# uber/aresdb

Hardware: AMD Instinct MI355X
Metric: rows/sec, 1B-row filter -> group-by-agg (whole job) (higher is better)
Workload: dtype u32 keys / f64 sums; 1 GPU; C3: filter d1<90 -> dims [floor(ts,3600), d1, d2, d3] (4 x uint32) -> SUM(m float32 -> float64) via HashReduce, validity bitmaps with 1% nulls, shard resident in HBM; rows_per_gpu=1000000000, batch_rows=67108864, batches=15, streams_per_query=2, parallelism=1 shard(s), one per GPU

## Files before the change

### aresdb_amd/csrc/algo/hash_reduce_lds.hip

```cpp
#include <hip/hip_runtime.h>

#include <atomic>
#include <functional>
#include <map>
#include <mutex>
#include <string>
#include <unordered_map>

#include <memory>
#include <mutex>
#include <vector>

#include "aggregate.hpp"
#include "common.hpp"
#include "device_model.hpp"
#include "ares_extensions.h"
#include "dim_layout.hpp"
#include "fast_eval.hpp"
#include "hash_reduce_lds.hpp"
#include "hr_kernels.hpp"
#include "hr_rtc.hpp"
#include "sort_reduce_fused.hpp"

namespace ares {

namespace {
using namespace hr;

__global__ __launch_bounds__(kThreads) void hr_partition_kernel(const uint8_t *dimValues, DimLayoutD L, size_t capacity,
                                                                const uint8_t *inputValues, AggSpec a, int length,
                                                                Workspace ws) {
  partition_generic_body(dimValues, L, capacity, inputValues, a, length, ws);
}

template <int ND, int VW>
__global__ __launch_bounds__(kThreads) void hr_partition4_kernel(const uint8_t *dimValues, size_t capacity,
                                                                 const uint8_t *inputValues, uint32_t rowStart, AggSpec a,
                                                                 int length, Workspace ws, int allowDirect) {
  DimVectorSource<ND, VW> src{dimValues, capacity, inputValues, rowStart};
  partition_body(src, a, length, ws, allowDirect);
}

template <int ND>
__global__ __launch_bounds__(kThreads) void hr_fused_scan_kernel(FusedPlanD plan, uint32_t rowBase, AggSpec a, int length,
                                                                 Workspace ws) {
  FusedSource<ND> src(plan, rowBase);
  partition_body(src, a, length, ws, 1);
}

template <int ND4, int RWB>
__global__ __launch_bounds__(kThreads) void hr_merge_kernel(const uint8_t *__restrict__ dimIn,
                                                            const uint8_t *__restrict__ inValues,
                                                            uint8_t *__restrict__ dimOut, DimLayoutD L, size_t capacity,
                                                            uint8_t *__restrict__ outputValues, AggSpec a, Workspace ws,
                                                            uint32_t prevSize) {
  merge_body<ND4, false, RWB>(dimIn, capacity, inValues, dimOut, L, capacity, outputValues, a, ws, nullptr, prevSize);
}

template <int ND, int RWB>
__global__ __launch_bounds__(kThreads) void hr_fused_merge_kernel(FusedPlanD plan, const uint8_t *__restrict__ prevDims,
                                                                  size_t prevCapacity,
                                                                  const uint8_t *__restrict__ prevValues, uint32_t prevSize,
                                                                  uint8_t *__restrict__ dimOut, size_t outCapacity,
                                                                  uint8_t *__restrict__ outputValues, AggSpec a, Workspace ws) {
  DimLayoutD L;
  L.numDims = ND;
  merge_body<ND, true, RWB>(prevDims, prevCapacity, prevValues, dimOut, L, outCapacity, outputValues, a, ws, &plan, prevSize);
}

std::mutex g_rangesMutex;
std::vector<std::pair<int, uint32_t *>> g_freeRanges;

struct SlotWidths {
  int nd = 0, dimBytes = 0;
  uint8_t width[kFusedDims] = {}, off[kFusedDims] = {};
  bool same(const SlotWidths &o) const { return nd == o.nd && memcmp(width, o.width, sizeof(width)) == 0; }
  size_t row_bytes() const { return static_cast<size_t>(dimBytes + nd); }
};
bool slot_widths(const uint8_t numDimsPerDimWidth[NUM_DIM_WIDTH], SlotWidths *out) {
  SlotWidths w;
  if (numDimsPerDimWidth[0] || numDimsPerDimWidth[1]) return false;
  for (int k = 2; k < NUM_DIM_WIDTH; k++)
    for (int j = 0; j < numDimsPerDimWidth[k]; j++) {
      if (w.nd >= kFusedDims) return false;
      w.width[w.nd] = static_cast<uint8_t>(1 << (NUM_DIM_WIDTH - 1 - k));
      w.off[w.nd] = static_cast<uint8_t>(w.dimBytes);
      w.dimBytes += w.width[w.nd];
      w.nd++;
    }
  *out = w;
  return w.nd >= 1;
}

struct GroupedState {
  int device;
  const uint8_t *dims;
  const uint8_t *values;
  size_t capacity;
  SlotWidths slots;
  int valueBytes, size, partBits;
  std::shared_ptr<uint32_t> ranges;
  std::shared_ptr<uint8_t> image;
  uint64_t lineage = 0;
  uint64_t gen = 0, parentGen = 0;
  bool lazyValues = false;
};
std::mutex g_groupedMutex;
std::vector<GroupedState> g_grouped;
constexpr size_t kRangesBytes = sizeof(uint32_t) * kMaxPartitions * kRangeWords;

bool grouped_enabled() {
  static EnvSwitch<bool> on("ARES_GROUPED", [](const char *e) { return !(e && e[0] == '0'); });
  return on.get() && deferral_hooks_active();
}

std::shared_ptr<uint32_t> take_ranges(int device) {
  uint32_t *p = nullptr;
  {
    std::lock_guard<std::mutex> lock(g_rangesMutex);
    for (size_t i = 0; i < g_freeRanges.size(); i++)
      if (g_freeRanges[i].first == device) {
        p = g_freeRanges[i].second;
        g_freeRanges[i] = g_freeRanges.back();
        g_freeRanges.pop_back();
        break;
      }
  }
  if (!p) {
    void *fresh = nullptr;
    hip_check(hipMalloc(&fresh, kRangesBytes), "hipMalloc");
    p = static_cast<uint32_t *>(fresh);
  }
  return std::shared_ptr<uint32_t>(p, [device](uint32_t *q) {
    std::lock_guard<std::mutex> lock(g_rangesMutex);
    g_freeRanges.emplace_back(device, q);
  });
}

constexpr size_t kImagePartBytes = static_cast<size_t>(kSlots) * 16;
constexpr size_t kImageCountsOff = kImagePartBytes * kMaxPartitions;
constexpr size_t kImageBytes = kImageCountsOff + sizeof(uint32_t) * kMaxPartitions;
std::vector<std::pair<int, uint8_t *>> g_freeImages;
std::atomic<uint64_t> g_lineage{0};
std::atomic<uint64_t> g_generation{0};

bool image_enabled() {
  static EnvSwitch<bool> on("ARES_IMAGE", [](const char *e) { return !(e && e[0] == '0'); });
  return on.get() && grouped_enabled();
}

std::shared_ptr<uint8_t> take_image(int device) {
  uint8_t *p = nullptr;
  {
    std::lock_guard<std::mutex> lock(g_rangesMutex);
    for (size_t i = 0; i < g_freeImages.size(); i++)
      if (g_freeImages[i].first == device) {
        p = g_freeImages[i].second;
        g_freeImages[i] = g_freeImages.back();
        g_freeImages.pop_back();
        break;
      }
  }
  if (!p) {
    void *fresh = nullptr;
    if (hipMalloc(&fresh, kImageBytes) != hipSuccess) {
      (void)hipGetLastError();
      grouped_trim(device);
      if (g_memTrimCache) g_memTrimCache(device);
      fresh = nullptr;
      if (hipMalloc(&fresh, kImageBytes) != hipSuccess) {
        (void)hipGetLastError();
        return nullptr;
      }
    }
    p = static_cast<uint8_t *>(fresh);
  }
  return std::shared_ptr<uint8_t>(p, [device](uint8_t *q) {
    std::lock_guard<std::mutex> lock(g_rangesMutex);
    g_freeImages.emplace_back(device, q);
  });
}
uint32_t *image_counts(uint8_t *image) { return reinterpret_cast<uint32_t *>(image + kImageCountsOff); }

template <int VW>
__global__ __launch_bounds__(kThreads) void hr_image_values_kernel(const uint4 *image, uint8_t *values, uint32_t size) {
  const uint4 *img = image + static_cast<size_t>(blockIdx.x) * kSlots;
  const uint32_t *keys = reinterpret_cast<const uint32_t *>(img), *pos = keys + kSlots;
  const uint64_t *vals = reinterpret_cast<const uint64_t *>(img + kSlots / 2);
  for (int s = threadIdx.x; s < kSlots; s += kThreads) {
    if (keys[s] == 0u) continue;
    const uint32_t at = pos[s];
    if (at >= size) continue;
    if (VW == 8) reinterpret_cast<uint64_t *>(values)[at] = vals[s];
    else reinterpret_cast<uint32_t *>(values)[at] = static_cast<uint32_t>(vals[s]);
  }
}

hipStream_t image_stream(int device) {
  static std::mutex mu;
  static std::map<int, hipStream_t> streams;
  std::lock_guard<std::mutex> lock(mu);
  auto it = streams.find(device);
  if (it != streams.end()) return it->second;
  hipStream_t s = nullptr;
  hip_check(hipStreamCreateWithFlags(&s, hipStreamNonBlocking), "hipStreamCreate");
  streams[device] = s;
  return s;
}

void materialize_values(GroupedState &s) {
  if (!s.lazyValues || !s.image) return;
  int current = 0;
  const bool have = hipGetDevice(&current) == hipSuccess;
  if (!have || current != s.device) hip_check(hipSetDevice(s.device), "hipSetDevice");
  hipStream_t stream = image_stream(s.device);
  uint8_t *values = const_cast<uint8_t *>(s.values);
  if (s.valueBytes == 8)
    ARES_LAUNCH("hr_image_values_kernel", hr_image_values_kernel<8>, 1 << s.partBits, kThreads, stream,
                reinterpret_cast<const uint4 *>(s.image.get()), values, static_cast<uint32_t>(s.size));
  else
    ARES_LAUNCH("hr_image_values_kernel", hr_image_values_kernel<4>, 1 << s.partBits, kThreads, stream,
                reinterpret_cast<const uint4 *>(s.image.get()), values, static_cast<uint32_t>(s.size));
  hip_check(hipStreamSynchronize(stream), "hipStreamSynchronize");
  mem_note_write(s.device, values, static_cast<size_t>(s.valueBytes) * s.size);
  s.lazyValues = false;
  if (have && current != s.device) (void)hipSetDevice(current);
}

bool state_overlaps(const GroupedState &s, const uint8_t *lo, const uint8_t *hi) {
  auto hit = [&](const uint8_t *a, size_t bytes) { return a < hi && lo < a + bytes; };
  for (int d = 0; d < s.slots.nd; d++) {
    if (hit(s.dims + s.capacity * s.slots.off[d], static_cast<size_t>(s.slots.width[d]) * s.size)) return true;
    if (hit(s.dims + s.capacity * s.slots.dimBytes + s.capacity * d, static_cast<size_t>(s.size))) return true;
  }
  return hit(s.values, static_cast<size_t>(s.valueBytes) * s.size);
}

bool grouped_lookup(int device, const uint8_t *dims, const uint8_t *values, size_t capacity, const SlotWidths &slots, int valueBytes,
                    GroupedState *out) {
  if (!grouped_enabled()) return false;
  std::lock_guard<std::mutex> lock(g_groupedMutex);
  for (const GroupedState &s : g_grouped)
    if (s.device == device && s.dims == dims && s.values == values && s.capacity == capacity && s.slots.same(slots) &&
        s.valueBytes == valueBytes) {
      *out = s;
      return true;
    }
  return false;
}

void grouped_register(const GroupedState &s) {
  std::lock_guard<std::mutex> lock(g_groupedMutex);
  if (g_grouped.size() >= 64) {
    materialize_values(g_grouped.front());
    g_grouped.erase(g_grouped.begin());
  }
  g_grouped.push_back(s);
}

struct Regions {
  Workspace ws;
  std::unique_ptr<StreamBuffer> buf;
  size_t headBytes;
};

int lean_min_groups() {
  static EnvSwitch<int> v("ARES_LEAN_MIN_GROUPS", [](const char *e) { return e ? atoi(e) : 6000; });
  return v.get();
}

std::mutex g_shapeMutex;
std::unordered_map<size_t, int> g_firstBatchGroups;

int part_bits_for(int64_t length) {
  static EnvSwitch<int> minBits("ARES_MIN_PART_BITS", [](const char *e) { return e ? atoi(e) : 0; });
  int partBits = minBits.get() > 0 ? (minBits.get() < 9 ? minBits.get() : 9) : 0;
  while ((8192ll << partBits) < length && (1 << partBits) < kMaxPartitions) partBits++;
  return partBits;
}

int grid_for(int64_t rows) {
  const int64_t tiles = (rows + kQuadTile - 1) / kQuadTile;
  return static_cast<int>(tiles < kMaxStreams ? (tiles < 1 ? 1 : tiles) : kMaxStreams);
}

bool compact_enabled() {
  static EnvSwitch<bool> on("ARES_COMPACT", [](const char *e) { return !(e && e[0] == '0'); });
  return on.get();
}

void make_regions(Regions &r, int partBits, int64_t rowsA, int64_t rowsB, int streams, int rwB, hipStream_t stream,
                  int lineRecords = 0) {
  const int numParts = 1 << partBits;
  Workspace &ws = r.ws;
  memset(&ws, 0, sizeof(ws));
  ws.partBits = partBits;
  ws.streams = streams;
  ws.capA = ((2ull * (static_cast<uint64_t>(rowsA) / numParts) + 2 * kSlots) | 63ull) + 18;
  ws.capB = 0;
  ws.lineRecords = lineRecords;
  size_t bBytes = 0;
  if (streams > 0) {
    const uint64_t mean = (static_cast<uint64_t>(rowsB) / (static_cast<uint64_t>(numParts) * streams)) << record_stream_slack();
    if (lineRecords == static_cast<int>(kCompactLineRecords)) {
      ws.capB = static_cast<uint32_t>(((2 * mean + 64) / kCompactLineRecords + 2) | 1ull);
      bBytes = 128ull * ws.capB * numParts * streams;
    } else if (lineRecords) {
      ws.capB = static_cast<uint32_t>(((2 * mean + 64 + 7) / 8 * 8) | 8ull);
      bBytes = sizeof(uint32_t) * rwB * static_cast<size_t>(ws.capB) * numParts * streams;
    } else {
      ws.capB = static_cast<uint32_t>(((2 * mean + 64) | 15ull) + 6);
      bBytes = sizeof(uint32_t) * rwB * static_cast<size_t>(ws.capB) * numParts * streams;
    }
  }
  bBytes = (bBytes + 255) / 256 * 256;
  const size_t headBytes = (sizeof(uint32_t) * (numParts + 8) + 255) / 256 * 256;
  const size_t countsBytes = (sizeof(uint32_t) * static_cast<size_t>(numParts) * (streams > 0 ? streams : 1) + 255) / 256 * 256;
  const size_t aBytes = (sizeof(uint4) * ws.capA * numParts + 255) / 256 * 256;
  r.buf.reset(new StreamBuffer(headBytes + countsBytes + aBytes + bBytes + 256, stream));
  uint8_t *base = r.buf->as<uint8_t>();
  ws.cursorsA = reinterpret_cast<uint32_t *>(base);
  ws.outCount = ws.cursorsA + numParts;
  ws.countsB = reinterpret_cast<uint32_t *>(base + headBytes);
  ws.recA = reinterpret_cast<uint4 *>(base + headBytes + countsBytes);
  ws.recB = reinterpret_cast<uint32_t *>(base + headBytes + countsBytes + aBytes);
  r.headBytes = headBytes;
  hip_check(hipMemsetAsync(base, 0, headBytes, stream), "hipMemsetAsync");
}

struct MergeResult {
  uint32_t groups, overflow, stale, needGeneric;
};
MergeResult read_result(const Workspace &ws, hipStream_t stream) {
  uint32_t w[4] = {0, 0, 0, 0};
  read_back_u32(ws.outCount, w, 4, stream);
  return MergeResult{w[0], w[1], w[2], w[3]};
}
uint32_t *result_slot() {
  static EnvSwitch<bool> on("ARES_RESULT_PINNED", [](const char *e) { return e && e[0] == '1'; });
  return on.get() ? reinterpret_cast<uint32_t *>(pinned_words()) : nullptr;
}
MergeResult read_result_pinned(hipStream_t stream) {
  hip_check(hipStreamSynchronize(stream), "hipStreamSynchronize");
  const volatile uint32_t *w = result_slot();
  return MergeResult{w[0], w[1], w[2], w[3]};
}

}

void grouped_note_write(int device, const void *ptr, size_t bytes) {
  sorted_state_note_write(device, ptr, bytes);
  const uint8_t *lo = static_cast<const uint8_t *>(ptr);
  const uint8_t *hi = lo + (bytes ? bytes : 1);
  std::lock_guard<std::mutex> lock(g_groupedMutex);
  for (size_t i = 0; i < g_grouped.size();) {
    GroupedState &st = g_grouped[i];
    if (st.device == device && state_overlaps(st, lo, hi)) {
      const uint8_t *vlo = st.values, *vhi = st.values + static_cast<size_t>(st.valueBytes) * st.size;
      if (st.lazyValues && !(lo <= vlo && vhi <= hi)) materialize_values(st);
      g_grouped.erase(g_grouped.begin() + i);
    } else {
      i++;
    }
  }
}

void grouped_materialize_for_read(int device, const void *ptr, size_t bytes) {
  if (!ptr) return;
  const uint8_t *lo = static_cast<const uint8_t *>(ptr);
  const uint8_t *hi = lo + (bytes ? bytes : 1);
  std::lock_guard<std::mutex> lock(g_groupedMutex);
  for (GroupedState &st : g_grouped) {
    if (st.device != device || !st.lazyValues) continue;
    const uint8_t *vlo = st.values, *vhi = st.values + static_cast<size_t>(st.valueBytes) * st.size;
    if (vlo < hi && lo < vhi) materialize_values(st);
  }
}

void grouped_trim(int device) {
  std::vector<void *> idle;
  {
    std::lock_guard<std::mutex> lock(g_rangesMutex);
    for (size_t i = 0; i < g_freeRanges.size();)
      if (g_freeRanges[i].first == device) {
        idle.push_back(g_freeRanges[i].second);
        g_freeRanges[i] = g_freeRanges.back();
        g_freeRanges.pop_back();
      } else {
        i++;
      }
    for (size_t i = 0; i < g_freeImages.size();)
      if (g_freeImages[i].first == device) {
        idle.push_back(g_freeImages[i].second);
        g_freeImages[i] = g_freeImages.back();
        g_freeImages.pop_back();
      } else {
        i++;
      }
  }
  for (void *p : idle) (void)hipFree(p);
}

void grouped_note_write(int device, const DimensionVector &v) {
  if (v.DimValues && v.VectorCapacity > 0) grouped_note_write(device, v.DimValues, dim_row_bytes(v.NumDimsPerDimWidth) * static_cast<size_t>(v.VectorCapacity));
}

namespace {
std::atomic<int> g_recordStreamSlack{0};
}
int record_stream_slack() { return g_recordStreamSlack.load(std::memory_order_relaxed); }
bool grow_record_stream_slack() {
  int s = g_recordStreamSlack.load(std::memory_order_relaxed);
  while (s < 2)
    if (g_recordStreamSlack.compare_exchange_weak(s, s + 1)) return true;
  return false;
}

bool hash_reduce_lds_supported(const AggSpec &a) {
  if (a.op == OP_AVG) return false;
  if (a.vtype == V_F32 && a.op != OP_SUM) return false;
  return true;
}

int hash_reduce_lds(int device, const DimensionVector &inputKeys, const uint8_t *inputValues,
                    const DimensionVector &outputKeys, uint8_t *outputValues, const AggSpec &a, int length,
                    hipStream_t stream) {
  const DimLayoutD L = make_dim_layout(inputKeys.NumDimsPerDimWidth);
  const size_t capacity = static_cast<size_t>(inputKeys.VectorCapacity);
  bool all4 = L.numDims >= 1 && L.numDims <= 4;
  for (int d = 0; d < L.numDims; d++) all4 = all4 && L.width[d] == 4;
  SlotWidths slots;
  const bool describable = slot_widths(inputKeys.NumDimsPerDimWidth, &slots);
  const int partBits = std::max(part_bits_for(length), (describable && !all4) ? 2 : 0);
  const int numParts = 1 << partBits;
  grouped_note_write(device, outputValues, static_cast<size_t>(a.width) * capacity);
  grouped_note_write(device, outputKeys.DimValues, static_cast<size_t>(L.rowBytes) * capacity);
  GroupedState prev;
  bool grouped = all4 && grouped_lookup(device, inputKeys.DimValues, inputValues, capacity, slots, a.width, &prev) &&
                 prev.ranges && prev.partBits == partBits && prev.size > 0 && prev.size <= length;
  const std::shared_ptr<uint32_t> outRangesRef = (describable && grouped_enabled()) ? take_ranges(device) : nullptr;
  uint32_t *outRanges = outRangesRef.get();
  MergeResult res{0, 0, 0, 0};
  for (;;) {
    const int start = grouped ? prev.size : 0;
    const int rows = length - start;
    RtcKernel lean;
    if (all4 && grouped && rows > 0 && start >= lean_min_groups() && (a.width == 4 || a.width == 8) && rtc_scan_available())
      lean = rtc_lookup(device, rtc_spec_vector_scan(L.numDims, a.width, partBits));
    const int streams = (all4 && rows > 0) ? (lean ? rtc_scan_grid(rows) : grid_for(rows)) : 0;
    const int rwB = (a.width == 8 || lean) ? 4 : 3;
    Regions r;
    make_regions(r, partBits, rows, rows, streams, rwB, stream, lean ? 8 : 0);
    Workspace &ws = r.ws;
    if (lean && a.width == 8) ws.widen.mode = 2;
    ws.prevRanges = grouped ? prev.ranges.get() : nullptr;
    ws.outRanges = outRanges;
    RtcKernel leanMerge = lean ? rtc_lookup(device, rtc_spec_vector_merge(L.numDims, a.width, partBits, a)) : nullptr;
    if (outRanges && !leanMerge) hip_check(hipMemsetAsync(outRanges, 0, kRangesBytes, stream), "hipMemsetAsync");
    if (lean) {
      rtc_vector_scan_launch(lean, RTC_VECTOR_SCAN, inputKeys.DimValues, capacity, inputValues + static_cast<size_t>(a.width) * start,
                             L.numDims, nullptr, static_cast<uint32_t>(start), rows, ws, stream);
    } else if (all4) {
      if (rows > 0) {
#define ARES_HR_CASE(ND)                                                                                             \
  case ND:                                                                                                           \
    if (a.width == 8)                                                                                                \
      ARES_LAUNCH("hr_partition4_kernel", (hr_partition4_kernel<ND, 8>), streams, kThreads, stream, inputKeys.DimValues, \
                  capacity, inputValues, static_cast<uint32_t>(start), a, rows, ws, 1);                             \
    else                                                                                                             \
      ARES_LAUNCH("hr_partition4_kernel", (hr_partition4_kernel<ND, 4>), streams, kThreads, stream, inputKeys.DimValues, \
                  capacity, inputValues, static_cast<uint32_t>(start), a, rows, ws, 1);                             \
    break;
        switch (L.numDims) {
          ARES_HR_CASE(1) ARES_HR_CASE(2) ARES_HR_CASE(3) ARES_HR_CASE(4)
        }
#undef ARES_HR_CASE
      }
    } else {
      const int64_t tiles = (static_cast<int64_t>(length) + kTileRows - 1) / kTileRows;
      const int grid = static_cast<int>(tiles < 256 ? tiles : 256);
      ARES_LAUNCH("hr_partition_kernel", hr_partition_kernel, grid, kThreads, stream, inputKeys.DimValues, L, capacity,
                  inputValues, a, length, ws);
    }
#define ARES_HR_MERGE(ND, RWB)                                                                                       \
  ARES_LAUNCH("hr_merge_kernel", (hr_merge_kernel<ND, RWB>), numParts, kThreads, stream, inputKeys.DimValues, inputValues, \
              outputKeys.DimValues, L, capacity, outputValues, a, ws, static_cast<uint32_t>(start))
#define ARES_HR_MERGE_ND(ND)                       \
  if (rwB == 4) ARES_HR_MERGE(ND, 4);              \
  else ARES_HR_MERGE(ND, 3);
    auto generic_merge = [&] {
      switch (all4 ? L.numDims : 0) {
        case 1: ARES_HR_MERGE_ND(1) break;
        case 2: ARES_HR_MERGE_ND(2) break;
        case 3: ARES_HR_MERGE_ND(3) break;
        case 4: ARES_HR_MERGE_ND(4) break;
        default: ARES_HR_MERGE(0, 3); break;
      }
    };
    if (leanMerge) {
      FusedPlanD none;
      memset(&none, 0, sizeof(none));
      rtc_merge_launch(leanMerge, none, inputKeys.DimValues, capacity, inputValues, static_cast<uint32_t>(start), outputKeys.DimValues,
                       capacity, outputValues, ws, stream, nullptr, result_slot());
    } else {
      generic_merge();
    }
    res = (leanMerge && result_slot()) ? read_result_pinned(stream) : read_result(ws, stream);
    mem_note_dim_rows(device, outputKeys, 0, res.groups);
    mem_note_write(device, outputValues, static_cast<size_t>(a.width) * res.groups);
    if (leanMerge && res.needGeneric && !res.overflow && !(grouped && res.stale)) {
      hip_check(hipMemsetAsync(ws.outCount, 0, 4 * sizeof(uint32_t), stream), "hipMemsetAsync");
      if (outRanges) hip_check(hipMemsetAsync(outRanges, 0, kRangesBytes, stream), "hipMemsetAsync");
      generic_merge();
      res = read_result(ws, stream);
      mem_note_dim_rows(device, outputKeys, 0, res.groups);
      mem_note_write(device, outputValues, static_cast<size_t>(a.width) * res.groups);
    }
#undef ARES_HR_MERGE_ND
#undef ARES_HR_MERGE
    if (hr_trace_enabled())
      fprintf(stderr, "hash_reduce_lds: length %d start %d rows %d streams %d capA %llu capB %u partBits %d -> groups %u overflow %u stale %u\n",
              length, start, rows, streams, static_cast<unsigned long long>(ws.capA), ws.capB, partBits, res.groups, res.overflow, res.stale);
    r.buf->mark_idle();
    if (grouped && res.stale) {
      grouped_note_write(device, inputKeys.DimValues, static_cast<size_t>(L.rowBytes) * capacity);
      grouped = false;
      continue;
    }
    break;
  }
  if (res.overflow) {
    static bool told = false;
    if (!told) {
      told = true;
      fprintf(stderr, "libalgorithm: a hash-partition region overflowed (skewed hashes?): HashReduce falls back to the global table\n");
    }
    return -1;
  }
  if (outRanges) {
    GroupedState s{device, outputKeys.DimValues, outputValues, capacity, slots, a.width, static_cast<int>(res.groups),
                   partBits, outRangesRef};
    if (res.groups > 0) grouped_register(s);
  }
  return static_cast<int>(res.groups);
}

static void fused_note_first_batch(size_t shape, int groups) {
  if (!shape || groups < 0) return;
  std::lock_guard<std::mutex> lock(g_shapeMutex);
  if (g_firstBatchGroups.size() > 4096) g_firstBatchGroups.clear();
  g_firstBatchGroups[shape] = groups;
}

int fused_hash_reduce_run(int device, const FusedPlanD &plan, int batchRows, const DimensionVector &prevKeys,
                          const uint8_t *prevValues, int prevSize, const DimensionVector &outKeys, uint8_t *outValues,
                          const AggSpec &a, hipStream_t stream) {
  SlotWidths slots;
  if (!slot_widths(outKeys.NumDimsPerDimWidth, &slots)) return kFusedUnavailable;
  const int nd = slots.nd;
  const bool narrow = fused_plan_narrow(plan, nd);
  const int mw = plan.measureWidth;
  const int64_t length = static_cast<int64_t>(batchRows) + prevSize;
  if (length == 0) return 0;
  const int partBits = std::max(part_bits_for(length), narrow ? 2 : 0);
  const int numParts = 1 << partBits;
  const size_t prevCapacity = static_cast<size_t>(prevKeys.VectorCapacity);
  const size_t outCapacity = static_cast<size_t>(outKeys.VectorCapacity);
  if (narrow && !(batchRows > 0 && rtc_scan_available())) return kFusedUnavailable;
  GroupedState outOld;
  const bool outFound = image_enabled() && grouped_lookup(device, outKeys.DimValues, outValues, outCapacity, slots, mw, &outOld);
  grouped_note_write(device, outValues, static_cast<size_t>(mw) * outCapacity);
  grouped_note_write(device, outKeys.DimValues, slots.row_bytes() * outCapacity);
  GroupedState prev;
  const bool found = prevSize > 0 && grouped_lookup(device, prevKeys.DimValues, prevValues, prevCapacity, slots, mw, &prev) &&
                     prev.partBits == partBits && prev.size == prevSize;
  bool grouped = found && prev.ranges != nullptr;
  const std::shared_ptr<uint32_t> outRangesRef = grouped_enabled() ? take_ranges(device) : nullptr;
  uint32_t *outRanges = outRangesRef.get();
  MergeResult res{0, 0, 0, 0};
  hr::Widen widen;
  widen.mode = mw == 8 ? 1 : 0;
  widen.rk = plan.measure.f.rk;
  widen.dtype = plan.measureDtype;
  size_t shape = 0;
  int expected = prevSize;
  bool known = prevSize > 0;
  const bool rtc = batchRows > 0 && rtc_scan_available();
  if (rtc && prevSize == 0) {
    const RtcSpec spec = rtc_spec_scan(plan, nd, 0, false);
    shape = std::hash<std::string>()(std::string(reinterpret_cast<const char *>(&spec), sizeof(spec)));
    std::lock_guard<std::mutex> lock(g_shapeMutex);
    auto it = g_firstBatchGroups.find(shape);
    if (it != g_firstBatchGroups.end()) {
      expected = it->second;
      known = true;
    }
  }
  const int chunkTiles = compact_enabled() ? rtc_compact_chunk_tiles(batchRows, partBits) : 0;
  const bool compact = chunkTiles > 0;
  const RtcKind leanKind = compact ? RTC_SCAN_COMPACT : RTC_SCAN_LINES16;
  RtcKernel lean, table, tableMerge, narrowMerge;
  SlowScope slowWhole("fused_hash_reduce_run");
  const bool wantLean = rtc && expected >= lean_min_groups() && (known || lean_min_groups() <= 0);
  const bool wantTable = rtc && !wantLean && (known || narrow);
  if (wantLean) lean = rtc_lookup(device, rtc_spec_scan(plan, nd, partBits, compact));
  else if (wantTable) table = rtc_lookup(device, rtc_spec_table_scan(plan, nd, partBits, a, widen));
  int imageMode = 0;
  RtcKernel imageMerge;
  std::shared_ptr<uint8_t> imageOut;
  uint32_t knownOut = 0;
  if (image_enabled() && wantLean && lean) {
    if (found && prev.image) imageMode = 2;
    else if (prevSize == 0 || grouped) imageMode = 1;
    if (imageMode) imageMerge = rtc_lookup(device, rtc_spec_merge(plan, nd, partBits, a, widen, compact, false, imageMode));
    if (!imageMerge) imageMode = 0;
  }
  if (imageMode == 2) {
    const bool mine = outFound && outOld.lineage == prev.lineage && outOld.image && outOld.image != prev.image &&
                      outOld.partBits == partBits && outOld.size <= prevSize && prev.parentGen != 0 && outOld.gen == prev.parentGen;
    knownOut = mine ? static_cast<uint32_t>(outOld.size) : 0u;
    imageOut = mine ? outOld.image : take_image(device);
    if (imageOut && !mine) hip_check(hipMemsetAsync(image_counts(imageOut.get()), 0xFF, sizeof(uint32_t) * kMaxPartitions, stream), "hipMemsetAsync");
  } else {
    if (imageMode == 1) imageOut = take_image(device);
    if (prevSize > 0) grouped_materialize_for_read(device, prevValues, static_cast<size_t>(mw) * prevSize);
  }
  if (imageMode && !imageOut) {
    imageMode = 0;
    knownOut = 0;
    if (prevSize > 0) grouped_materialize_for_read(device, prevValues, static_cast<size_t>(mw) * prevSize);
  }
  {
    if (hr_trace_enabled())
      fprintf(stderr, "fused_hash_reduce_run: batch %d prev %d partBits %d | found %d (state: size %d partBits %d ranges %d image %d lazy %d) grouped %d "
                      "| lean %d table %d compact %d narrow %d -> image mode %d knownOut %u\n",
              batchRows, prevSize, partBits, found ? 1 : 0, found ? prev.size : -1, found ? prev.partBits : -1, found && prev.ranges ? 1 : 0,
              found && prev.image ? 1 : 0, found && prev.lazyValues ? 1 : 0, grouped ? 1 : 0, lean ? 1 : 0, table ? 1 : 0, compact ? 1 : 0,
              narrow ? 1 : 0, imageMode, knownOut);
  }
  if (narrow && !imageMode) {
    narrowMerge = rtc_lookup(device, rtc_spec_merge(plan, nd, partBits, a, widen, wantLean && compact,
                                                    wantTable || (prevSize > 0 && !grouped)));
    if (!narrowMerge) return kFusedUnavailable;
  }
  if (narrow && !(wantLean ? lean : table)) return kFusedUnavailable;
  bool launched = false;
  for (;;) {
    const bool prevToA = narrow && prevSize > 0 && !grouped && imageMode != 2;
    if (narrow && !imageMode) {
      narrowMerge = rtc_lookup(device, rtc_spec_merge(plan, nd, partBits, a, widen, lean && compact, table || prevToA));
      if (!narrowMerge) return launched ? -1 : kFusedUnavailable;
      if (table) tableMerge = narrowMerge;
    }
    launched = true;
    const int streams = batchRows > 0 ? (lean ? rtc_scan_grid(batchRows) : table ? 0 : grid_for(batchRows)) : 0;
    Regions r;
    {
      SlowScope slow("make_regions");
      const int64_t rowsA = !lean ? length : (prevSize > 0 && !grouped && imageMode != 2) ? prevSize : 0;
      make_regions(r, partBits, rowsA, batchRows, streams, lean ? 4 : 3, stream,
                   !lean ? 0 : compact ? static_cast<int>(kCompactLineRecords) : 8);
    }
    Workspace &ws = r.ws;
    ws.widen = widen;
    ws.chunkRows = static_cast<uint32_t>(chunkTiles) * 4096u;
    ws.rowBase = static_cast<uint32_t>(prevSize);
    ws.prevRanges = (grouped && imageMode != 2) ? prev.ranges.get() : nullptr;
    ws.outRanges = outRanges;
    Workspace wsPrev = ws;
    wsPrev.streams = 0;
    RtcKernel leanMerge = imageMode ? imageMerge
                          : narrow  ? (lean ? narrowMerge : nullptr)
                          : (lean && (prevSize == 0 || grouped)) ? rtc_lookup(device, rtc_spec_merge(plan, nd, partBits, a, widen, compact)) : nullptr;
    RtcImageArgs imageArgs{nullptr, nullptr, nullptr, nullptr, 0u};
    if (imageMode) {
      imageArgs.in = imageMode == 2 ? prev.image.get() : nullptr;
      imageArgs.inCount = imageMode == 2 ? image_counts(prev.image.get()) : nullptr;
      imageArgs.out = imageOut.get();
      imageArgs.outCount = image_counts(imageOut.get());
      imageArgs.knownOut = knownOut;
    }
    const RtcImageArgs *imagePtr = imageMode ? &imageArgs : nullptr;
    if (prevToA) {
      const DimLayoutD prevLayout = make_dim_layout(prevKeys.NumDimsPerDimWidth);
      const int64_t tiles = (static_cast<int64_t>(prevSize) + kTileRows - 1) / kTileRows;
      ARES_LAUNCH("hr_partition_kernel", hr_partition_kernel, static_cast<int>(tiles < 256 ? tiles : 256), kThreads, stream,
                  prevKeys.DimValues, prevLayout, prevCapacity, prevValues, a, prevSize, wsPrev);
    }
    if (outRanges && !leanMerge && !tableMerge) hip_check(hipMemsetAsync(outRanges, 0, kRangesBytes, stream), "hipMemsetAsync");
#define ARES_FUSED_CASE(ND)                                                                                            \
  case ND:                                                                                                             \
    if (prevSize > 0 && !grouped && !narrow && imageMode != 2) {                                                       \
      if (mw == 8)                                                                                                     \
        ARES_LAUNCH("hr_partition4_kernel", (hr_partition4_kernel<ND, 8>), grid_for(prevSize), kThreads, stream,        \
                    prevKeys.DimValues, prevCapacity, prevValues, 0u, a, prevSize, wsPrev, 0);                         \
      else                                                                                                             \
        ARES_LAUNCH("hr_partition4_kernel", (hr_partition4_kernel<ND, 4>), grid_for(prevSize), kThreads, stream,        \
                    prevKeys.DimValues, prevCapacity, prevValues, 0u, a, prevSize, wsPrev, 0);                         \
    }                                                                                                                  \
    if (batchRows > 0 && lean)                                                                                         \
      rtc_scan_launch(lean, leanKind, plan, static_cast<uint32_t>(prevSize), batchRows, ws, stream);                   \
    else if (batchRows > 0 && table)                                                                                   \
      rtc_scan_launch(table, RTC_SCAN_TABLE, plan, static_cast<uint32_t>(prevSize), batchRows, ws, stream);            \
    else if (batchRows > 0)                                                                                            \
      ARES_LAUNCH("hr_fused_scan_kernel", hr_fused_scan_kernel<ND>, streams, kThreads, stream, plan,                   \
                  static_cast<uint32_t>(prevSize), a, batchRows, ws);                                                  \
    if (leanMerge || tableMerge)                                                                                       \
      rtc_merge_launch(leanMerge ? leanMerge : tableMerge, plan, prevKeys.DimValues, prevCapacity, prevValues,         \
                       static_cast<uint32_t>(prevSize), outKeys.DimValues, outCapacity, outValues, ws, stream, imagePtr, \
                       result_slot());                                                                                 \
    else if (lean)                                                                                                     \
      ARES_LAUNCH("hr_fused_merge_kernel", (hr_fused_merge_kernel<ND, 4>), numParts, kThreads, stream, plan,            \
                  prevKeys.DimValues, prevCapacity, prevValues, static_cast<uint32_t>(prevSize), outKeys.DimValues,    \
                  outCapacity, outValues, a, ws);                                                                      \
    else                                                                                                               \
      ARES_LAUNCH("hr_fused_merge_kernel", (hr_fused_merge_kernel<ND, 3>), numParts, kThreads, stream, plan,            \
                  prevKeys.DimValues, prevCapacity, prevValues, static_cast<uint32_t>(prevSize), outKeys.DimValues,    \
                  outCapacity, outValues, a, ws);                                                                      \
    break;
    switch (nd) {
      ARES_FUSED_CASE(1) ARES_FUSED_CASE(2) ARES_FUSED_CASE(3) ARES_FUSED_CASE(4)
      default:
        if (batchRows > 0 && lean) rtc_scan_launch(lean, leanKind, plan, static_cast<uint32_t>(prevSize), batchRows, ws, stream);
        else if (batchRows > 0 && table) rtc_scan_launch(table, RTC_SCAN_TABLE, plan, static_cast<uint32_t>(prevSize), batchRows, ws, stream);
        rtc_merge_launch(leanMerge ? leanMerge : tableMerge, plan, prevKeys.DimValues, prevCapacity, prevValues, static_cast<uint32_t>(prevSize),
                         outKeys.DimValues, outCapacity, outValues, ws, stream, imagePtr, result_slot());
        break;
    }
    {
      SlowScope slow("read_result");
      res = ((leanMerge || tableMerge) && result_slot()) ? read_result_pinned(stream) : read_result(ws, stream);
    }
    if (imageMode == 2) res.groups += static_cast<uint32_t>(prevSize);
    if (imageMode == 2) {
      if (res.groups > knownOut) mem_note_dim_rows(device, outKeys, knownOut, res.groups - knownOut);
    } else {
      mem_note_dim_rows(device, outKeys, 0, res.groups);
      mem_note_write(device, outValues, static_cast<size_t>(mw) * res.groups);
    }
    if ((narrow || imageMode == 2) && res.needGeneric) {
      r.buf->mark_idle();
      return -1;
    }
    if (imageMode == 1 && res.needGeneric) imageMode = 0;
    if (leanMerge && res.needGeneric && !res.overflow && !(grouped && res.stale)) {
      hip_check(hipMemsetAsync(ws.outCount, 0, 4 * sizeof(uint32_t), stream), "hipMemsetAsync");
      if (outRanges) hip_check(hipMemsetAsync(outRanges, 0, kRangesBytes, stream), "hipMemsetAsync");
      switch (nd) {
#define ARES_FUSED_REMERGE(ND)                                                                                         \
  case ND:                                                                                                             \
    ARES_LAUNCH("hr_fused_merge_kernel", (hr_fused_merge_kernel<ND, 4>), numParts, kThreads, stream, plan,              \
                prevKeys.DimValues, prevCapacity, prevValues, static_cast<uint32_t>(prevSize), outKeys.DimValues,      \
                outCapacity, outValues, a, ws);                                                                        \
    break;
        ARES_FUSED_REMERGE(1) ARES_FUSED_REMERGE(2) ARES_FUSED_REMERGE(3) ARES_FUSED_REMERGE(4)
#undef ARES_FUSED_REMERGE
      }
      res = read_result(ws, stream);
      mem_note_dim_rows(device, outKeys, 0, res.groups);
      mem_note_write(device, outValues, static_cast<size_t>(mw) * res.groups);
    }
#undef ARES_FUSED_CASE
    r.buf->mark_idle();
    if (grouped && res.stale) {
      grouped_note_write(device, prevKeys.DimValues, slots.row_bytes() * prevCapacity);
      grouped = false;
      imageMode = 0;
      continue;
    }
    if (res.overflow && lean && grow_record_stream_slack()) continue;
    break;
  }
  if (res.overflow) {
    return -1;
  }
  fused_note_first_batch(shape, static_cast<int>(res.groups));
  if (shape && !lean && !table) {
    if (static_cast<int>(res.groups) >= lean_min_groups()) {
      (void)rtc_lookup(device, rtc_spec_scan(plan, nd, partBits, compact));
      (void)rtc_lookup(device, rtc_spec_merge(plan, nd, partBits, a, widen, compact));
    } else {
      (void)rtc_lookup(device, rtc_spec_table_scan(plan, nd, partBits, a, widen));
    }
  }
  if (outRanges) {
    GroupedState s{device, outKeys.DimValues, outValues, outCapacity, slots, mw, static_cast<int>(res.groups), partBits, outRangesRef};
    if (imageMode == 2) {
      s.ranges = nullptr;
      s.image = imageOut;
      s.lineage = prev.lineage;
      s.gen = ++g_generation;
      s.parentGen = prev.gen;
      s.lazyValues = true;
    } else if (imageMode == 1) {
      s.image = imageOut;
      s.lineage = ++g_lineage;
      s.gen = ++g_generation;
    }
    if (res.groups > 0) grouped_register(s);
  }
  return static_cast<int>(res.groups);
}

namespace {

struct NotFusable : std::runtime_error {
  explicit NotFusable(const std::string &why) : std::runtime_error("not fusable: " + why) {}
};

void fused_expr(const AresFusedExpr &e, bool compareOnly, int batchRows, hipStream_t stream, FusedPlanD &plan, int maxCols,
                FusedExpr &out) {
  if (e.arity != 1 && e.arity != 2) throw NotFusable("arity");
  if (e.lhs.Type != VectorPartyInput || (e.arity == 2 && e.rhs.Type != ConstantInput))
    throw NotFusable("operands must be a main-table column and a constant");
  if (static_cast<int64_t>(e.lhs.Vector.VP.Length) < batchRows) throw NotFusable("column shorter than the batch");
  InputVector ins[2] = {e.lhs, e.arity == 2 ? e.rhs : e.lhs};
  EvalParams p;
  CallTemps temps;
  build_params(ins, e.arity, stream, nullptr, nullptr, 0, e.functor, p, temps);
  FastOperands f;
  if (!fast_operands(p, f, compareOnly)) throw NotFusable("expression shape");
  out.col = fused_column(plan, f, maxCols, compareOnly ? kFusedReuseFirst : kFusedNoReuse);
  if (out.col < 0) throw NotFusable("too many distinct columns");
  out.f = f;
  out.f.vals = nullptr;
  out.f.nulls = nullptr;
  out.outKind = e.outType == Int32 ? K_I32 : e.outType == Uint32 ? K_U32 : K_F32;
}

int fused_filter_hash_reduce(int device, const AresFusedQuery &q, int batchRows, const DimensionVector &prevKeys,
                             uint8_t *prevValues, int prevSize, const DimensionVector &outKeys, uint8_t *outValues,
                             hipStream_t stream) {
  if (q.numDims < 1 || q.numDims > kGenericFusedDims) throw NotFusable("1..4 dimensions");
  if (q.numFilters < 0 || q.numFilters > kExtensionFilters) throw NotFusable("at most 4 filters");
  const int nd = q.numDims;
  for (int k = 0; k < NUM_DIM_WIDTH; k++)
    if (outKeys.NumDimsPerDimWidth[k] != (k == 2 ? nd : 0) || (prevSize > 0 && prevKeys.NumDimsPerDimWidth[k] != (k == 2 ? nd : 0)))
      throw NotFusable("dimension vector layout");
  const int mt = q.measure.outType;
  if (!(mt == Int32 || mt == Uint32 || mt == Float32 || mt == Int64 || mt == Float64)) throw NotFusable("measure type");
  const int mw = (mt == Int64 || mt == Float64) ? 8 : 4;
  const AggSpec a = make_agg_spec(q.aggFunc, mw);
  if (!hash_reduce_lds_supported(a)) throw NotFusable("aggregate");
  if (batchRows < 0 || prevSize < 0 || static_cast<int64_t>(batchRows) + prevSize > INT32_MAX) throw NotFusable("size");
  if (static_cast<int64_t>(outKeys.VectorCapacity) < static_cast<int64_t>(batchRows) + prevSize)
    throw std::invalid_argument("outKeys.VectorCapacity < prevSize + batchRows");

  FusedPlanD plan;
  memset(&plan, 0, sizeof(plan));
  const int maxCols = nd + 2;
  plan.numFilters = q.numFilters;
  for (int d = 0; d < nd; d++) {
    const int t = q.dims[d].outType;
    if (!(t == Int32 || t == Uint32 || t == Float32)) throw NotFusable("dimension type");
    fused_expr(q.dims[d], false, batchRows, stream, plan, maxCols, plan.dims[d]);
  }
  fused_expr(q.measure, false, batchRows, stream, plan, maxCols, plan.measure);
  for (int k = 0; k < q.numFilters; k++) fused_expr(q.filters[k], true, batchRows, stream, plan, maxCols, plan.filters[k]);
  plan.measureDtype = mt;
  plan.measureWidth = mw;
  plan.identity = identity_bits(q.aggFunc, mt);
  if (mw == 8 && plan.identity != 0) throw NotFusable("8-byte aggregate with a non-zero identity");

  const int groups = fused_hash_reduce_run(device, plan, batchRows, prevKeys, prevValues, prevSize, outKeys, outValues, a, stream);
  if (groups == kFusedUnavailable)
    throw NotFusable("the kernels generated for this plan's shape are not loaded yet (compiled in the background), or the shape is outside what they cover; "
                     "run the unfused sequence for this batch");
  if (groups < 0) throw NotFusable("a hash partition overflowed (skewed hashes); run the unfused sequence");
  return groups;
}

}

}

extern "C" CGoCallResHandle AresFusedFilterHashReduce(const AresFusedQuery *query, int batchRows, DimensionVector prevKeys,
                                                      uint8_t *prevValues, int prevSize, DimensionVector outKeys,
                                                      uint8_t *outValues, void *cudaStream, int device) {
  ARES_ABI_BEGIN(device)
  if (!query) throw std::invalid_argument("null query");
  resHandle.res = ares::int_result(ares::fused_filter_hash_reduce(device, *query, batchRows, prevKeys, prevValues, prevSize, outKeys,
                                                                  outValues, reinterpret_cast<hipStream_t>(cudaStream)));
  ARES_ABI_END("AresFusedFilterHashReduce")
}
```

### aresdb_amd/csrc/algo/hr_rtc.hip

```cpp
#include <dlfcn.h>
#include <hip/hip_runtime.h>
#include <sys/stat.h>
#include <cerrno>
#include <unistd.h>

#include <atomic>
#include <chrono>
#include <condition_variable>
#include <fstream>
#include <memory>
#include <mutex>
#include <string>
#include <thread>
#include <unordered_map>
#include <vector>

#include "common.hpp"
#include "hash_reduce_lds.hpp"
#include "hr_kernels.hpp"
#include "hr_rtc.hpp"

namespace ares {

bool phases_enabled() {
  static const bool on = [] { const char *e = getenv("ARES_HR_PHASES"); return e && e[0] == '1'; }();
  return on;
}

namespace {

typedef struct _hiprtcProgram *RtcProgram;
struct RtcApi {
  int (*create)(RtcProgram *, const char *, const char *, int, const char **, const char **) = nullptr;
  int (*compile)(RtcProgram, int, const char **) = nullptr;
  int (*logSize)(RtcProgram, size_t *) = nullptr;
  int (*log)(RtcProgram, char *) = nullptr;
  int (*codeSize)(RtcProgram, size_t *) = nullptr;
  int (*code)(RtcProgram, char *) = nullptr;
  int (*destroy)(RtcProgram *) = nullptr;
  int (*version)(int *, int *) = nullptr;
  bool ok = false;
};
const RtcApi &rtc_api() {
  static const RtcApi api = [] {
    RtcApi a;
    const char *e = getenv("ARES_RTC");
    if (e && e[0] == '0') return a;
    void *h = dlopen("libhiprtc.so", RTLD_NOW | RTLD_LOCAL);
    if (!h) h = dlopen("libhiprtc.so.7", RTLD_NOW | RTLD_LOCAL);
    if (!h) h = dlopen("/opt/rocm/lib/libhiprtc.so", RTLD_NOW | RTLD_LOCAL);
    if (!h) return a;
    a.create = reinterpret_cast<decltype(a.create)>(dlsym(h, "hiprtcCreateProgram"));
    a.compile = reinterpret_cast<decltype(a.compile)>(dlsym(h, "hiprtcCompileProgram"));
    a.logSize = reinterpret_cast<decltype(a.logSize)>(dlsym(h, "hiprtcGetProgramLogSize"));
    a.log = reinterpret_cast<decltype(a.log)>(dlsym(h, "hiprtcGetProgramLog"));
    a.codeSize = reinterpret_cast<decltype(a.codeSize)>(dlsym(h, "hiprtcGetCodeSize"));
    a.code = reinterpret_cast<decltype(a.code)>(dlsym(h, "hiprtcGetCode"));
    a.destroy = reinterpret_cast<decltype(a.destroy)>(dlsym(h, "hiprtcDestroyProgram"));
    a.version = reinterpret_cast<decltype(a.version)>(dlsym(h, "hiprtcVersion"));
    a.ok = a.create && a.compile && a.logSize && a.log && a.codeSize && a.code && a.destroy;
    return a;
  }();
  return api;
}

struct RtcArgs {
  const uint32_t *vals[kFusedCols];
  const uint8_t *nulls[kFusedCols];
  uint32_t *recB;
  uint32_t *countsB;
  uint32_t *overflow;
  uint64_t *phases;
  uint4 *recA;
  uint32_t *cursorsA;
  uint64_t capA;
  uint32_t bitOff[kFusedCols];
  uint32_t rowBase;
  int length;
  uint32_t capB;
  uint32_t chunkTiles;
  uint32_t k[kNumConsts];
  uint32_t pad;
};
static_assert(sizeof(RtcArgs) % 8 == 0, "Args is passed as one buffer");

struct RtcMergeArgs {
  const uint32_t *vals[kFusedCols];
  const uint8_t *nulls[kFusedCols];
  const uint32_t *recB;
  const uint32_t *countsB;
  const uint32_t *prevRanges;
  const uint8_t *prevDims;
  const uint8_t *prevValues;
  uint8_t *dimOut;
  uint8_t *outValues;
  uint32_t *outCount;
  uint32_t *outRanges;
  uint64_t prevCapacity, outCapacity;
  uint32_t bitOff[kFusedCols];
  uint32_t capB, streams, prevSize, chunkRows;
  uint64_t *phases;
  uint32_t k[kNumConsts];
  uint32_t pad;
  const uint4 *recA;
  const uint32_t *cursorsA;
  uint64_t capA;
  const uint4 *imgIn;
  uint4 *imgOut;
  const uint32_t *imgInCount;
  uint32_t *imgOutCount;
  uint32_t *hostOut;
  uint32_t knownOut, pad2;
};
static_assert(sizeof(RtcMergeArgs) % 8 == 0, "MArgs is passed as one buffer");

}

struct RtcEntry {
  int device = 0;
  std::mutex m;
  std::condition_variable cv;
  bool ready = false;
  bool codeReady = false;
  bool fromDisk = false;
  std::vector<char> code;
  std::string diskPath;
  hipModule_t module = nullptr;
  hipFunction_t fn = nullptr;
  std::atomic<uint64_t> lastUse{0};
  ~RtcEntry();
};

namespace {
std::mutex g_graveMutex;
std::vector<std::pair<int, hipModule_t>> g_graveyard;
constexpr size_t kGraveyardLimit = 128;
}

RtcEntry::~RtcEntry() {
  if (!module) return;
  std::vector<std::pair<int, hipModule_t>> unload;
  {
    std::lock_guard<std::mutex> lock(g_graveMutex);
    g_graveyard.emplace_back(device, module);
    if (g_graveyard.size() >= kGraveyardLimit) {
      unload.assign(g_graveyard.begin(), g_graveyard.begin() + kGraveyardLimit / 2);
      g_graveyard.erase(g_graveyard.begin(), g_graveyard.begin() + kGraveyardLimit / 2);
    }
  }
  if (unload.empty()) return;
  int current = 0;
  const bool have = hipGetDevice(&current) == hipSuccess;
  int synced = -1;
  for (auto &dm : unload) {
    if (dm.first != synced) {
      (void)hipSetDevice(dm.first);
      (void)hipDeviceSynchronize();
      synced = dm.first;
    }
    (void)hipModuleUnload(dm.second);
  }
  if (have) (void)hipSetDevice(current);
  (void)hipGetLastError();
}

namespace {

struct RtcCache {
  std::mutex mu;
  std::unordered_map<std::string, std::shared_ptr<RtcEntry>> map;
  std::mutex frontMu;
  std::unordered_map<std::string, RtcKernel> front;
  std::atomic<uint64_t> tick{0};
  std::atomic<int> pending{0};
  std::mutex idleMu;
  std::condition_variable idleCv;
  std::atomic<long> compiles{0}, diskHits{0}, evictions{0};
};
RtcCache &cache() {
  static RtcCache *c = new RtcCache;
  return *c;
}

size_t cache_capacity() {
  static const size_t cap = [] {
    const char *e = getenv("ARES_RTC_CACHE_ENTRIES");
    const long v = e ? atol(e) : 256;
    return static_cast<size_t>(v < 4 ? 4 : v);
  }();
  return cap;
}

bool rtc_async() {
  static const bool on = [] {
    const char *e = getenv("ARES_RTC_ASYNC");
    return !(e && e[0] == '0');
  }();
  return on;
}

std::string disk_dir() {
  static const std::string dir = [] {
    std::string d;
    if (const char *e = getenv("ARES_RTC_CACHE_DIR")) {
      d = e;
      if (d == "0" || d == "off") d.clear();
      if (d.empty()) return d;
    } else if (const char *x = getenv("XDG_CACHE_HOME")) {
      d = std::string(x) + "/aresdb_amd/rtc";
    } else if (const char *h = getenv("HOME")) {
      d = std::string(h) + "/.cache/aresdb_amd/rtc";
    } else {
      return d;
    }
    std::string partial;
    for (size_t i = 0; i <= d.size(); i++)
      if (i == d.size() || (d[i] == '/' && i > 0)) {
        partial = d.substr(0, i);
        if (mkdir(partial.c_str(), 0700) != 0 && errno != EEXIST) return std::string();
      }
    return d;
  }();
  return dir;
}

constexpr uint64_t kDiskMagic = 0x3143545253455241ull;
uint64_t fnv1a(const std::string &s, uint64_t h) {
  for (unsigned char c : s) {
    h ^= c;
    h *= 1099511628211ull;
  }
  return h;
}

constexpr const char *kRtcOptions[] = {"-O3", "-std=c++17", "-munsafe-fp-atomics"};
constexpr int kRtcOptionCount = 3;

std::string disk_name(const std::string &arch, const std::string &source) {
  int major = 0, minor = 0, runtime = 0;
  if (rtc_api().version) (void)rtc_api().version(&major, &minor);
  if (hipRuntimeGetVersion(&runtime) != hipSuccess) {
    (void)hipGetLastError();
    runtime = 0;
  }
  std::string salt = arch + "|hiprtc " + std::to_string(major) + "." + std::to_string(minor) + "|runtime " + std::to_string(runtime) + "|";
  for (int k = 0; k < kRtcOptionCount; k++) salt += std::string(kRtcOptions[k]) + " ";
  salt += "|";
  char b[48];
  snprintf(b, sizeof(b), "%016llx%016llx.co", static_cast<unsigned long long>(fnv1a(source, fnv1a(salt, 14695981039346656037ull))),
           static_cast<unsigned long long>(fnv1a(source, fnv1a(salt, 0x9e3779b97f4a7c15ull))));
  return b;
}

std::string device_arch(int device) {
  hipDeviceProp_t prop;
  if (hipGetDeviceProperties(&prop, device) != hipSuccess) {
    (void)hipGetLastError();
    return "gfx950";
  }
  return prop.gcnArchName[0] ? std::string(prop.gcnArchName) : std::string("gfx950");
}

bool compile_source(const std::string &source, const std::string &arch, const char *entry, std::vector<char> &code) {
  const RtcApi &api = rtc_api();
  RtcProgram prog = nullptr;
  if (!api.ok || !api.create) return false;
  if (api.create(&prog, source.c_str(), "hr_rtc.hip", 0, nullptr, nullptr) != 0) return false;
  const std::string archOpt = "--offload-arch=" + arch;
  const char *opts[1 + kRtcOptionCount] = {archOpt.c_str()};
  for (int k = 0; k < kRtcOptionCount; k++) opts[1 + k] = kRtcOptions[k];
  bool ok = false;
  if (api.compile(prog, 1 + kRtcOptionCount, opts) == 0) {
    size_t size = 0;
    if (api.codeSize(prog, &size) == 0 && size) {
      code.resize(size);
      ok = api.code(prog, code.data()) == 0;
    }
  } else {
    size_t n = 0;
    std::string log;
    if (api.logSize(prog, &n) == 0 && n) {
      log.resize(n);
      api.log(prog, &log[0]);
    }
    fprintf(stderr, "libalgorithm: hiprtc could not compile %s (generic kernel used): %s\n", entry, log.c_str());
  }
  api.destroy(&prog);
  return ok;
}

void rtc_trace(const char *what, const std::string &entry, double ms, size_t bytes) {
  static const char *path = getenv("ARES_RTC_TRACE");
  if (!path || !path[0]) return;
  static std::mutex mu;
  std::lock_guard<std::mutex> lock(mu);
  if (FILE *o = fopen(path, "a")) {
    const double now = std::chrono::duration<double, std::milli>(std::chrono::steady_clock::now().time_since_epoch()).count();
    fprintf(o, "%.3f %s %s %.3f ms %zu bytes\n", now, what, entry.c_str(), ms, bytes);
    fclose(o);
  }
}
struct TraceClock {
  std::chrono::steady_clock::time_point t0 = std::chrono::steady_clock::now();
  double ms() const { return std::chrono::duration<double, std::milli>(std::chrono::steady_clock::now() - t0).count(); }
};

std::string disk_path(int device, const std::string &source) {
  const std::string dir = disk_dir();
  return dir.empty() ? std::string() : dir + "/" + disk_name(device_arch(device), source);
}

bool read_disk(const std::string &path, const std::string &entryName, std::vector<char> &code) {
  code.clear();
  if (path.empty()) return false;
  TraceClock tRead;
  std::ifstream in(path, std::ios::binary | std::ios::ate);
  if (!in) return false;
  const std::streamsize n = in.tellg();
  uint64_t head[3] = {0, 0, 0};
  if (n > static_cast<std::streamsize>(sizeof(head))) {
    in.seekg(0);
    if (in.read(reinterpret_cast<char *>(head), sizeof(head)) && head[0] == kDiskMagic && head[1] == static_cast<uint64_t>(n) - sizeof(head)) {
      code.resize(static_cast<size_t>(head[1]));
      if (!in.read(code.data(), static_cast<std::streamsize>(code.size())) ||
          fnv1a(std::string(code.data(), code.size()), 14695981039346656037ull) != head[2])
        code.clear();
    }
  }
  if (code.empty()) {
    (void)unlink(path.c_str());
    return false;
  }
  rtc_trace("disk_read", entryName, tRead.ms(), code.size());
  return true;
}

void write_disk(const std::string &path, const std::vector<char> &code) {
  if (path.empty() || code.empty()) return;
  const std::string tmp = path + ".tmp" + std::to_string(static_cast<long>(getpid())) + "." + std::to_string(cache().tick.load());
  std::ofstream out(tmp, std::ios::binary);
  const uint64_t head[3] = {kDiskMagic, static_cast<uint64_t>(code.size()), fnv1a(std::string(code.data(), code.size()), 14695981039346656037ull)};
  if (out && out.write(reinterpret_cast<const char *>(head), sizeof(head)) && out.write(code.data(), static_cast<std::streamsize>(code.size())) &&
      (out.close(), true)) {
    if (rename(tmp.c_str(), path.c_str()) != 0) (void)unlink(tmp.c_str());
  } else {
    (void)unlink(tmp.c_str());
  }
}

void load_entry(RtcEntry &e, const std::string &entryName) {
  TraceClock tLoad;
  hipModule_t module = nullptr;
  hipFunction_t fn = nullptr;
  if (!e.code.empty() && hipModuleLoadData(&module, e.code.data()) == hipSuccess) {
    if (hipModuleGetFunction(&fn, module, entryName.c_str()) != hipSuccess) fn = nullptr;
  } else {
    module = nullptr;
  }
  (void)hipGetLastError();
  rtc_trace("module_load", entryName, tLoad.ms(), e.code.size());
  if (fn) {
    int scratch = 0;
    if (hipFuncGetAttribute(&scratch, HIP_FUNC_ATTRIBUTE_LOCAL_SIZE_BYTES, fn) == hipSuccess)
      rtc_trace("scratch_bytes_per_lane", entryName, 0.0, static_cast<size_t>(scratch));
    (void)hipGetLastError();
  }
  if (!fn && e.fromDisk && !e.diskPath.empty()) (void)unlink(e.diskPath.c_str());
  if (fn && !e.fromDisk) write_disk(e.diskPath, e.code);
  e.code.clear();
  e.code.shrink_to_fit();
  e.module = module;
  e.fn = fn;
  e.codeReady = false;
  e.ready = true;
}

void compile_entry(const std::shared_ptr<RtcEntry> &e, const std::string &source, const std::string &entryName) {
  RtcCache &c = cache();
  std::vector<char> code;
  TraceClock tCompile;
  const bool ok = compile_source(source, device_arch(e->device), entryName.c_str(), code);
  c.compiles++;
  rtc_trace("hiprtc_compile", entryName, tCompile.ms(), code.size());
  {
    std::lock_guard<std::mutex> lock(e->m);
    if (ok) {
      e->code.swap(code);
      e->codeReady = true;
    } else {
      e->ready = true;
    }
  }
  e->cv.notify_all();
  if (c.pending.fetch_sub(1) == 1) {
    std::lock_guard<std::mutex> lock(c.idleMu);
    c.idleCv.notify_all();
  }
}

void wait_idle() {
  RtcCache &c = cache();
  std::unique_lock<std::mutex> lock(c.idleMu);
  c.idleCv.wait(lock, [&] { return c.pending.load() == 0; });
}

RtcKernel compiled_kernel(int device, const std::string &source, const char *entry, bool wait) {
  if (source.empty()) return nullptr;
  RtcCache &c = cache();
  const std::string key = std::to_string(device) + "|" + entry + "|" + source;
  std::shared_ptr<RtcEntry> e;
  std::vector<std::shared_ptr<RtcEntry>> evicted;
  bool created = false;
  {
    std::lock_guard<std::mutex> lock(c.mu);
    auto it = c.map.find(key);
    if (it != c.map.end()) {
      e = it->second;
    } else {
      while (c.map.size() >= cache_capacity()) {
        auto victim = c.map.end();
        for (auto jt = c.map.begin(); jt != c.map.end(); ++jt) {
          bool ready;
          {
            std::lock_guard<std::mutex> el(jt->second->m);
            ready = jt->second->ready || jt->second->codeReady;
          }
          if (ready && (victim == c.map.end() || jt->second->lastUse.load() < victim->second->lastUse.load())) victim = jt;
        }
        if (victim == c.map.end()) break;
        evicted.push_back(victim->second);
        c.map.erase(victim);
        c.evictions++;
      }
      e = std::make_shared<RtcEntry>();
      e->device = device;
      c.map.emplace(key, e);
      created = true;
      c.pending++;
      static const int registered = atexit([] { wait_idle(); });
      (void)registered;
    }
    e->lastUse.store(++c.tick);
  }
  evicted.clear();
  if (created) {
    e->diskPath = disk_path(device, source);
    std::vector<char> code;
    if (read_disk(e->diskPath, entry, code)) {
      c.diskHits++;
      {
        std::lock_guard<std::mutex> lock(e->m);
        e->code.swap(code);
        e->fromDisk = true;
        e->codeReady = true;
      }
      e->cv.notify_all();
      if (c.pending.fetch_sub(1) == 1) {
        std::lock_guard<std::mutex> idle(c.idleMu);
        c.idleCv.notify_all();
      }
    } else if (rtc_async() && !wait) {
      std::thread([e, source, name = std::string(entry)] { compile_entry(e, source, name); }).detach();
    } else {
      compile_entry(e, source, entry);
    }
  }
  std::unique_lock<std::mutex> lock(e->m);
  if (!e->ready && !e->codeReady) {
    if (rtc_async() && !wait) return nullptr;
    e->cv.wait(lock, [&] { return e->ready || e->codeReady; });
  }
  if (!e->ready) {
    (void)hipSetDevice(device);
    load_entry(*e, entry);
    e->cv.notify_all();
  }
  return e->fn ? e : nullptr;
}

template <typename Args>
void fill_columns(Args &args, const FusedPlanD &plan) {
  memset(&args, 0, sizeof(args));
  for (int c = 0; c < plan.numCols; c++) {
    args.vals[c] = plan.cols[c].vals;
    args.nulls[c] = plan.cols[c].nulls;
    args.bitOff[c] = plan.cols[c].bitOff;
  }
  for (int d = 0; d < kFusedDims; d++) args.k[const_slot_dim(d)] = plan.dims[d].f.bbits;
}

struct PhaseReport {
  uint64_t *dev = nullptr;
  int launches = 0;
  uint64_t *buffer(size_t workgroups) {
    if (!dev) hip_check(hipMalloc(reinterpret_cast<void **>(&dev), sizeof(uint64_t) * 8 * workgroups), "hipMalloc");
    return dev;
  }
  bool fetch(std::vector<uint64_t> &h, int workgroups, hipStream_t stream) {
    h.resize(static_cast<size_t>(8) * workgroups);
    hip_check(hipMemcpyAsync(h.data(), dev, sizeof(uint64_t) * h.size(), hipMemcpyDeviceToHost, stream), "hipMemcpyAsync");
    hip_check(hipStreamSynchronize(stream), "hipStreamSynchronize");
    return ++launches <= 3 || launches % 64 == 0;
  }
};

void launch(const RtcKernel &kernel, void *args, size_t size, unsigned grid, hipStream_t stream, const char *name) {
  void *config[] = {HIP_LAUNCH_PARAM_BUFFER_POINTER, args, HIP_LAUNCH_PARAM_BUFFER_SIZE, &size, HIP_LAUNCH_PARAM_END};
  KernelTimer timer(name, stream);
  hip_check(hipModuleLaunchKernel(kernel->fn, grid, 1, 1, hr::kThreads, 1, 1, 0, stream, nullptr, config), "hipModuleLaunchKernel");
}

void launch_scan(const RtcKernel &kernel, const FusedPlanD &plan, uint32_t rowBase, int length, const hr::Workspace &ws, int grid,
                 uint32_t chunkTiles, uint32_t pad, hipStream_t stream, const char *name) {
  RtcArgs args;
  fill_columns(args, plan);
  for (int k = 0; k < plan.numFilters && k < kFusedFilters; k++)
    args.k[const_slot_filter(k)] = host_cvt32(plan.filters[k].f.bbits, plan.filters[k].f.bkind, plan.filters[k].f.I);
  args.k[const_slot_measure()] = plan.measure.f.bbits;
  args.recB = ws.recB;
  args.countsB = ws.countsB;
  args.overflow = ws.outCount + 1;
  args.recA = ws.recA;
  args.cursorsA = ws.cursorsA;
  args.capA = ws.capA;
  args.rowBase = rowBase;
  args.length = length;
  args.capB = ws.capB;
  args.chunkTiles = chunkTiles;
  args.pad = pad;
  static PhaseReport report;
  if (phases_enabled()) args.phases = report.buffer(hr::kMaxStreams);
  launch(kernel, &args, sizeof(args), static_cast<unsigned>(grid), stream, name);
  std::vector<uint64_t> h;
  if (phases_enabled() && report.fetch(h, grid, stream)) {
    double sum[7] = {0, 0, 0, 0, 0, 0, 0};
    for (int g = 0; g < grid; g++)
      for (int k = 0; k < 7; k++) sum[k] += static_cast<double>(h[static_cast<size_t>(8) * g + k]);
    const double n = grid * 1e3;
    fprintf(stderr, "%s phases (launch %d, %d workgroups, %d rows): kcycles per workgroup: eval+count %.1f, scan %.1f, scatter %.1f, lines %.1f, leftovers %.1f, drain %.1f, last lines %.1f\n",
            name, report.launches, grid, length, sum[0] / n, sum[1] / n, sum[2] / n, sum[3] / n, sum[4] / n, sum[5] / n, sum[6] / n);
  }
}

}

bool rtc_scan_available() { return rtc_api().ok; }

int rtc_scan_grid(int64_t rows) {
  const int64_t tiles = (rows + 4095) / 4096;
  return static_cast<int>(tiles < hr::kMaxStreams ? (tiles < 1 ? 1 : tiles) : hr::kMaxStreams);
}

int rtc_compact_chunk_tiles(int64_t rows, int partBits) {
  if (partBits < 3 || rows <= 0) return 0;
  const int64_t tiles = (rows + 4095) / 4096;
  const int64_t grid = rtc_scan_grid(rows);
  const int64_t chunk = (tiles + grid - 1) / grid;
  return chunk <= (1ll << (partBits - 3)) ? static_cast<int>(chunk) : 0;
}

RtcKernel rtc_lookup(int device, const RtcSpec &spec, bool wait) {
  if (!rtc_api().ok) return nullptr;
  std::string key(reinterpret_cast<const char *>(&spec), sizeof(spec));
  key.append(reinterpret_cast<const char *>(&device), sizeof(device));
  RtcCache &c = cache();
  {
    std::lock_guard<std::mutex> lock(c.frontMu);
    auto it = c.front.find(key);
    if (it != c.front.end()) return it->second;
  }
  RtcKernel k = compiled_kernel(device, rtc_source(spec), rtc_entry_name(spec.kind), wait);
  if (k) {
    std::lock_guard<std::mutex> lock(c.frontMu);
    if (c.front.size() >= 64) c.front.clear();
    c.front.emplace(key, k);
  }
  return k;
}

void rtc_scan_launch(const RtcKernel &kernel, RtcKind kind, const FusedPlanD &plan, uint32_t rowBase, int length, const hr::Workspace &ws,
                     hipStream_t stream) {
  const int grid = kind == RTC_SCAN_TABLE ? rtc_scan_grid(length) : ws.streams;
  const uint32_t chunkTiles = kind == RTC_SCAN_COMPACT ? ws.chunkRows / 4096u : 0u;
  launch_scan(kernel, plan, rowBase, length, ws, grid, chunkTiles, 0u, stream,
              kind == RTC_SCAN_TABLE ? "hr_table_scan_rtc" : rtc_entry_name(kind));
}

void rtc_vector_scan_launch(const RtcKernel &kernel, RtcKind kind, const uint8_t *dimValues, size_t capacity, const void *measures, int nd,
                            const int *widths, uint32_t rowBase, int length, const hr::Workspace &ws, hipStream_t stream, int totalPartBits,
                            bool spread) {
  FusedPlanD plan;
  memset(&plan, 0, sizeof(plan));
  fused_plan_vector_columns(plan, dimValues, capacity, nd, widths, rowBase);
  plan.cols[nd].vals = static_cast<const uint32_t *>(measures);
  launch_scan(kernel, plan, rowBase, length, ws, ws.streams, totalPartBits > 0 ? static_cast<uint32_t>(32 - totalPartBits) : 0u,
              spread ? 1u : 0u, stream, kind == RTC_SORT_VECTOR_SCAN ? "sr_vector_scan_rtc" : rtc_entry_name(kind));
}

void rtc_merge_launch(const RtcKernel &kernel, const FusedPlanD &plan, const uint8_t *prevDims, size_t prevCapacity, const uint8_t *prevValues,
                      uint32_t prevSize, uint8_t *dimOut, size_t outCapacity, uint8_t *outValues, const hr::Workspace &ws,
                      hipStream_t stream, const RtcImageArgs *image, uint32_t *hostOut) {
  RtcMergeArgs args;
  fill_columns(args, plan);
  args.recB = ws.recB;
  args.countsB = ws.countsB;
  args.prevRanges = ws.prevRanges;
  args.prevDims = prevDims;
  args.prevValues = prevValues;
  args.dimOut = dimOut;
  args.outValues = outValues;
  args.outCount = ws.outCount;
  args.outRanges = ws.outRanges;
  args.prevCapacity = prevCapacity;
  args.outCapacity = outCapacity;
  args.capB = ws.capB;
  args.recA = ws.recA;
  args.cursorsA = ws.cursorsA;
  args.capA = ws.capA;
  args.streams = static_cast<uint32_t>(ws.streams);
  args.prevSize = prevSize;
  args.chunkRows = ws.chunkRows;
  if (image) {
    args.imgIn = reinterpret_cast<const uint4 *>(image->in);
    args.imgOut = reinterpret_cast<uint4 *>(image->out);
    args.imgInCount = image->inCount;
    args.imgOutCount = image->outCount;
    args.knownOut = image->knownOut;
  }
  args.hostOut = hostOut;
  static PhaseReport report;
  if (phases_enabled()) {
    args.phases = report.buffer(hr::kMaxPartitions);
    hip_check(hipMemsetAsync(args.phases, 0, sizeof(uint64_t) * 8 * hr::kMaxPartitions, stream), "hipMemsetAsync");
  }
  launch(kernel, &args, sizeof(args), 1u << ws.partBits, stream, "hr_merge_rtc");
  const int np = 1 << ws.partBits;
  std::vector<uint64_t> h;
  if (phases_enabled() && report.fetch(h, np, stream)) {
    uint64_t first = ~0ull, last = 0;
    double sum[5] = {0, 0, 0, 0, 0}, whole = 0;
    for (int p = 0; p < np; p++) {
      const uint64_t *t = &h[static_cast<size_t>(8) * p];
      if (t[0] < first) first = t[0];
      if (t[5] > last) last = t[5];
      for (int k = 0; k < 5; k++) sum[k] += static_cast<double>(t[k + 1] - t[k]) * 0.01;
      whole += static_cast<double>(t[5] - t[0]) * 0.01;
    }
    fprintf(stderr, "hr_merge_rtc phases (launch %d, %d partitions, prev %u): span %.1f us; per partition avg %.1f us = init %.1f + prev %.1f + records %.1f + count %.1f + emit %.1f\n",
            report.launches, np, prevSize, static_cast<double>(last - first) * 0.01, whole / np, sum[0] / np, sum[1] / np, sum[2] / np, sum[3] / np, sum[4] / np);
  }
}

}

extern "C" size_t AresRtcWait(long *counters) {
  ares::wait_idle();
  ares::RtcCache &c = ares::cache();
  if (counters) {
    counters[0] = c.compiles.load();
    counters[1] = c.diskHits.load();
    counters[2] = c.evictions.load();
  }
  std::lock_guard<std::mutex> lock(c.mu);
  return c.map.size();
}
```

### aresdb_amd/csrc/algo/hr_rtc.hpp

```cpp
#pragma once

#include <hip/hip_runtime.h>

#include <memory>

#include "hr_rtc_gen.hpp"

namespace ares {
namespace hr { struct Workspace; }

struct RtcEntry;
using RtcKernel = std::shared_ptr<RtcEntry>;

bool rtc_scan_available();
int rtc_scan_grid(int64_t rows);
int rtc_compact_chunk_tiles(int64_t rows, int partBits);

RtcKernel rtc_lookup(int device, const RtcSpec &spec, bool wait = false);

void rtc_scan_launch(const RtcKernel &kernel, RtcKind kind, const FusedPlanD &plan, uint32_t rowBase, int length, const hr::Workspace &ws,
                     hipStream_t stream);
void rtc_vector_scan_launch(const RtcKernel &kernel, RtcKind kind, const uint8_t *dimValues, size_t capacity, const void *measures, int nd,
                            const int *widths, uint32_t rowBase, int length, const hr::Workspace &ws, hipStream_t stream,
                            int totalPartBits = 0, bool spread = false);
struct RtcImageArgs {
  const void *in;
  void *out;
  const uint32_t *inCount;
  uint32_t *outCount;
  uint32_t knownOut;
};
void rtc_merge_launch(const RtcKernel &kernel, const FusedPlanD &plan, const uint8_t *prevDims, size_t prevCapacity,
                      const uint8_t *prevValues, uint32_t prevSize, uint8_t *dimOut, size_t outCapacity, uint8_t *outValues,
                      const hr::Workspace &ws, hipStream_t stream, const RtcImageArgs *image = nullptr, uint32_t *hostOut = nullptr);

}
```

### aresdb_amd/csrc/algo/hr_rtc_gen.hip

```cpp
#include <cstdio>
#include <functional>
#include <sstream>
#include <string>
#include <vector>

#include "hr_kernels.hpp"
#include "hr_rtc_gen.hpp"

namespace ares {

namespace {

bool int_kind(int k) { return k == K_I32 || k == K_U32; }
bool col_kind(int k) { return k == K_I32 || k == K_U32 || k == K_F32; }

std::string hex(uint32_t v) {
  char b[16];
  snprintf(b, sizeof(b), "0x%08xu", v);
  return b;
}

std::string const_name(int slot) { return "a.k[" + std::to_string(slot) + "]"; }

bool gen_value(const RtcExpr &f, std::ostringstream &o, const char *v, const char *okb, const char *r, const std::string &kc,
// ... 93 lines not shown
bool gen_widen(std::ostringstream &o, const RtcSpec &s) {
  o << "__device__ __forceinline__ u64 widen(u32 raw) {\n";
  if (s.widenMode == 0) o << "  return raw;\n";
  else if (s.widenDtype == Float64)
    o << (s.widenRk == K_F32 ? "  return (u64)__double_as_longlong((double)__uint_as_float(raw));\n"
          : s.widenRk == K_I32 ? "  return (u64)__double_as_longlong((double)(i32)raw);\n"
                          : "  return (u64)__double_as_longlong((double)raw);\n");
  else
    o << (s.widenRk == K_F32 ? "  return (u64)(i64)__uint_as_float(raw);\n" : s.widenRk == K_I32 ? "  return (u64)(i64)(i32)raw;\n" : "  return (u64)(i64)raw;\n");
  o << "}\n";
  return true;
}

bool gen_agg(std::ostringstream &o, const RtcSpec &s) {
  o << "__device__ __forceinline__ void agg(u64 *slot, u64 bits) {\n";
  switch (s.aggVtype) {
    case V_F64: o << "  __hip_atomic_fetch_add(reinterpret_cast<double *>(slot), __longlong_as_double((long long)bits), __ATOMIC_RELAXED, __HIP_MEMORY_SCOPE_WORKGROUP);\n"; break;
    case V_U64: case V_I64: o << "  __hip_atomic_fetch_add(slot, bits, __ATOMIC_RELAXED, __HIP_MEMORY_SCOPE_WORKGROUP);\n"; break;
    case V_F32: o << "  __hip_atomic_fetch_add(reinterpret_cast<float *>(slot), __uint_as_float((u32)bits), __ATOMIC_RELAXED, __HIP_MEMORY_SCOPE_WORKGROUP);\n"; break;
    case V_U32:
      o << "  __hip_atomic_fetch_" << (s.aggOp == OP_SUM ? "add" : s.aggOp == OP_MIN ? "min" : "max")
        << "(reinterpret_cast<u32 *>(slot), (u32)bits, __ATOMIC_RELAXED, __HIP_MEMORY_SCOPE_WORKGROUP);\n";
      break;
    case V_I32:
      o << "  __hip_atomic_fetch_" << (s.aggOp == OP_SUM ? "add" : s.aggOp == OP_MIN ? "min" : "max")
        << "(reinterpret_cast<i32 *>(slot), (i32)(u32)bits, __ATOMIC_RELAXED, __HIP_MEMORY_SCOPE_WORKGROUP);\n";
      break;
    default: return false;
  }
  o << "}\n";
  char ident[32];
  snprintf(ident, sizeof(ident), "0x%016llxull", static_cast<unsigned long long>(s.aggIdentity));
  o << "#define IDENT " << ident << "\n";
  return true;
}

struct Lines16 {
  const char *fourth;
  const char *part = "(PB ? hh[j] >> (32 - (PB ? PB : 1)) : 0u)";
  const char *row = "a.rowBase + i0 + j";
};
static void kernel_body_lines16(std::ostringstream &o, const RtcSpec &s, const Lines16 &rec) {
  const char *fourth = rec.fourth, *part = rec.part, *row = rec.row, *entry = rtc_entry_name(s.kind);
  phase_macros(o, s);
  o << "#define T 4096u\n"
       "__device__ __forceinline__ u32 lane_up(u32 v, u32 lane, u32 off) { return (u32)__builtin_amdgcn_ds_bpermute((int)((lane - off) << 2), (int)v); }\n"
       "extern \"C\" __global__ void __launch_bounds__(1024) " << entry << "(Args a) {\n"
       "  __shared__ uint4 sRec[T];\n"
       "  __shared__ uint4 sLeft[NP * 7u];\n"
       "  __shared__ u32 sCount[2][NP];\n"
       "  __shared__ u32 sStart[NP], sLeftN[NP], sCursor[NP];\n"
       "  __shared__ u32 sLines[(T + NP * 7u) / 8u + 1u];\n"
       "  __shared__ u32 sWave[16];\n"
       "  __shared__ u32 sTotalLines;\n"
       "  const u32 tid = threadIdx.x, lane = tid & 63u, wave = tid >> 6;\n"
       "  for (u32 p = tid; p < NP; p += 1024u) { sCount[0][p] = 0u; sCount[1][p] = 0u; sLeftN[p] = 0u; sCursor[p] = 0u; }\n"
       "  __syncthreads();\n"
       "  uint4 *myB = reinterpret_cast<uint4 *>(a.recB) + (u64)blockIdx.x * NP * a.capB;\n"
       "  const u32 numTiles = ((u32)a.length + T - 1u) / T;\n"
       "  u32 tile = blockIdx.x, par = 0u;\n"
       "  Raw R;\n"
       "  PH_DECL\n"
       "  load_tile(R, a, tile * T + tid * 4u);\n"
       "  while (tile < numTiles) {\n"
       "    u32 i0 = tile * T + tid * 4u;\n"
       "    u32 hh[4], cv[4], cw[4], alive[4], rank[4];\n"
       "    const u32 next = tile + gridDim.x;\n"
       "    eval4p(R, a, i0, hh, cv, cw, alive, next * T + tid * 4u);\n"
       "    u32 *cnt = sCount[par];\n"
       "#pragma unroll\n"
       "    for (int j = 0; j < 4; j++) {\n"
       "      rank[j] = 0u;\n"
       "      if (alive[j]) rank[j] = __hip_atomic_fetch_add(&cnt[" << part << "], 1u, __ATOMIC_RELAXED, __HIP_MEMORY_SCOPE_WORKGROUP);\n"
       "    }\n"
       "    __syncthreads();\n"
       "    PH(0)\n"
       "    u32 myCount = 0u, myLeft = 0u;\n"
       "    if (tid < NP) { myCount = cnt[tid]; myLeft = sLeftN[tid]; }\n"
       "    const u32 myHave = myCount + myLeft, myLines = myHave >> 3;\n"
       "    const u32 packed = (myCount << 16) | myLines;\n"
       "    u32 incl = packed;\n"
       "#pragma unroll\n"
       "    for (u32 off = 1u; off < 64u; off <<= 1) { const u32 t = lane_up(incl, lane, off); if (lane >= off) incl += t; }\n"
       "    if (lane == 63u) sWave[wave] = incl;\n"
       "    __syncthreads();\n"
       "    u32 before = 0u;\n"
       "#pragma unroll\n"
       "    for (u32 w = 0u; w < (NP + 63u) / 64u; w++) { const u32 t = sWave[w]; before += w < wave ? t : 0u; }\n"
       "    const u32 excl = before + incl - packed;\n"
       "    const u32 myStart = excl >> 16, myLineStart = excl & 0xFFFFu;\n"
       "    if (tid < NP) {\n"
       "      sStart[tid] = myStart;\n"
       "      for (u32 c = 0u; c < myLines; c++) sLines[myLineStart + c] = tid | (c << 9);\n"
       "      if (tid == NP - 1u) sTotalLines = myLineStart + myLines;\n"
       "    }\n"
       "    __syncthreads();\n"
       "    PH(1)\n"
       "#pragma unroll\n"
       "    for (int j = 0; j < 4; j++)\n"
       "      if (alive[j]) sRec[sStart[" << part << "] + rank[j]] = make_uint4(" << row << ", hh[j], cv[j], " << fourth << ");\n"
       "    __syncthreads();\n"
       "    PH(2)\n"
       "    const u32 totalLines = sTotalLines;\n"
       "    for (u32 L0 = tid >> 3; L0 < totalLines; L0 += 512u) {\n"
       "      const u32 q = tid & 7u;\n"
       "      u32 e[4], lf[4], st[4], cu[4];\n"
       "#pragma unroll\n"
       "      for (u32 j = 0u; j < 4u; j++) { const u32 L = L0 + j * 128u; e[j] = L < totalLines ? sLines[L] : 0u; }\n"
       "#pragma unroll\n"
       "      for (u32 j = 0u; j < 4u; j++) { const u32 p = e[j] & 511u; lf[j] = sLeftN[p]; st[j] = sStart[p]; cu[j] = sCursor[p]; }\n"
       "      uint4 rec[4];\n"
       "#pragma unroll\n"
       "      for (u32 j = 0u; j < 4u; j++) {\n"
       "        const u32 p = e[j] & 511u, idx = (e[j] >> 9) * 8u + q;\n"
       "        const uint4 *src = idx < lf[j] ? sLeft + p * 7u + idx : sRec + ((st[j] + idx - lf[j]) & (T - 1u));\n"
       "        rec[j] = *src;\n"
       "      }\n"
       "#pragma unroll\n"
       "      for (u32 j = 0u; j < 4u; j++) {\n"
       "        const u32 p = e[j] & 511u, at = cu[j] + (e[j] >> 9) * 8u + q;\n"
       "        if (L0 + j * 128u < totalLines && at < a.capB) myB[(u64)p * a.capB + at] = rec[j];\n"
       "      }\n"
       "    }\n"
       "    __syncthreads();\n"
       "    PH(3)\n"
       "    if (tid < NP) {\n"
       "      const u32 rem = myHave & 7u;\n"
       "      const u32 n = myLines ? rem : myCount;\n"
       "      const uint4 *src = sRec + (myLines ? myStart + myLines * 8u - myLeft : myStart);\n"
       "      uint4 *dst = sLeft + tid * 7u + (myLines ? 0u : myLeft);\n"
       "      uint4 t[7];\n"
       "#pragma unroll\n"
       "      for (u32 k = 0u; k < 7u; k++) t[k] = src[k < n ? k : 0u];\n"
       "#pragma unroll\n"
       "      for (u32 k = 0u; k < 7u; k++) if (k < n) dst[k] = t[k];\n"
       "      sLeftN[tid] = rem;\n"
       "      u32 cur = sCursor[tid] + myLines * 8u;\n"
       "      if (cur > a.capB) { *a.overflow = 1u; cur = a.capB; }\n"
       "      sCursor[tid] = cur;\n"
       "      cnt[tid] = 0u;\n"
       "    }\n"
       "    par ^= 1u;\n"
       "    tile = next;\n"
       "    PH(4)\n"
       "  }\n"
       "  __syncthreads();\n"
       "  PH(5)\n"
       "  for (u32 p = tid >> 3; p < NP; p += 128u) {\n"
       "    const u32 left = sLeftN[p], j = tid & 7u, cur = sCursor[p];\n"
       "    const bool fits = cur + 8u <= a.capB;\n"
       "    if (left && fits) myB[(u64)p * a.capB + cur + j] = j < left ? sLeft[p * 7u + j] : make_uint4(0xFFFFFFFFu, 0u, 0u, 0u);\n"
       "    if (left && !fits) *a.overflow = 1u;\n"
       "    if (j == 0u) a.countsB[(u64)blockIdx.x * NP + p] = (left && fits) ? cur + 8u : cur;\n"
       "  }\n"
       "  PH(6)\n"
       "  PH_OUT\n"
       "}\n";
}

static void kernel_body_compact(std::ostringstream &o, const RtcSpec &s) {
  phase_macros(o, s);
  o << "#define STORE_LINE(p, v) (*(p) = (v))\n"
       "#define T 4096u\n#define LR 14u\n#define LEFT 13u\n#define LPL 5u\n"
       "__device__ __forceinline__ u32 lane_up(u32 v, u32 lane, u32 off) { return (u32)__builtin_amdgcn_ds_bpermute((int)((lane - off) << 2), (int)v); }\n"
       "__device__ __forceinline__ u32 or8(u32 v) {\n"
       "  v |= (u32)__builtin_amdgcn_mov_dpp((int)v, 0xB1, 0xF, 0xF, true);\n"
       "  v |= (u32)__builtin_amdgcn_mov_dpp((int)v, 0x4E, 0xF, 0xF, true);\n"
       "  v |= (u32)__builtin_amdgcn_mov_dpp((int)v, 0x141, 0xF, 0xF, true);\n"
       "  return v;\n"
       "}\n"
       "__device__ __forceinline__ u32 wave_incl_scan(u32 v) {\n"
       "  v += (u32)__builtin_amdgcn_update_dpp(0, (int)v, 0x111, 0xF, 0xF, false);\n"
       "  v += (u32)__builtin_amdgcn_update_dpp(0, (int)v, 0x112, 0xF, 0xF, false);\n"
       "  v += (u32)__builtin_amdgcn_update_dpp(0, (int)v, 0x114, 0xF, 0xF, false);\n"
       "  v += (u32)__builtin_amdgcn_update_dpp(0, (int)v, 0x118, 0xF, 0xF, false);\n"
       "  v += (u32)__builtin_amdgcn_update_dpp(0, (int)v, 0x142, 0xA, 0xF, false);\n"
       "  v += (u32)__builtin_amdgcn_update_dpp(0, (int)v, 0x143, 0xC, 0xF, false);\n"
       "  return v;\n"
       "}\n"
       "extern \"C\" __global__ void __launch_bounds__(1024) hr_scan_rtc(Args a) {\n"
       "  __shared__ u64 sRec[T + NP * LEFT];\n"
       "  __shared__ u16 sLo[T + NP * LEFT];\n"
       "  __shared__ u32 sCount[2][NP];\n"
       "  __shared__ u32 sStart[NP];\n"
       "  __shared__ uint2 sLines[(T + NP * LEFT) / LR + 2u];\n"
       "  __shared__ u32 sWave[16];\n"
       "  __shared__ u32 sTotalLines;\n"
       "  const u32 tid = threadIdx.x, lane = tid & 63u, wave = tid >> 6;\n"
       "  for (u32 p = tid; p < NP; p += 1024u) { sCount[0][p] = 0u; sCount[1][p] = 0u; }\n"
       "  u32 myLeftN = 0u, myCursor = 0u;\n"
       "  __syncthreads();\n"
       "  u64 *myB = reinterpret_cast<u64 *>(a.recB) + (u64)blockIdx.x * NP * a.capB * 16u;\n"
       "  const u32 numTiles = ((u32)a.length + T - 1u) / T;\n"
       "  const u32 firstTile = blockIdx.x * a.chunkTiles;\n"
       "  const u32 endTile = firstTile + a.chunkTiles < numTiles ? firstTile + a.chunkTiles : numTiles;\n"
       "  u32 tile = firstTile, par = 0u;\n"
       "  Raw R;\n"
       "  PH_DECL\n"
       "  load_tile(R, a, tile * T + tid * 4u);\n"
       "  const u32 q = tid & 15u, r8 = q & 7u;\n"
       "  const u32 kk = (q >> 3) * 7u + (r8 ? r8 - 1u : 0u);\n"
       "  const u32 sh = r8 ? 9u * (r8 - 1u) : 0u;\n"
       "  while (tile < endTile) {\n"
       "    u32 i0 = tile * T + tid * 4u;\n"
       "    u32 hh[4], cv[4], cw[4], alive[4], rank[4];\n"
       "    const u32 next = tile + 1u;\n"
       "    eval4p(R, a, i0, hh, cv, cw, alive, next * T + tid * 4u);\n"
       "    const u32 rc0 = i0 - firstTile * T;\n"
       "    u32 *cnt = sCount[par];\n"
       "#pragma unroll\n"
       "    for (int j = 0; j < 4; j++) {\n"
       "      rank[j] = 0u;\n"
       "      if (alive[j]) rank[j] = __hip_atomic_fetch_add(&cnt[hh[j] >> (32 - PB)], 1u, __ATOMIC_RELAXED, __HIP_MEMORY_SCOPE_WORKGROUP);\n"
       "    }\n"
       "    __syncthreads();\n"
       "    PH(0)\n"
       "    u32 myCount = 0u, myLeft = 0u;\n"
       "    if (tid < NP) { myCount = cnt[tid]; myLeft = myLeftN; }\n"
       "    const u32 myHave = myCount + myLeft, myLines = myHave / LR;\n"
       "    const u32 packed = (myCount << 16) | myLines;\n"
       "    const u32 incl = wave_incl_scan(packed);\n"
       "    if (lane == 63u) sWave[wave] = incl;\n"
       "    __syncthreads();\n"
       "    u32 before = 0u;\n"
       "#pragma unroll\n"
       "    for (u32 w = 0u; w < (NP + 63u) / 64u; w++) { const u32 t = sWave[w]; before += w < wave ? t : 0u; }\n"
       "    const u32 excl = before + incl - packed;\n"
       "    const u32 myStart = excl >> 16, myLineStart = excl & 0xFFFFu;\n"
       "    if (tid < NP) {\n"
       "      sStart[tid] = myLines ? myStart : T + tid * LEFT + myLeft;\n"
       "      for (u32 c = 0u; c < myLines; c++) sLines[myLineStart + c] = make_uint2(tid | (c << 9) | (myLeft << 18), myStart | (myCursor << 13));\n"
       "      if (tid == NP - 1u) sTotalLines = myLineStart + myLines;\n"
       "    }\n"
       "    __syncthreads();\n"
       "    PH(1)\n"
       "#pragma unroll\n"
       "    for (int j = 0; j < 4; j++)\n"
       "      if (alive[j]) {\n"
       "        const u32 at = sStart[hh[j] >> (32 - PB)] + rank[j], rc = rc0 + (u32)j;\n"
       "        sRec[at] = ((u64)((hh[j] << PB) | (rc >> 9)) << 32) | cv[j];\n"
       "        sLo[at] = (u16)(rc & 511u);\n"
       "      }\n"
       "    __syncthreads();\n"
       "    PH(2)\n"
       "    const u32 totalLines = sTotalLines;\n"
       "    for (u32 L0 = tid >> 4; L0 < totalLines; L0 += 64u * LPL) {\n"
       "      u32 e[LPL], lf[LPL], st[LPL], cu[LPL], lo[LPL];\n"
       "      u64 rec[LPL];\n"
       "#pragma unroll\n"
       "      for (u32 j = 0u; j < LPL; j++) {\n"
       "        const u32 L = L0 + j * 64u;\n"
       "        const uint2 w = L < totalLines ? sLines[L] : make_uint2(0u, 0u);\n"
       "        e[j] = w.x & 0x3FFFFu; lf[j] = w.x >> 18; st[j] = w.y & 0x1FFFu; cu[j] = w.y >> 13;\n"
       "      }\n"
       "#pragma unroll\n"
       "      for (u32 j = 0u; j < LPL; j++) {\n"
       "        const u32 p = e[j] & 511u, idx = (e[j] >> 9) * LR + kk;\n"
       "        const u32 at = idx < lf[j] ? T + p * LEFT + idx : st[j] + idx - lf[j];\n"
       "        rec[j] = sRec[at];\n"
       "        lo[j] = sLo[at];\n"
       "      }\n"
       "#pragma unroll\n"
       "      for (u32 j = 0u; j < LPL; j++) {\n"
       "        const u64 mine = r8 ? (u64)lo[j] << sh : 0ull;\n"
       "        const u64 hdr = ((u64)or8((u32)(mine >> 32)) << 32) | or8((u32)mine);\n"
       "        const u32 p = e[j] & 511u, line = cu[j] + (e[j] >> 9);\n"
       "        if (L0 + j * 64u < totalLines && line < a.capB) STORE_LINE(&myB[((u64)p * a.capB + line) * 16u + q], r8 ? rec[j] : hdr);\n"
       "      }\n"
       "    }\n"
       "    __syncthreads();\n"
       "    PH(3)\n"
       "    if (tid < NP) {\n"
       "      const u32 rem = myHave - myLines * LR;\n"
       "      if (myLines) {\n"
       "        const u32 from = myStart + myLines * LR - myLeft, to = T + tid * LEFT;\n"
       "        u64 t[LEFT]; u16 tl[LEFT];\n"
       "#pragma unroll\n"
       "        for (u32 k = 0u; k < LEFT; k++) { t[k] = sRec[from + k]; tl[k] = sLo[from + k]; }\n"
       "#pragma unroll\n"
       "        for (u32 k = 0u; k < LEFT; k++) { sRec[to + k] = t[k]; sLo[to + k] = tl[k]; }\n"
       "      }\n"
       "      myLeftN = rem;\n"
       "      u32 cur = myCursor + myLines;\n"
       "      if (cur > a.capB) { *a.overflow = 1u; cur = a.capB; }\n"
       "      myCursor = cur;\n"
       "      cnt[tid] = 0u;\n"
       "    }\n"
       "    par ^= 1u;\n"
       "    tile = next;\n"
       "    PH(4)\n"
       "  }\n"
       "  __syncthreads();\n"
       "  if (tid < NP) sLines[tid] = make_uint2(myLeftN, myCursor);\n"
       "  __syncthreads();\n"
       "  PH(5)\n"
       "  for (u32 p = tid >> 4; p < NP; p += 64u) {\n"
       "    const uint2 m = sLines[p];\n"
       "    const u32 left = m.x, cur = m.y;\n"
       "    const bool fits = cur < a.capB, has = r8 && kk < left;\n"
       "    const u64 rec = has ? sRec[T + p * LEFT + kk] : 0ull;\n"
       "    const u64 mine = has ? (u64)sLo[T + p * LEFT + kk] << sh : 0ull;\n"
       "    const u64 hdr = ((u64)or8((u32)(mine >> 32)) << 32) | or8((u32)mine);\n"
       "    if (left && fits) STORE_LINE(&myB[((u64)p * a.capB + cur) * 16u + q], r8 ? rec : hdr);\n"
       "    if (left && !fits) *a.overflow = 1u;\n"
       "    if (q == 0u) a.countsB[(u64)blockIdx.x * NP + p] = cur * LR + ((left && fits) ? left : 0u);\n"
       "  }\n"
       "  PH(6)\n"
       "  PH_OUT\n"
       "}\n";
}

static void kernel_body_table(std::ostringstream &o) {
  o << "#define T 4096u\n#define SLOTS " << hr::kSlots << "u\n#define BUCKETS (SLOTS / 4u)\n#define LIMIT " << (hr::kSlots * 3 / 4)
    << "u\n#define EMPTY 0xFFFFFFFFu\n#define QCAP 128u\n"
       "struct Probe { u32 b, slot; bool done, spill; };\n"
       "__device__ __forceinline__ void probe_round(u32 *sKeys, u32 *sClaims, Probe &q, u32 h) {\n"
       "  const uint4 k = *reinterpret_cast<const uint4 *>(sKeys + 4u * q.b);\n"
       "  const bool e0 = k.x == EMPTY, e1 = k.y == EMPTY, e2 = k.z == EMPTY, e3 = k.w == EMPTY;\n"
       "  const bool m0 = k.x == h, m1 = k.y == h, m2 = k.z == h, m3 = k.w == h;\n"
       "  const bool anyM = m0 | m1 | m2 | m3, anyE = e0 | e1 | e2 | e3;\n"
       "  const u32 mi = m0 ? 0u : m1 ? 1u : m2 ? 2u : 3u, ei = e0 ? 0u : e1 ? 1u : e2 ? 2u : 3u;\n"
       "  const bool active = !q.done, hit = active & anyM;\n"
       "  q.slot = hit ? 4u * q.b + mi : q.slot;\n"
       "  bool claimed = false;\n"
       "  if (active & !anyM & anyE) {\n"
       "    if (__hip_atomic_load(sClaims, __ATOMIC_RELAXED, __HIP_MEMORY_SCOPE_WORKGROUP) >= LIMIT) {\n"
       "      q.spill = true; claimed = true;\n"
       "    } else {\n"
       "      u32 expected = EMPTY;\n"
       "      if (__hip_atomic_compare_exchange_strong(sKeys + 4u * q.b + ei, &expected, h, __ATOMIC_RELAXED, __ATOMIC_RELAXED, __HIP_MEMORY_SCOPE_WORKGROUP)) {\n"
       "        __hip_atomic_fetch_add(sClaims, 1u, __ATOMIC_RELAXED, __HIP_MEMORY_SCOPE_WORKGROUP);\n"
       "        q.slot = 4u * q.b + ei; claimed = true;\n"
       "      }\n"
       "    }\n"
       "  }\n"
       "  q.b = (active & !anyM & !anyE) ? (q.b + 1u) & (BUCKETS - 1u) : q.b;\n"
       "  q.done = q.done | hit | claimed;\n"
       "}\n"
       "__device__ __forceinline__ void insert(const Args &a, u32 *sKeys, u32 *sRows, u64 *sVals, u32 *sClaims, u32 row, u32 h, u32 carried) {\n"
       "  const u64 value = widen(carried);\n"
       "  Probe q; q.b = h & (BUCKETS - 1u); q.slot = 0u; q.done = false; q.spill = h == EMPTY;\n"
       "  for (u32 tries = 0u; tries < BUCKETS + 8u && !q.done && !q.spill; tries++) probe_round(sKeys, sClaims, q, h);\n"
       "  if (q.done && !q.spill) {\n"
       "    __hip_atomic_fetch_min(sRows + q.slot, row, __ATOMIC_RELAXED, __HIP_MEMORY_SCOPE_WORKGROUP);\n"
       "    agg(sVals + q.slot, value);\n"
       "  } else {\n"
       "    const u32 p = PB ? h >> (32 - (PB ? PB : 1)) : 0u;\n"
       "    const u64 at = atomicAdd(a.cursorsA + p, 1u);\n"
       "    if (at < a.capA) a.recA[(u64)p * a.capA + at] = make_uint4(row, h, (u32)value, (u32)(value >> 32));\n"
       "    else *a.overflow = 1u;\n"
       "  }\n"
       "}\n"
       "__device__ __forceinline__ void drain(const Args &a, u32 *queue, u32 first, u32 count, u32 lane, u32 *sKeys, u32 *sRows, u64 *sVals, u32 *sClaims) {\n"
       "  asm volatile(\"s_waitcnt lgkmcnt(0)\" ::: \"memory\");\n"
       "  if (lane < count) {\n"
       "    const u32 e = 3u * (first + lane);\n"
       "    insert(a, sKeys, sRows, sVals, sClaims, queue[e], queue[e + 1u], queue[e + 2u]);\n"
       "  }\n"
       "  asm volatile(\"s_waitcnt lgkmcnt(0)\" ::: \"memory\");\n"
       "}\n"
       "__device__ __forceinline__ void row_one(const Args &a, bool valid, u32 row, u32 h, u32 carried, u32 lane, u32 *sKeys, u32 *sRows, u64 *sVals, u32 *sClaims, u32 *queue, u32 &qn) {\n"
       "  const u32 b = h & (BUCKETS - 1u);\n"
       "  const uint4 k = *reinterpret_cast<const uint4 *>(sKeys + 4u * b);\n"
       "  const bool m0 = k.x == h, m1 = k.y == h, m2 = k.z == h, m3 = k.w == h;\n"
       "  const bool hit = valid && h != EMPTY && (m0 || m1 || m2 || m3);\n"
       "  if (hit) {\n"
       "    const u32 slot = 4u * b + (m0 ? 0u : m1 ? 1u : m2 ? 2u : 3u);\n"
       "    __hip_atomic_fetch_min(sRows + slot, row, __ATOMIC_RELAXED, __HIP_MEMORY_SCOPE_WORKGROUP);\n"
       "    agg(sVals + slot, widen(carried));\n"
       "  }\n"
       "  const bool pend = valid && !hit;\n"
       "  const u64 m = __ballot(pend);\n"
       "  if (m) {\n"
       "    if (pend) {\n"
       "      const u32 e = 3u * (qn + __builtin_amdgcn_mbcnt_hi((u32)(m >> 32), __builtin_amdgcn_mbcnt_lo((u32)m, 0u)));\n"
       "      queue[e] = row; queue[e + 1u] = h; queue[e + 2u] = carried;\n"
       "    }\n"
       "    qn += (u32)__popcll(m);\n"
       "    if (qn >= 64u) { qn -= 64u; drain(a, queue, qn, 64u, lane, sKeys, sRows, sVals, sClaims); }\n"
       "  }\n"
       "}\n"
       "extern \"C\" __global__ void __launch_bounds__(1024) hr_scan_rtc(Args a) {\n"
       "  __shared__ __attribute__((aligned(16))) u32 sKeys[SLOTS];\n"
       "  __shared__ u32 sRows[SLOTS];\n"
       "  __shared__ u64 sVals[SLOTS];\n"
       "  __shared__ u32 sQueue[16u * QCAP * 3u];\n"
       "  __shared__ u32 sPartCount[NP], sPartBase[NP];\n"
       "  __shared__ u32 sClaims;\n"
       "  const u32 tid = threadIdx.x, lane = tid & 63u, wave = tid >> 6;\n"
       "  for (u32 s = tid; s < SLOTS; s += 1024u) { sKeys[s] = EMPTY; sRows[s] = 0xFFFFFFFFu; sVals[s] = IDENT; }\n"
       "  for (u32 p = tid; p < NP; p += 1024u) sPartCount[p] = 0u;\n"
       "  if (tid == 0u) sClaims = 0u;\n"
       "  __syncthreads();\n"
       "  const u32 numTiles = ((u32)a.length + T - 1u) / T, G = gridDim.x;\n"
       "  u32 tile = blockIdx.x, qn = 0u;\n"
       "  u32 *queue = sQueue + wave * (QCAP * 3u);\n"
       "  Raw R0, R1;\n"
       "  load_tile(R0, a, tile * T + tid * 4u);\n"
       "  load_tile(R1, a, (tile + G) * T + tid * 4u);\n"
       "#define TILE_STEP(R)                                                                                   \\\n"
       "  {                                                                                                    \\\n"
       "    u32 i0 = tile * T + tid * 4u;                                                                      \\\n"
       "    const u32 next = tile + 2u * G;                                                                    \\\n"
       "    u32 hh[4], cv[4], cw[4], alive[4];                                                                 \\\n"
       "    eval4p(R, a, i0, hh, cv, cw, alive, next * T + tid * 4u);                                          \\\n"
       "    const u32 row0 = a.rowBase + i0;                                                                   \\\n"
       "    row_one(a, alive[0] != 0u, row0, hh[0], cv[0], lane, sKeys, sRows, sVals, &sClaims, queue, qn);    \\\n"
       "    row_one(a, alive[1] != 0u, row0 + 1u, hh[1], cv[1], lane, sKeys, sRows, sVals, &sClaims, queue, qn); \\\n"
       "    row_one(a, alive[2] != 0u, row0 + 2u, hh[2], cv[2], lane, sKeys, sRows, sVals, &sClaims, queue, qn); \\\n"
       "    row_one(a, alive[3] != 0u, row0 + 3u, hh[3], cv[3], lane, sKeys, sRows, sVals, &sClaims, queue, qn); \\\n"
       "    tile += G;                                                                                         \\\n"
       "  }\n"
       "  while (tile < numTiles) {\n"
       "    TILE_STEP(R0)\n"
       "    if (tile >= numTiles) break;\n"
       "    TILE_STEP(R1)\n"
       "  }\n"
       "  if (qn) drain(a, queue, 0u, qn, lane, sKeys, sRows, sVals, &sClaims);\n"
       "  __syncthreads();\n"
       "  u32 rank[SLOTS / 1024u];\n"
       "#pragma unroll\n"
       "  for (u32 k = 0u; k < SLOTS / 1024u; k++) {\n"
       "    const u32 key = sKeys[tid + k * 1024u];\n"
       "    rank[k] = 0u;\n"
       "    if (key != EMPTY) rank[k] = __hip_atomic_fetch_add(&sPartCount[PB ? key >> (32 - (PB ? PB : 1)) : 0u], 1u, __ATOMIC_RELAXED, __HIP_MEMORY_SCOPE_WORKGROUP);\n"
       "  }\n"
       "  __syncthreads();\n"
       "  for (u32 p = tid; p < NP; p += 1024u) { const u32 c = sPartCount[p]; if (c) sPartBase[p] = atomicAdd(a.cursorsA + p, c); }\n"
       "  __syncthreads();\n"
       "#pragma unroll\n"
       "  for (u32 k = 0u; k < SLOTS / 1024u; k++) {\n"
       "    const u32 s = tid + k * 1024u;\n"
       "    const u32 key = sKeys[s];\n"
       "    if (key == EMPTY) continue;\n"
       "    const u32 p = PB ? key >> (32 - (PB ? PB : 1)) : 0u;\n"
       "    const u64 at = (u64)sPartBase[p] + rank[k], v = sVals[s];\n"
       "    if (at < a.capA) a.recA[(u64)p * a.capA + at] = make_uint4(sRows[s], key, (u32)v, (u32)(v >> 32));\n"
       "    else *a.overflow = 1u;\n"
       "  }\n"
       "}\n";
}


struct SlotLayout {
  int nd = 0, valueBytes = 0;
  int width[kFusedDims] = {4, 4, 4, 4, 4, 4, 4, 4}, off[kFusedDims] = {};
  bool all4 = true, ok = true;
};
SlotLayout slot_layout(const int32_t *widths, int nd, int maxWidth) {
  SlotLayout L;
  L.nd = nd;
  int prev = maxWidth;
  for (int d = 0; d < nd && d < kFusedDims; d++) {
    const int w = widths[d];
    L.ok = L.ok && (w == 16 || w == 8 || w == 4 || w == 2 || w == 1) && w <= prev;
    prev = w;
    L.width[d] = w;
    L.off[d] = L.valueBytes;
    L.valueBytes += w;
    L.all4 = L.all4 && w == 4;
  }
  L.all4 = L.all4 && nd <= 4;
  return L;
}
std::vector<std::string> row_words(const SlotLayout &L, const std::function<std::string(int, int)> &val,
                                   const std::function<std::string(int)> &okb) {
  std::vector<std::string> w(static_cast<size_t>((L.valueBytes + L.nd + 3) / 4));
  auto add = [&](int byteOff, const std::string &e) {
    std::string &x = w[static_cast<size_t>(byteOff / 4)];
    const int sh = 8 * (byteOff % 4);
    const std::string term = sh ? "(" + e + " << " + std::to_string(sh) + ")" : e;
    x = x.empty() ? term : x + " | " + term;
  };
  for (int d = 0; d < L.nd; d++)
    for (int k = 0; 4 * k < L.width[d] || k == 0; k++) add(L.off[d] + 4 * k, val(d, k));
  for (int d = 0; d < L.nd; d++) add(L.valueBytes + d, okb(d));
  return w;
}
void gen_row_hash(std::ostringstream &o, const SlotLayout &L, const std::function<std::string(int)> &val,
                  const std::function<std::string(int)> &okb, const std::string &out, const char *indent) {
  const int total = L.valueBytes + L.nd, words = (total + 3) / 4;
  const std::vector<std::string> w = row_words(L, [&](int d, int) { return val(d); }, okb);
  o << indent << "{\n" << indent << "  u32 g = 0u;\n";
  for (int k = 0; k < total / 4; k++) o << indent << "  g = mix(g, " << w[static_cast<size_t>(k)] << ");\n";
  if (total % 4) o << indent << "  { u32 k = (" << w[static_cast<size_t>(words - 1)] << ") * 0xcc9e2d51u; k = rotl(k, 15) * 0x1b873593u; g ^= k; }\n";
  o << indent << "  g ^= " << total << "u; g ^= g >> 16; g *= 0x85ebca6bu; g ^= g >> 13; g *= 0xc2b2ae35u; g ^= g >> 16;\n"
    << indent << "  " << out << " = g;\n" << indent << "}\n";
}
void gen_row_hash64(std::ostringstream &o, const SlotLayout &L, const std::function<std::string(int, int)> &val,
                    const std::function<std::string(int)> &okb, const std::string &out, const char *indent) {
  const int total = L.valueBytes + L.nd, words = (total + 3) / 4;
  const std::vector<std::string> w = row_words(L, val, okb);
  auto lane64 = [&](int firstWord) {
    if (firstWord >= words) return std::string();
    std::string e = "(u64)(" + w[static_cast<size_t>(firstWord)] + ")";
    if (firstWord + 1 < words) e += " | ((u64)(" + w[static_cast<size_t>(firstWord + 1)] + ") << 32)";
    return e;
  };
  const std::string in = indent;
  o << in << "{\n" << in << "  u64 g1 = 0ull, g2 = 0ull, q1, q2;\n";
  const int blocks = total / 16;
  for (int b = 0; b < blocks; b++) {
    o << in << "  q1 = " << lane64(4 * b) << "; q2 = " << lane64(4 * b + 2) << ";\n"
      << in << "  q1 *= MC1; q1 = rotl64(q1, 31); q1 *= MC2; g1 ^= q1; g1 = rotl64(g1, 27); g1 += g2; g1 = g1 * 5ull + 0x52dce729ull;\n"
      << in << "  q2 *= MC2; q2 = rotl64(q2, 33); q2 *= MC1; g2 ^= q2; g2 = rotl64(g2, 31); g2 += g1; g2 = g2 * 5ull + 0x38495ab5ull;\n";
  }
  const int tail = total % 16;
  if (tail > 8) o << in << "  q2 = " << lane64(4 * blocks + 2) << "; q2 *= MC2; q2 = rotl64(q2, 33); q2 *= MC1; g2 ^= q2;\n";
  if (tail > 0) o << in << "  q1 = " << lane64(4 * blocks) << "; q1 *= MC1; q1 = rotl64(q1, 31); q1 *= MC2; g1 ^= q1;\n";
  o << in << "  g1 ^= " << total << "ull; g2 ^= " << total << "ull; g1 += g2; g2 += g1;\n"
    << in << "  g1 = fmix64(g1); g2 = fmix64(g2); g1 += g2;\n"
    << in << "  " << out << " = g1;\n" << in << "}\n";
}
const char *kPrelude64 =
    "#define MC1 0x87c37b91114253d5ull\n#define MC2 0x4cf5ad432745937full\n"
    "__device__ __forceinline__ u64 rotl64(u64 x, int r) { return (x << r) | (x >> (64 - r)); }\n"
    "__device__ __forceinline__ u64 fmix64(u64 k) { k ^= k >> 33; k *= 0xff51afd7ed558ccdull; k ^= k >> 33; k *= 0xc4ceb9fe1a85ec53ull; k ^= k >> 33; return k; }\n";
const char *width_mask(int w) { return w == 4 ? "" : w == 2 ? " & 0xFFFFu" : " & 0xFFu"; }
std::string slot_load(const SlotLayout &L, int d, const char *base, const char *cap, const std::string &row) {
  const std::string at = std::string(base) + " + (u64)" + std::to_string(L.off[d]) + " * " + cap + " + " + std::to_string(L.width[d]) + "ull * " + row;
  return L.width[d] == 4 ? "*reinterpret_cast<const u32 *>(" + at + ")" : L.width[d] == 2 ? "(u32)*reinterpret_cast<const u16 *>(" + at + ")" : "(u32)*(" + at + ")";
}
std::string slot_store(const SlotLayout &L, int d, const char *base, const char *cap, const std::string &row, const std::string &v) {
  const std::string at = std::string(base) + " + (u64)" + std::to_string(L.off[d]) + " * " + cap + " + " + std::to_string(L.width[d]) + "ull * " + row;
  return L.width[d] == 4 ? "*reinterpret_cast<u32 *>(" + at + ") = " + v + ";" : L.width[d] == 2 ? "*reinterpret_cast<u16 *>(" + at + ") = (u16)(" + v + ");" : "*(" + at + ") = (u8)(" + v + ");";
}
std::string column_elem(int step, bool sgn, const std::string &base, const std::string &idx) {
  if (step == 4) return base + "[" + idx + "]";
  if (step == 2) return sgn ? "(u32)(i32)reinterpret_cast<const short *>(" + base + ")[" + idx + "]" : "(u32)reinterpret_cast<const u16 *>(" + base + ")[" + idx + "]";
  return sgn ? "(u32)(i32)reinterpret_cast<const signed char *>(" + base + ")[" + idx + "]" : "(u32)reinterpret_cast<const u8 *>(" + base + ")[" + idx + "]";
}
bool column_signed(const RtcSpec &s, int c) {
  for (int d = 0; d < s.nd; d++)
    if (s.dims[d].col == c) return s.dims[d].akind == K_I32;
  if (!s.constMeasure && s.measure.col == c) return s.measure.akind == K_I32;
  for (int k = 0; k < s.numFilters; k++)
    if (s.filters[k].col == c) return s.filters[k].akind == K_I32;
  return false;
}

std::string generate(const RtcSpec &s) {
  const int nd = s.nd, partBits = s.partBits, kind = s.kind;
  const uint32_t nullMask = s.nullMask;
  if (nd < 1 || nd > kFusedDims || s.numCols < 0 || s.numCols > kFusedCols || s.numFilters < 0 || s.numFilters > kFusedFilters) return "";
  if (kind == RTC_SCAN_COMPACT && partBits < 3) return "";
  const SlotLayout SL = slot_layout(s.dimWidth, nd, 4);
  if (!SL.ok) return "";
  for (int c = 0; c < s.numCols; c++) {
    const int st = s.step[c];
    if (!(st == 4 || st == 2 || st == 1)) return "";
  }
  std::ostringstream o;
  const int nc = s.numCols;
  const bool sort64 = kind == RTC_SCAN_SORT64;
  const bool constMeasure = sort64 && s.constMeasure;
  if (s.constMeasure && !sort64) return "";
  const bool avg = s.measureAvg != 0;
  if (avg && (!sort64 || constMeasure || s.measureWidth != 8 || s.identity != 0)) return "";
  const int firstFilterCol = constMeasure ? nd : nd + 1;
  o << kPrelude << (sort64 ? kPrelude64 : "") << args_text()
    << "#define NC " << nc << "\n#define ND " << nd << "\n#define PB " << partBits << "\n#define NP " << (1 << partBits) << "\n"
       "struct Raw { u32 v[NC][4]; u32 win[NC]; };\n";
  o << "__device__ __forceinline__ u32 clampi(const Args &a, u32 i0) { const u32 lim = a.length >= 4 ? (u32)a.length - 4u : 0u; return i0 < lim ? i0 : lim; }\n";
  for (int c = 0; c < nc; c++) {
    o << "__device__ __forceinline__ void load_col" << c << "(Raw &r, const Args &a, u32 i0c) {\n";
    const int step = s.step[c];
    if (step != 4) {
      const bool sgn = column_signed(s, c);
      const char *ptr = step == 2 ? "reinterpret_cast<const u16 *>(a.vals[" : "reinterpret_cast<const u8 *>(a.vals[";
      if (step == 2) {
        o << "  const U2 t = __builtin_nontemporal_load(reinterpret_cast<const U2a *>(" << ptr << c << "]) + i0c));\n  const u32 t0 = t.x, t1 = t.y;\n";
        if (sgn) o << "  r.v[" << c << "][0] = (u32)((i32)(t0 << 16) >> 16); r.v[" << c << "][1] = (u32)((i32)t0 >> 16); r.v[" << c << "][2] = (u32)((i32)(t1 << 16) >> 16); r.v[" << c << "][3] = (u32)((i32)t1 >> 16);\n";
        else o << "  r.v[" << c << "][0] = t0 & 0xFFFFu; r.v[" << c << "][1] = t0 >> 16; r.v[" << c << "][2] = t1 & 0xFFFFu; r.v[" << c << "][3] = t1 >> 16;\n";
      } else {
        o << "  const u32 t0 = __builtin_nontemporal_load(reinterpret_cast<const U1a *>(" << ptr << c << "]) + i0c));\n";
        if (sgn) o << "  r.v[" << c << "][0] = (u32)((i32)(t0 << 24) >> 24); r.v[" << c << "][1] = (u32)((i32)(t0 << 16) >> 24); r.v[" << c << "][2] = (u32)((i32)(t0 << 8) >> 24); r.v[" << c << "][3] = (u32)((i32)t0 >> 24);\n";
        else o << "  r.v[" << c << "][0] = t0 & 0xFFu; r.v[" << c << "][1] = (t0 >> 8) & 0xFFu; r.v[" << c << "][2] = (t0 >> 16) & 0xFFu; r.v[" << c << "][3] = t0 >> 24;\n";
      }
    } else {
      o << "  const U4 t = __builtin_nontemporal_load(reinterpret_cast<const U4a *>(a.vals[" << c << "] + i0c)); r.v[" << c << "][0] = t.x; r.v[" << c
        << "][1] = t.y; r.v[" << c << "][2] = t.z; r.v[" << c << "][3] = t.w;\n";
    }
    if (nullMask & (1u << c))
      o << "  r.win[" << c << "] = reinterpret_cast<const PU16 *>(a.nulls[" << c << "] + ((i0c + a.bitOff[" << c << "]) >> 3))->v;\n";
    else
      o << "  r.win[" << c << "] = 0xFFFFu;\n";
    o << "}\n";
  }
  o << "__device__ __forceinline__ void load_tile(Raw &r, const Args &a, u32 i0) {\n  const u32 i0c = clampi(a, i0);\n";
  for (int c = 0; c < nc; c++) o << "  load_col" << c << "(r, a, i0c);\n";
  o << "}\n";
  {
    const std::string bar = "  __builtin_amdgcn_sched_barrier(0);\n";
    auto prefetch = [&](int c) { o << bar << "  load_col" << c << "(r, a, i0nc);\n" << bar; };
    o << "__device__ __forceinline__ void eval4p(Raw &r, const Args &a, u32 &i0, u32 (&hh)[4], u32 (&cv)[4], u32 (&cw)[4], u32 (&alive)[4], u32 i0n) {\n"
         "  u32 okc[NC];\n"
         "  cw[0] = cw[1] = cw[2] = cw[3] = 0u;\n"
         "  const u32 i0c = clampi(a, i0), i0nc = clampi(a, i0n);\n"
         "  const u32 sh = i0 - i0c < 4u ? i0 - i0c : 4u;\n"
         "  i0 = i0c;\n";
    for (int c = 0; c < nc; c++) {
      if (nullMask & (1u << c)) o << "  okc[" << c << "] = (r.win[" << c << "] >> ((i0c + a.bitOff[" << c << "]) & 7u)) & 0xFu;\n";
      else o << "  okc[" << c << "] = 0xFu;\n";
    }
    o << "#pragma unroll\n"
         "  for (int j = 0; j < 4; j++) {\n"
         "    u32 keep = ((u32)j >= sh && (int)(i0c + j) < a.length) ? 1u : 0u;\n";
    for (int k = 0; k < s.numFilters; k++) {
      const RtcExpr &e = s.filters[k];
      if (e.col < 0 || e.col >= nc) return "";
      o << "    {\n      const u32 v = r.v[" << e.col << "][j]; const u32 okb = (okc[" << e.col << "] >> j) & 1u;\n";
      if (!gen_compare(e, o, "v", "okb", "keep", const_name(const_slot_filter(k)))) return "";
      o << "    }\n";
    }
    o << "    alive[j] = keep;\n  }\n";
    for (int c = firstFilterCol; c < nc; c++) prefetch(c);
    if (constMeasure) {
      o << "  cv[0] = cv[1] = cv[2] = cv[3] = " << const_name(const_slot_measure()) << ";\n";
    } else {
      const RtcExpr &e = s.measure;
      if (e.col != nd) return "";
      o << "#pragma unroll\n  for (int j = 0; j < 4; j++) {\n"
           "    const u32 v = r.v[" << nd << "][j]; const u32 okb = (okc[" << nd << "] >> j) & 1u; u32 x;\n";
      if (!gen_value(e, o, "v", "okb", "x", const_name(const_slot_measure()), sort64)) return "";
      if (avg) {
        const int rk = e.rk;
        if (!(rk == K_F32 || rk == K_I32 || rk == K_U32) || !(s.measureDtype == Float64 || s.measureDtype == Int64)) return "";
        const bool f64 = s.measureDtype == Float64;
        const char *cvt = rk == K_F32 ? (f64 ? "x" : "__float_as_uint((float)(i64)__uint_as_float(x))")
                          : rk == K_I32 ? (f64 ? "__float_as_uint((float)(double)(i32)x)" : "__float_as_uint((float)(i64)(i32)x)")
                                        : (f64 ? "__float_as_uint((float)(double)x)" : "__float_as_uint((float)(i64)x)");
        o << "    cv[j] = okb ? " << cvt << " : 0u;\n"
             "    alive[j] |= (alive[j] & (okb ^ 1u)) << 31;\n";
      } else if (s.measureWidth == 8) {
        if (s.identity != 0) return "";
        o << "    cv[j] = okb ? x : 0u;\n";
      } else {
        const int target = s.measureDtype == Int32 ? K_I32 : s.measureDtype == Uint32 ? K_U32 : K_F32;
        if (!plain_store(e.rk, target)) return "";
        o << "    cv[j] = okb ? x : " << hex(static_cast<uint32_t>(s.identity)) << ";\n";
      }
      o << "  }\n";
      prefetch(nd);
    }
    if (SL.all4 && !sort64) {
    o << "  u32 h[4] = {0u, 0u, 0u, 0u}, okbytes[4] = {0u, 0u, 0u, 0u};\n";
    for (int d = 0; d < nd; d++) {
      const RtcExpr &e = s.dims[d];
      if (e.col != d || !plain_store(e.rk, e.outKind)) return "";
      o << "#pragma unroll\n  for (int j = 0; j < 4; j++) {\n"
           "    const u32 v = r.v[" << d << "][j]; const u32 okb = (okc[" << d << "] >> j) & 1u; u32 x;\n";
      if (!gen_value(e, o, "v", "okb", "x", const_name(const_slot_dim(d)))) return "";
      o << "    h[j] = mix(h[j], x); okbytes[j] |= okb << " << 8 * d << ";\n  }\n";
      prefetch(d);
    }
    o << "#pragma unroll\n  for (int j = 0; j < 4; j++) {\n    u32 g = h[j];\n";
    if (nd == 4) o << "    g = mix(g, okbytes[j]);\n";
    else o << "    { u32 k = okbytes[j] * 0xcc9e2d51u; k = rotl(k, 15) * 0x1b873593u; g ^= k; }\n";
    o << "    g ^= " << 5 * nd << "u; g ^= g >> 16; g *= 0x85ebca6bu; g ^= g >> 13; g *= 0xc2b2ae35u; g ^= g >> 16;\n"
         "    hh[j] = g;\n  }\n}\n";
    } else {
      for (int d = 0; d < nd; d++) o << "  u32 xv" << d << "[4], xo" << d << "[4];\n";
      for (int d = 0; d < nd; d++) {
        const RtcExpr &e = s.dims[d];
        if (e.col != d || !plain_store(e.rk, e.outKind) || (SL.width[d] != 4 && !int_kind(e.rk))) return "";
        o << "#pragma unroll\n  for (int j = 0; j < 4; j++) {\n"
             "    const u32 v = r.v[" << d << "][j]; const u32 okb = (okc[" << d << "] >> j) & 1u; u32 x;\n";
        if (!gen_value(e, o, "v", "okb", "x", const_name(const_slot_dim(d)))) return "";
        o << "    xv" << d << "[j] = x" << width_mask(SL.width[d]) << "; xo" << d << "[j] = okb;\n  }\n";
        prefetch(d);
      }
      o << "#pragma unroll\n  for (int j = 0; j < 4; j++) {\n";
      if (sort64) {
        o << "    u64 h64;\n";
        gen_row_hash64(o, SL, [](int d, int) { return "xv" + std::to_string(d) + "[j]"; }, [](int d) { return "xo" + std::to_string(d) + "[j]"; },
                       "h64", "    ");
        o << "    hh[j] = (u32)(h64 >> 32); cw[j] = (u32)h64;\n";
      } else {
        gen_row_hash(o, SL, [](int d) { return "xv" + std::to_string(d) + "[j]"; }, [](int d) { return "xo" + std::to_string(d) + "[j]"; },
                     "hh[j]", "    ");
      }
      o << "  }\n}\n";
    }
  }
  if (kind == RTC_SCAN_TABLE) {
    if (!gen_widen(o, s) || !gen_agg(o, s)) return "";
    kernel_body_table(o);
  } else if (kind == RTC_SCAN_COMPACT) {
    kernel_body_compact(o, s);
  } else {
    Lines16 rec{sort64 ? "cw[j]" : "0u"};
    if (avg) rec.row = "(a.rowBase + i0 + j) | (alive[j] & 0x80000000u)";
    kernel_body_lines16(o, s, rec);
  }
  return o.str();
}

std::string generate_vector(const RtcSpec &s) {
  const int nd = s.nd, vw = s.vectorVW, partBits = s.partBits;
  const bool hll = s.kind == RTC_HLL_SCAN, sort64 = hll || s.kind == RTC_SORT_VECTOR_SCAN;
  if (nd < 1 || nd > (sort64 ? kFusedDims : kGenericFusedDims) || (vw != 4 && vw != 8) || (sort64 && vw != 4)) return "";
  if (hll && (partBits < 1 || partBits > 9)) return "";
  const SlotLayout SL = slot_layout(s.dimWidth, nd, sort64 ? 16 : 4);
  if (!SL.ok || (!sort64 && !SL.all4)) return "";
  const int *width = SL.width;
  int wb[kFusedDims] = {};
  bool narrow = false, wide = false;
  int nw = 0;
  for (int d = 0; d < nd; d++) {
    narrow = narrow || width[d] != 4;
    wide = wide || width[d] > 4;
    wb[d] = nw;
    nw += width[d] > 4 ? width[d] / 4 : 1;
  }
  if (wide && SL.valueBytes > kSortVectorValueBytes) return "";
  std::ostringstream o;
  const int mq = vw / 4;
  o << kPrelude << (sort64 ? kPrelude64 : "") << args_text()
    << "#define ND " << nd << "\n#define MQ " << mq << "\n#define PB " << partBits << "\n#define NP " << (1 << partBits) << "\n";
  if (wide) o << "#define NW " << nw << "\nstruct Raw { u32 v[NW][4]; u32 ok[ND]; u32 m[MQ * 4]; };\n";
  else o << "struct Raw { u32 v[ND][4]; u32 ok[ND]; u32 m[MQ * 4]; };\n";
  o << "__device__ __forceinline__ void load_full(Raw &r, const Args &a, u32 i0) {\n";
  if (narrow) {
    for (int d = 0; d < nd; d++) {
      const int v = wb[d];
      if (width[d] > 4) {
        const int q = width[d] / 4;
        o << "  {\n    const PU32x4 *p = reinterpret_cast<const PU32x4 *>(reinterpret_cast<const u8 *>(a.vals[" << d << "]) + " << width[d] << "ull * i0);\n";
        for (int k = 0; k < q; k++) o << "    const PU32x4 t" << k << " = p[" << k << "];\n";
        o << "   ";
        for (int k = 0; k < q; k++)
          for (int e = 0; e < 4; e++) o << " r.v[" << v + (4 * k + e) % q << "][" << (4 * k + e) / q << "] = t" << k << ".v[" << e << "];";
        o << "\n  }\n";
      } else if (width[d] == 4)
        o << "  { const PU32x4 t = *reinterpret_cast<const PU32x4 *>(a.vals[" << d << "] + i0); r.v[" << v << "][0] = t.v[0]; r.v[" << v
          << "][1] = t.v[1]; r.v[" << v << "][2] = t.v[2]; r.v[" << v << "][3] = t.v[3]; }\n";
      else if (width[d] == 2)
        o << "  { const PU32x2 t = *reinterpret_cast<const PU32x2 *>(reinterpret_cast<const u8 *>(a.vals[" << d << "]) + 2ull * i0); r.v[" << v
          << "][0] = t.v[0] & 0xFFFFu; r.v[" << v << "][1] = t.v[0] >> 16; r.v[" << v << "][2] = t.v[1] & 0xFFFFu; r.v[" << v << "][3] = t.v[1] >> 16; }\n";
      else
        o << "  { const u32 t = reinterpret_cast<const PU32 *>(reinterpret_cast<const u8 *>(a.vals[" << d << "]) + i0)->v; r.v[" << v
          << "][0] = t & 0xFFu; r.v[" << v << "][1] = (t >> 8) & 0xFFu; r.v[" << v << "][2] = (t >> 16) & 0xFFu; r.v[" << v << "][3] = t >> 24; }\n";
      o << "  r.ok[" << d << "] = reinterpret_cast<const PU32 *>(a.nulls[" << d << "] + i0)->v;\n";
    }
  } else {
  o << "#pragma unroll\n"
       "  for (int d = 0; d < ND; d++) {\n"
       "    const PU32x4 t = *reinterpret_cast<const PU32x4 *>(a.vals[d] + i0);\n"
       "    r.v[d][0] = t.v[0]; r.v[d][1] = t.v[1]; r.v[d][2] = t.v[2]; r.v[d][3] = t.v[3];\n"
       "    r.ok[d] = reinterpret_cast<const PU32 *>(a.nulls[d] + i0)->v;\n"
       "  }\n";
  }
  o << ""
       "#pragma unroll\n"
       "  for (int q = 0; q < MQ; q++) {\n"
       "    const PU32x4 t = *reinterpret_cast<const PU32x4 *>(a.vals[ND] + (u64)i0 * MQ + 4 * q);\n"
       "    r.m[4 * q] = t.v[0]; r.m[4 * q + 1] = t.v[1]; r.m[4 * q + 2] = t.v[2]; r.m[4 * q + 3] = t.v[3];\n"
       "  }\n"
       "}\n"
       "__device__ __forceinline__ void load_tail(Raw &r, const Args &a, u32 i0) {\n";
  if (narrow) {
    for (int d = 0; d < nd; d++) {
      const char *elem = width[d] == 4 ? "a.vals[%d][i0 + j]" : width[d] == 2 ? "(u32)reinterpret_cast<const u16 *>(a.vals[%d])[i0 + j]" : "(u32)reinterpret_cast<const u8 *>(a.vals[%d])[i0 + j]";
      char buf[128];
      snprintf(buf, sizeof(buf), elem, d);
      o << "  r.ok[" << d << "] = 0u;\n"
           "  for (int j = 0; j < 4; j++) {\n"
           "    const bool in = (int)(i0 + j) < a.length;\n";
      if (width[d] > 4)
        for (int k = 0; k < width[d] / 4; k++)
          o << "    r.v[" << wb[d] + k << "][j] = in ? a.vals[" << d << "][" << width[d] / 4 << "ull * (i0 + j) + " << k << "] : 0u;\n";
      else
        o << "    r.v[" << wb[d] << "][j] = in ? " << buf << " : 0u;\n";
      o << "    r.ok[" << d << "] |= in ? (u32)a.nulls[" << d << "][i0 + j] << (8 * j) : 0u;\n"
           "  }\n";
    }
  } else {
  o << "#pragma unroll\n"
       "  for (int d = 0; d < ND; d++) {\n"
       "    r.ok[d] = 0u;\n"
       "    for (int j = 0; j < 4; j++) {\n"
       "      const bool in = (int)(i0 + j) < a.length;\n"
       "      r.v[d][j] = in ? a.vals[d][i0 + j] : 0u;\n"
       "      r.ok[d] |= in ? (u32)a.nulls[d][i0 + j] << (8 * j) : 0u;\n"
       "    }\n"
       "  }\n";
  }
  o << "  for (int j = 0; j < 4; j++)\n"
       "    for (int q = 0; q < MQ; q++) r.m[j * MQ + q] = (int)(i0 + j) < a.length ? a.vals[ND][(u64)(i0 + j) * MQ + q] : 0u;\n"
       "}\n"
       "__device__ __forceinline__ void eval4(const Raw &r, const Args &a, u32 i0, u32 (&hh)[4], u32 (&cv)[4], u32 (&cw)[4], u32 (&alive)[4]) {\n"
       "#pragma unroll\n"
       "  for (int j = 0; j < 4; j++) {\n"
       "    alive[j] = (int)(i0 + j) < a.length ? 1u : 0u;\n";
  if (sort64) {
    o << "    u64 h64;\n";
    gen_row_hash64(o, SL, [&](int d, int k) { return "r.v[" + std::to_string(wb[d] + k) + "][j]"; },
                   [](int d) { return "((r.ok[" + std::to_string(d) + "] >> (8 * j)) & 0xFFu)"; }, "h64", "    ");
    if (hll) o << "    h64 = (h64 & 0xFFFFFFFFFFFF0000ull) | (u64)(r.m[j] & 0x3FFFu);\n";
    o << "    hh[j] = (u32)(h64 >> 32);\n"
         "    cv[j] = r.m[j];\n"
         "    cw[j] = (u32)h64;\n"
         "  }\n"
         "}\n";
  } else {
  o << "    u32 h = 0u, okbytes = 0u;\n"
       "#pragma unroll\n"
       "    for (int d = 0; d < ND; d++) { h = mix(h, r.v[d][j]); okbytes |= ((r.ok[d] >> (8 * j)) & 0xFFu) << (8 * d); }\n";
  if (nd == 4) o << "    h = mix(h, okbytes);\n";
  else o << "    { u32 k = okbytes * 0xcc9e2d51u; k = rotl(k, 15) * 0x1b873593u; h ^= k; }\n";
  o << "    h ^= " << 5 * nd << "u; h ^= h >> 16; h *= 0x85ebca6bu; h ^= h >> 13; h *= 0xc2b2ae35u; h ^= h >> 16;\n"
       "    hh[j] = h;\n"
       "    cv[j] = r.m[j * MQ];\n"
       "    cw[j] = MQ == 2 ? r.m[j * MQ + MQ - 1] : 0u;\n"
       "  }\n"
       "}\n";
  }
  o << "__device__ __forceinline__ void load_tile(Raw &r, const Args &a, u32 i0) { if ((int)(i0 + 3u) < a.length) load_full(r, a, i0); else if ((int)i0 < a.length) load_tail(r, a, i0); }\n"
       "__device__ __forceinline__ void eval4p(Raw &r, const Args &a, u32 &i0, u32 (&hh)[4], u32 (&cv)[4], u32 (&cw)[4], u32 (&alive)[4], u32 i0n) {\n"
       "  eval4(r, a, i0, hh, cv, cw, alive);\n"
       "  load_tile(r, a, i0n);\n"
       "}\n";
  Lines16 rec{"cw[j]"};
  if (hll)
    rec.part = "(((hh[j] ^ (cw[j] * 0x9E3779B1u)) * 0x85EBCA6Bu) >> (32 - PB))";
  else if (sort64)
    rec.part = "(a.pad ? (((hh[j] >> a.chunkTiles) ^ ((((hh[j] >> a.chunkTiles) >> PB) * 0x9E3779B1u) >> 23)) & (NP - 1u)) "
               ": (PB ? hh[j] >> (32 - (PB ? PB : 1)) : 0u))";
  kernel_body_lines16(o, s, rec);
  return o.str();
}

std::string generate_merge(const RtcSpec &s) {
  const int nd = s.nd, partBits = s.partBits, image = s.image, vectorVW = s.kind == RTC_VECTOR_MERGE ? s.vectorVW : 0;
  const bool compact = s.compact != 0, regionA = s.regionA != 0;
  if (nd < 1 || nd > kFusedDims) return "";
  if (image && vectorVW) return "";
  if (compact && (vectorVW || partBits < 3)) return "";
  if (partBits < 2) return "";
  const SlotLayout SL = slot_layout(s.dimWidth, nd, 4);
  if (!SL.ok || (vectorVW && !SL.all4)) return "";
  std::ostringstream o;
  o << kPrelude
    << "struct MArgs { const u32 *vals[" << kFusedCols << "]; const u8 *nulls[" << kFusedCols << "]; const u32 *recB; const u32 *countsB;\n"
       "  const u32 *prevRanges; const u8 *prevDims; const u8 *prevValues; u8 *dimOut; u8 *outValues; u32 *outCount; u32 *outRanges;\n"
       "  u64 prevCapacity, outCapacity; u32 bitOff[" << kFusedCols << "]; u32 capB, streams, prevSize, chunkRows; u64 *phases; u32 k[" << kNumConsts << "]; u32 pad;\n"
       "  const uint4 *recA; const u32 *cursorsA; u64 capA;\n"
       "  const uint4 *imgIn; uint4 *imgOut; const u32 *imgInCount; u32 *imgOutCount; u32 *hostOut; u32 knownOut, pad2; };\n"
       "#define FINISH() { __syncthreads(); if (threadIdx.x == 0u && a.hostOut) { __threadfence(); \\\n"
       "  if (atomicAdd(a.outCount + 4, 1u) == gridDim.x - 1u) { __threadfence(); const volatile u32 *oc = a.outCount; \\\n"
       "    a.hostOut[0] = oc[0]; a.hostOut[1] = oc[1]; a.hostOut[2] = oc[2]; a.hostOut[3] = oc[3]; } } }\n"
       "#define ND " << nd << "\n#define VB " << SL.valueBytes << "\n#define PB " << partBits << "\n#define NP " << (1 << partBits) << "\n"
       "#define SLOTS " << hr::kSlots << "\n#define LIMIT " << hr::kMergeLimit << "u\n#define RANGEWORDS " << hr::kRangeWords
    << "\n#define MAXRANGES " << hr::kMaxRanges << "u\n"
       "#define HMASK ((1u << (32 - PB)) - 1u)\n#define OCC 0x40000000u\n#define NEWG 0x80000000u\n";
  gen_widen(o, s);
  if (!gen_agg(o, s)) return "";
  if (s.phases)
    o << "#define STAMP(k) if (threadIdx.x == 0u) a.phases[(u64)blockIdx.x * 8u + (k)] = __builtin_amdgcn_s_memrealtime();\n";
  else
    o << "#define STAMP(k)\n";
  o << "#define BUCKETS (SLOTS / 4)\n"
       "struct Probe { u32 b, slot; bool done, isNew; };\n"
       "__device__ __forceinline__ void probe_round(u32 *sKeys, u32 *sClaimed, u32 *sOverflow, Probe &q, u32 want, u32 claimKey) {\n"
       "  const uint4 k = *reinterpret_cast<const uint4 *>(sKeys + 4u * q.b);\n"
       "  const bool e0 = k.x == 0u, e1 = k.y == 0u, e2 = k.z == 0u, e3 = k.w == 0u;\n"
       "  const bool m0 = (k.x & ~NEWG) == want, m1 = (k.y & ~NEWG) == want, m2 = (k.z & ~NEWG) == want, m3 = (k.w & ~NEWG) == want;\n"
       "  const bool anyM = m0 | m1 | m2 | m3, anyE = e0 | e1 | e2 | e3;\n"
       "  const u32 mi = m0 ? 0u : m1 ? 1u : m2 ? 2u : 3u, ei = e0 ? 0u : e1 ? 1u : e2 ? 2u : 3u;\n"
       "  const u32 mk = m0 ? k.x : m1 ? k.y : m2 ? k.z : k.w;\n"
       "  const bool active = !q.done, hit = active & anyM;\n"
       "  q.slot = hit ? 4u * q.b + mi : q.slot;\n"
       "  q.isNew = hit ? (mk & NEWG) != 0u : q.isNew;\n"
       "  bool claimed = false;\n"
       "  if (active & !anyM & anyE) {\n"
       "    u32 expected = 0u;\n"
       "    if (__hip_atomic_compare_exchange_strong(sKeys + 4u * q.b + ei, &expected, claimKey, __ATOMIC_RELAXED, __ATOMIC_RELAXED, __HIP_MEMORY_SCOPE_WORKGROUP)) {\n"
       "      if (__hip_atomic_fetch_add(sClaimed, 1u, __ATOMIC_RELAXED, __HIP_MEMORY_SCOPE_WORKGROUP) >= LIMIT)\n"
       "        __hip_atomic_store(sOverflow, 1u, __ATOMIC_RELAXED, __HIP_MEMORY_SCOPE_WORKGROUP);\n"
       "      q.slot = 4u * q.b + ei; q.isNew = true; claimed = true;\n"
       "    }\n"
       "  }\n"
       "  q.b = (active & !anyM & !anyE) ? (q.b + 1u) & (BUCKETS - 1u) : q.b;\n"
       "  q.done = q.done | hit | claimed;\n"
       "}\n"
       "__device__ __forceinline__ void insert(u32 *sKeys, u32 *sRows, u64 *sVals, u32 *sClaimed, u32 *sOverflow, u32 row, u32 h, u64 value, bool batch) {\n"
       "  const u32 want = (h & HMASK) | OCC;\n"
       "  Probe q; q.b = h & (BUCKETS - 1u); q.slot = 0u; q.done = false; q.isNew = false;\n"
       "  for (u32 tries = 0u; tries < 4u * BUCKETS && !q.done; tries++) probe_round(sKeys, sClaimed, sOverflow, q, want, batch ? want | NEWG : want);\n"
       "  if (q.done) {\n"
       "    if (q.isNew || !batch) __hip_atomic_fetch_min(sRows + q.slot, row, __ATOMIC_RELAXED, __HIP_MEMORY_SCOPE_WORKGROUP);\n"
       "    agg(sVals + q.slot, value);\n"
       "  } else {\n"
       "    __hip_atomic_store(sOverflow, 1u, __ATOMIC_RELAXED, __HIP_MEMORY_SCOPE_WORKGROUP);\n"
       "  }\n"
       "}\n";
  if (vectorVW == 8)
    o << "#define QCAP 96u\n#define QW 4u\n#define QDRAIN 32u\n#define VALB(z, w) ((((u64)(w)) << 32) | (z))\n";
  else if (vectorVW == 4)
    o << "#define QCAP 128u\n#define QW 3u\n#define QDRAIN 64u\n#define VALB(z, w) ((u64)(z))\n";
  else
    o << "#define QCAP 128u\n#define QW 3u\n#define QDRAIN 64u\n#define VALB(z, w) widen(z)\n";
  o << "struct Seg { const uint4 *ptr; u32 n, rem, rb; };\n"
       "struct Stage { uint4 r[4]; u32 n[4], rem[4], rb[4]; };\n"
       "__device__ __forceinline__ void drain(u32 *queue, u32 first, u32 count, u32 lane, u32 *sKeys, u32 *sRows, u64 *sVals, u32 *sClaimed, u32 *sOverflow) {\n"
       "  asm volatile(\"s_waitcnt lgkmcnt(0)\" ::: \"memory\");\n"
       "  if (lane < count) {\n"
       "    const u32 e = QW * (first + lane);\n"
       "    const u32 row = queue[e], h = queue[e + 1u], z = queue[e + 2u], w = QW == 4u ? queue[e + QW - 1u] : 0u;\n"
       "    insert(sKeys, sRows, sVals, sClaimed, sOverflow, row, h, VALB(z, w), true);\n"
       "  }\n"
       "  asm volatile(\"s_waitcnt lgkmcnt(0)\" ::: \"memory\");\n"
       "}\n"
       "__device__ __forceinline__ void consume_one(bool valid, u32 row, u32 h, u32 z, u32 w, u32 lane, u32 *sKeys, u32 *sRows, u64 *sVals, u32 *sClaimed, u32 *sOverflow, u32 *queue, u32 &qn) {\n"
       "  const u32 b = h & (BUCKETS - 1u), want = (h & HMASK) | OCC;\n"
       "  const uint4 k = *reinterpret_cast<const uint4 *>(sKeys + 4u * b);\n"
       "  const bool m0 = (k.x & ~NEWG) == want, m1 = (k.y & ~NEWG) == want, m2 = (k.z & ~NEWG) == want, m3 = (k.w & ~NEWG) == want;\n"
       "  const bool hit = valid && (m0 || m1 || m2 || m3);\n"
       "  if (hit) {\n"
       "    const u32 mi = m0 ? 0u : m1 ? 1u : m2 ? 2u : 3u;\n"
       "    const u32 mk = m0 ? k.x : m1 ? k.y : m2 ? k.z : k.w;\n"
       "    if (mk & NEWG) __hip_atomic_fetch_min(sRows + 4u * b + mi, row, __ATOMIC_RELAXED, __HIP_MEMORY_SCOPE_WORKGROUP);\n"
       "    agg(sVals + 4u * b + mi, VALB(z, w));\n"
       "  }\n"
       "  const bool pend = valid && !hit;\n"
       "  const u64 m = __ballot(pend);\n"
       "  if (m) {\n"
       "    if (pend) {\n"
       "      const u32 e = QW * (qn + __builtin_amdgcn_mbcnt_hi((u32)(m >> 32), __builtin_amdgcn_mbcnt_lo((u32)m, 0u)));\n"
       "      queue[e] = row; queue[e + 1u] = h; queue[e + 2u] = z;\n"
       "      if (QW == 4u) queue[e + QW - 1u] = w;\n"
       "    }\n"
       "    qn += (u32)__popcll(m);\n"
       "    if (qn >= QDRAIN) { const u32 take = qn < 64u ? qn : 64u; qn -= take; drain(queue, qn, take, lane, sKeys, sRows, sVals, sClaimed, sOverflow); }\n"
       "  }\n"
       "}\n";
  if (compact)
    o << "__device__ __forceinline__ void consume(const Stage &s, u32 lane, u32 p, u32 *sKeys, u32 *sRows, u64 *sVals, u32 *sClaimed, u32 *sOverflow, u32 *queue, u32 &qn) {\n"
         "  const u32 pos = 2u * (lane & 3u);\n"
         "  const u32 recBase = (lane >> 3) * 14u + 7u * ((lane >> 2) & 1u);\n"
         "#pragma unroll\n"
         "  for (int k = 0; k < 4; k++) {\n"
         "    const u64 hdr = ((u64)(u32)__builtin_amdgcn_mov_dpp((int)s.r[k].y, 0x00, 0xF, 0xF, true) << 32) | (u32)__builtin_amdgcn_mov_dpp((int)s.r[k].x, 0x00, 0xF, 0xF, true);\n"
         "#pragma unroll\n"
         "    for (u32 j = 0u; j < 2u; j++) {\n"
         "      const u32 ph = pos + j;\n"
         "      const u32 k7 = ph ? ph - 1u : 0u;\n"
         "      const bool valid = lane < s.n[k] && ph != 0u && recBase + k7 < s.rem[k];\n"
         "      const u32 z = j ? s.r[k].z : s.r[k].x, hw = j ? s.r[k].w : s.r[k].y;\n"
         "      const u32 lo9 = (u32)(hdr >> (9u * k7)) & 511u;\n"
         "      const u32 h = (p << (32 - PB)) | (hw >> PB);\n"
         "      const u32 row = s.rb[k] + (((hw & ((1u << PB) - 1u)) << 9) | lo9);\n"
         "      consume_one(valid, row, h, z, 0u, lane, sKeys, sRows, sVals, sClaimed, sOverflow, queue, qn);\n"
         "    }\n"
         "  }\n"
         "}\n";
  else
    o << "__device__ __forceinline__ void consume(const Stage &s, u32 lane, u32 p, u32 *sKeys, u32 *sRows, u64 *sVals, u32 *sClaimed, u32 *sOverflow, u32 *queue, u32 &qn) {\n"
         "#pragma unroll\n"
         "  for (int k = 0; k < 4; k++) {\n"
         "    const bool valid = lane < s.n[k] && s.r[k].x != 0xFFFFFFFFu;\n"
         "    consume_one(valid, s.r[k].x, s.r[k].y, s.r[k].z, s.r[k].w, lane, sKeys, sRows, sVals, sClaimed, sOverflow, queue, qn);\n"
         "  }\n"
         "}\n";
  if (!vectorVW) o << "__device__ __forceinline__ void eval_row(const MArgs &a, u32 row, u32 (&bits)[ND], u32 (&ok)[ND]) {\n";
  for (int d = 0; d < nd && !vectorVW; d++) {
    const RtcExpr &e = s.dims[d];
    const int c = e.col;
    if (c < 0 || c >= kFusedCols || !plain_store(e.rk, e.outKind) || (SL.width[d] != 4 && !int_kind(e.rk))) return "";
    o << "  {\n    const u32 v = " << column_elem(s.step[c], e.akind == K_I32, "a.vals[" + std::to_string(c) + "]", "row") << ";\n";
    if (s.nullMask & (1u << c)) o << "    const u32 bit = row + a.bitOff[" << c << "]; const u32 okb = (a.nulls[" << c << "][bit >> 3] >> (bit & 7u)) & 1u;\n";
    else o << "    const u32 okb = 1u;\n";
    o << "    u32 x;\n";
    if (!gen_value(e, o, "v", "okb", "x", const_name(const_slot_dim(d)))) return "";
    o << "    bits[" << d << "] = x; ok[" << d << "] = okb;\n  }\n";
  }
  if (!vectorVW) o << "}\n";
  const bool wide = s.aggWidth == 8;
  o << "extern \"C\" __global__ void __launch_bounds__(1024) hr_merge_rtc(MArgs a) {\n"
       "  __shared__ __attribute__((aligned(16))) u32 sKeys[SLOTS];\n"
       "  __shared__ __attribute__((aligned(16))) u32 sRows[SLOTS];\n"
       "  __shared__ __attribute__((aligned(16))) u64 sVals[SLOTS];\n"
       "  __shared__ u32 sRunCount[256];\n"
       "  __shared__ u32 sQueue[16u * QCAP * QW];\n"
       "  __shared__ u32 sClaimed, sOverflow, sCount, sBase, sEmit;\n"
       "  const u32 tid = threadIdx.x, lane = tid & 63u, wave = tid >> 6, p = blockIdx.x;\n"
       "  STAMP(0)\n";
  if (image == 2)
    o << "  {\n"
         "    const uint4 *img = a.imgIn + (u64)p * SLOTS;\n"
         "    for (u32 i = tid; i < SLOTS / 4u; i += 1024u) {\n"
         "      reinterpret_cast<uint4 *>(sKeys)[i] = img[i];\n"
         "      reinterpret_cast<uint4 *>(sRows)[i] = img[SLOTS / 4u + i];\n"
         "    }\n"
         "    for (u32 i = tid; i < SLOTS / 2u; i += 1024u) reinterpret_cast<uint4 *>(sVals)[i] = img[SLOTS / 2u + i];\n"
         "    if (tid == 0u) { sClaimed = a.imgInCount[p]; sOverflow = 0u; sCount = 0u; sEmit = 0u; }\n"
         "  }\n";
  else
    o << "  for (u32 s = tid; s < SLOTS; s += 1024u) { sKeys[s] = 0u; sRows[s] = 0xFFFFFFFFu; sVals[s] = IDENT; }\n"
         "  if (tid == 0u) { sClaimed = 0u; sOverflow = 0u; sCount = 0u; sEmit = 0u; }\n";
  o << "  const u32 G = a.streams;\n"
       "  if (tid < G) sRunCount[tid] = a.countsB[(u64)tid * NP + p];\n"
       "  const u32 *ranges = a.prevRanges ? a.prevRanges + (u64)p * RANGEWORDS : nullptr;\n"
       "  u32 nRanges = ranges ? ranges[0] : 0u;\n"
       "  if (nRanges > MAXRANGES) { if (tid == 0u) a.outCount[2] = 1u; nRanges = 0u; }\n"
       "  __syncthreads();\n"
       "  STAMP(1)\n"
       "  {\n"
       "    const u8 *nullsIn = a.prevDims + (u64)VB * a.prevCapacity;\n"
       "    for (u32 r = 0u; r < nRanges; r++) {\n"
       "      const u32 start = ranges[1u + 2u * r], cnt = ranges[2u + 2u * r];\n"
       "      for (u32 i0 = 0u; i0 < cnt; i0 += 4096u) {\n"
       "        u32 hh[4], rr[4]; u64 vv[4]; bool okk[4];\n"
       "#pragma unroll\n"
       "        for (int k = 0; k < 4; k++) {\n"
       "          const u32 i = i0 + (u32)k * 1024u + tid;\n"
       "          okk[k] = i < cnt;\n"
       "          const u32 row = start + (okk[k] ? i : 0u);\n"
       "          rr[k] = row;\n"
       "          okk[k] = okk[k] && row < a.prevSize;\n"
       "          const u32 safe = row < a.prevSize ? row : 0u;\n"
       "          u32 h = 0u;\n";
  if (SL.all4) {
    o << "          u32 okbytes = 0u;\n"
         "#pragma unroll\n"
         "          for (int d = 0; d < ND; d++) {\n"
         "            h = mix(h, *reinterpret_cast<const u32 *>(a.prevDims + (u64)(4 * d) * a.prevCapacity + 4ull * safe));\n"
         "            okbytes |= (u32)nullsIn[(u64)d * a.prevCapacity + safe] << (8 * d);\n"
         "          }\n";
    if (nd == 4) o << "          h = mix(h, okbytes);\n";
    else o << "          { u32 kk = okbytes * 0xcc9e2d51u; kk = rotl(kk, 15) * 0x1b873593u; h ^= kk; }\n";
    o << "          h ^= " << 5 * nd << "u; h ^= h >> 16; h *= 0x85ebca6bu; h ^= h >> 13; h *= 0xc2b2ae35u; h ^= h >> 16;\n";
  } else {
    for (int d = 0; d < nd; d++)
      o << "          const u32 pv" << d << " = " << slot_load(SL, d, "a.prevDims", "a.prevCapacity", "safe") << ", po" << d
        << " = (u32)nullsIn[(u64)" << d << " * a.prevCapacity + safe];\n";
    gen_row_hash(o, SL, [](int d) { return "pv" + std::to_string(d); }, [](int d) { return "po" + std::to_string(d); }, "h", "          ");
  }
  o <<
       "          hh[k] = h;\n"
    << (wide ? "          vv[k] = reinterpret_cast<const u64 *>(a.prevValues)[safe];\n"
             : "          vv[k] = reinterpret_cast<const u32 *>(a.prevValues)[safe];\n")
    << "        }\n"
       "#pragma unroll\n"
       "        for (int k = 0; k < 4; k++) {\n"
       "          const u32 i = i0 + (u32)k * 1024u + tid;\n"
       "          if (i >= cnt) continue;\n"
       "          if (!okk[k] || (PB && (hh[k] >> (32 - (PB ? PB : 1))) != p)) { a.outCount[2] = 1u; continue; }\n"
       "          insert(sKeys, sRows, sVals, &sClaimed, &sOverflow, rr[k], hh[k], vv[k], false);\n"
       "        }\n"
       "      }\n"
       "    }\n"
       "  }\n"
       "  __syncthreads();\n"
       "  STAMP(2)\n";
  if (regionA)
    o << "  {\n"
         "    const u32 cur = a.cursorsA[p];\n"
         "    const u32 nA = cur < a.capA ? cur : (u32)a.capA;\n"
         "    const uint4 *recs = a.recA + (u64)p * a.capA;\n"
         "    for (u32 i = tid; i < nA; i += 1024u) {\n"
         "      const uint4 r = recs[i];\n"
         "      insert(sKeys, sRows, sVals, &sClaimed, &sOverflow, r.x, r.y, ((u64)r.w << 32) | r.z, true);\n"
         "    }\n"
         "  }\n"
         "  __syncthreads();\n";
  o << "  u32 maxRun = 0u;\n"
       "  for (u32 g = lane; g < G; g += 64u) { const u32 c = sRunCount[g]; maxRun = c > maxRun ? c : maxRun; }\n"
       "#pragma unroll\n"
       "  for (int off = 32; off > 0; off >>= 1) { const u32 t = (u32)__shfl_xor((int)maxRun, off); maxRun = t > maxRun ? t : maxRun; }\n"
       "  const u32 LPR = (maxRun + " << (compact ? "13u) / 14u" : "7u) / 8u") << ";\n"
       "  if (G > 0u && LPR <= 4u && LPR <= a.capB" << (compact ? "" : " / 8u") << ") {\n"
       "    u32 qn = 0u;\n"
       "    u32 *queue = sQueue + wave * (QCAP * QW);\n"
       "    const u32 units = G * 8u * LPR;\n"
       "    for (u32 base = 0u; base < units; base += 4096u) {\n"
       "      Stage s;\n"
       "#pragma unroll\n"
       "      for (int k = 0; k < 4; k++) {\n"
       "        const u32 u = base + (u32)k * 1024u + tid;\n"
       "        const bool in = u < units;\n"
       "        const u32 ul = in ? u >> 3 : 0u, g = ul / LPR, l = ul - g * LPR, cnt = in ? sRunCount[g] : 0u;\n"
    << (compact ? "        const u32 here = cnt > l * 14u ? cnt - l * 14u : 0u;\n"
                  "        s.r[k] = reinterpret_cast<const uint4 *>(a.recB)[(((u64)g * NP + p) * a.capB + l) * 8u + (u & 7u)];\n"
                  "        s.n[k] = here ? 64u : 0u; s.rem[k] = (lane >> 3) * 14u + here; s.rb[k] = a.prevSize + g * a.chunkRows;\n"
                : "        const u32 here = cnt > l * 8u ? cnt - l * 8u : 0u;\n"
                  "        s.r[k] = reinterpret_cast<const uint4 *>(a.recB)[((u64)g * NP + p) * a.capB + l * 8u + (u & 7u)];\n"
                  "        s.n[k] = (u & 7u) < here ? 64u : 0u; s.rem[k] = 0u; s.rb[k] = 0u;\n")
    << "      }\n"
       "      consume(s, lane, p, sKeys, sRows, sVals, &sClaimed, &sOverflow, queue, qn);\n"
       "    }\n"
       "    while (qn) { const u32 take = qn < 64u ? qn : 64u; qn -= take; drain(queue, qn, take, lane, sKeys, sRows, sVals, &sClaimed, &sOverflow); }\n"
       "  } else\n"
       "  if (G > 0u) {\n"
       "    const uint4 *dummy = reinterpret_cast<const uint4 *>(a.recB);\n"
       "    u32 j = 0u, off = 0u, qn = 0u;\n"
       "    u32 *queue = sQueue + wave * (QCAP * QW);\n"
       "    const u32 myRuns = (G + 15u - wave) / 16u;\n"
       "    const u32 myCnt = lane < myRuns ? sRunCount[wave + 16u * lane] : 0u;\n";
  if (compact)
    o << "    auto next = [&]() -> Seg {\n"
         "      Seg c{dummy, 0u, 0u, 0u};\n"
         "      while (j < myRuns) {\n"
         "        const u32 cnt = (u32)__builtin_amdgcn_readlane((int)myCnt, (int)j);\n"
         "        const u32 units = ((cnt + 13u) / 14u) * 8u;\n"
         "        if (off < units) {\n"
         "          c.ptr = reinterpret_cast<const uint4 *>(a.recB) + ((u64)(wave + 16u * j) * NP + p) * a.capB * 8u + off;\n"
         "          c.n = units - off < 64u ? units - off : 64u;\n"
         "          c.rem = cnt - (off >> 3) * 14u;\n"
         "          c.rb = a.prevSize + (wave + 16u * j) * a.chunkRows;\n"
         "          off += 64u;\n"
         "          break;\n"
         "        }\n"
         "        j++; off = 0u;\n"
         "      }\n"
         "      return c;\n"
         "    };\n";
  else
    o << "    auto next = [&]() -> Seg {\n"
         "      Seg c{dummy, 0u, 0u, 0u};\n"
         "      while (j < myRuns) {\n"
         "        const u32 cnt = (u32)__builtin_amdgcn_readlane((int)myCnt, (int)j);\n"
         "        if (off < cnt) {\n"
         "          c.ptr = reinterpret_cast<const uint4 *>(a.recB) + ((u64)(wave + 16u * j) * NP + p) * a.capB + off;\n"
         "          c.n = cnt - off < 64u ? cnt - off : 64u;\n"
         "          off += 64u;\n"
         "          break;\n"
         "        }\n"
         "        j++; off = 0u;\n"
         "      }\n"
         "      return c;\n"
         "    };\n";
  o << "    auto load = [&](Stage &s) {\n"
       "#pragma unroll\n"
       "      for (int k = 0; k < 4; k++) {\n"
       "        const Seg c = next();\n"
       "        s.n[k] = c.n; s.rem[k] = c.rem; s.rb[k] = c.rb;\n"
       "        s.r[k] = c.ptr[lane < c.n ? lane : (c.n ? c.n - 1u : 0u)];\n"
       "      }\n"
       "    };\n"
       "    Stage s0, s1, s2;\n"
       "    load(s0);\n"
       "    load(s1);\n"
       "    for (;;) {\n"
       "      load(s2);\n"
       "      if (!s0.n[0]) break;\n"
       "      consume(s0, lane, p, sKeys, sRows, sVals, &sClaimed, &sOverflow, queue, qn);\n"
       "      load(s0);\n"
       "      if (!s1.n[0]) break;\n"
       "      consume(s1, lane, p, sKeys, sRows, sVals, &sClaimed, &sOverflow, queue, qn);\n"
       "      load(s1);\n"
       "      if (!s2.n[0]) break;\n"
       "      consume(s2, lane, p, sKeys, sRows, sVals, &sClaimed, &sOverflow, queue, qn);\n"
       "    }\n"
       "    while (qn) { const u32 take = qn < 64u ? qn : 64u; qn -= take; drain(queue, qn, take, lane, sKeys, sRows, sVals, &sClaimed, &sOverflow); }\n"
       "  }\n"
       "  __syncthreads();\n"
       "  STAMP(3)\n"
       "  if (sOverflow) { if (tid == 0u) a.outCount[3] = 1u; FINISH() return; }\n";
  const char *kStoreKeysPos =
      "    for (u32 i = tid; i < SLOTS / 4u; i += 1024u) {\n"
      "      img[i] = reinterpret_cast<const uint4 *>(sKeys)[i];\n"
      "      img[SLOTS / 4u + i] = reinterpret_cast<const uint4 *>(sRows)[i];\n"
      "    }\n";
  const char *kStoreVals = "    for (u32 i = tid; i < SLOTS / 2u; i += 1024u) img[SLOTS / 2u + i] = reinterpret_cast<const uint4 *>(sVals)[i];\n";
  if (image == 2) {
    o << "  u32 mineNew = 0u;\n"
         "#pragma unroll\n"
         "  for (int k = 0; k < SLOTS / 1024; k++) mineNew += (sKeys[tid + (u32)k * 1024u] & NEWG) != 0u;\n"
         "  if (mineNew) __hip_atomic_fetch_add(&sCount, mineNew, __ATOMIC_RELAXED, __HIP_MEMORY_SCOPE_WORKGROUP);\n"
         "  __syncthreads();\n"
         "  const u32 totalNew = sCount;\n"
         "  if (tid == 0u) sBase = a.prevSize + (totalNew ? atomicAdd(a.outCount, totalNew) : 0u);\n"
         "  __syncthreads();\n"
         "  STAMP(4)\n"
         "  u8 *nullsOut = a.dimOut + (u64)VB * a.outCapacity;\n"
         "  if (totalNew) {\n"
         "#pragma unroll\n"
         "    for (int half = 0; half < 2; half++) {\n"
         "      u32 dv[4][ND], nv[4][ND], at[4]; bool has[4];\n"
         "#pragma unroll\n"
         "      for (int kk = 0; kk < 4; kk++) {\n"
         "        const u32 s = tid + (u32)(half * 4 + kk) * 1024u;\n"
         "        has[kk] = (sKeys[s] & NEWG) != 0u;\n"
         "        const u64 m = __ballot(has[kk]);\n"
         "        u32 waveBase = 0u;\n"
         "        if (lane == 0u && m) waveBase = __hip_atomic_fetch_add(&sEmit, (u32)__popcll(m), __ATOMIC_RELAXED, __HIP_MEMORY_SCOPE_WORKGROUP);\n"
         "        waveBase = (u32)__builtin_amdgcn_readfirstlane((int)waveBase);\n"
         "        at[kk] = sBase + waveBase + __builtin_amdgcn_mbcnt_hi((u32)(m >> 32), __builtin_amdgcn_mbcnt_lo((u32)m, 0u));\n"
         "        if (has[kk]) eval_row(a, sRows[s] - a.prevSize, dv[kk], nv[kk]);\n"
         "      }\n"
         "#pragma unroll\n"
         "      for (int kk = 0; kk < 4; kk++) {\n"
         "        if (!has[kk]) continue;\n"
         "        const u32 s = tid + (u32)(half * 4 + kk) * 1024u;\n";
    for (int d = 0; d < nd; d++)
      o << "        " << slot_store(SL, d, "a.dimOut", "a.outCapacity", "at[kk]", "dv[kk][" + std::to_string(d) + "]") << " nullsOut[(u64)" << d
        << " * a.outCapacity + at[kk]] = (u8)nv[kk][" << d << "];\n";
    o << "        sRows[s] = at[kk];\n"
         "        sKeys[s] &= ~NEWG;\n"
         "      }\n"
         "    }\n"
         "  }\n"
         "  __syncthreads();\n"
         "  {\n"
         "    uint4 *img = a.imgOut + (u64)p * SLOTS;\n"
         "    const u32 newCount = a.imgInCount[p] + totalNew;\n"
         "    if (a.imgOutCount[p] != newCount) {\n"
      << kStoreKeysPos
      << "    }\n"
      << kStoreVals
      << "    __syncthreads();\n"
         "    if (tid == 0u) a.imgOutCount[p] = newCount;\n"
         "  }\n"
         "  if (a.knownOut < a.prevSize) {\n"
         "    const u8 *nullsIn = a.prevDims + (u64)VB * a.prevCapacity;\n"
         "    const u32 n = a.prevSize - a.knownOut, share = (n + NP - 1u) / NP;\n"
         "    const u32 lo = a.knownOut + p * share, hi = lo + share < a.prevSize ? lo + share : a.prevSize;\n"
         "    for (u32 r = lo + tid; r < hi; r += 1024u) {\n";
    for (int d = 0; d < nd; d++)
      o << "      " << slot_store(SL, d, "a.dimOut", "a.outCapacity", "r", slot_load(SL, d, "a.prevDims", "a.prevCapacity", "r")) << " nullsOut[(u64)" << d
        << " * a.outCapacity + r] = nullsIn[(u64)" << d << " * a.prevCapacity + r];\n";
    o << "    }\n"
         "  }\n"
         "  STAMP(5)\n"
         "  FINISH()\n"
         "}\n";
    return o.str();
  }
  o <<
       "  u32 mineCount = 0u;\n"
       "#pragma unroll\n"
       "  for (int k = 0; k < SLOTS / 1024; k++) mineCount += sKeys[tid + (u32)k * 1024u] != 0u;\n"
       "  if (mineCount) __hip_atomic_fetch_add(&sCount, mineCount, __ATOMIC_RELAXED, __HIP_MEMORY_SCOPE_WORKGROUP);\n"
       "  __syncthreads();\n"
       "  const u32 total = sCount;\n"
       "  if (tid == 0u) {\n"
       "    u32 base = 0u;\n"
       "    if (total) base = atomicAdd(a.outCount, total);\n"
       "    sBase = base;\n"
       "    if (a.outRanges) { u32 *o = a.outRanges + (u64)p * RANGEWORDS; o[0] = total ? 1u : 0u; o[1] = base; o[2] = total; }\n"
       "  }\n"
       "  __syncthreads();\n"
       "  STAMP(4)\n"
    << (image == 1 ? "" : "  if (!total) { FINISH() return; }\n")
    << "  const u8 *nullsIn = a.prevDims + (u64)VB * a.prevCapacity;\n"
       "  u8 *nullsOut = a.dimOut + (u64)VB * a.outCapacity;\n"
       "#pragma unroll\n"
       "  for (int half = 0; half < 2; half++) {\n"
       "    u32 dv[4][ND], nv[4][ND], at[4]; bool has[4];\n"
       "#pragma unroll\n"
       "    for (int kk = 0; kk < 4; kk++) {\n"
       "      const u32 s = tid + (u32)(half * 4 + kk) * 1024u;\n"
       "      has[kk] = sKeys[s] != 0u;\n"
       "      const u64 m = __ballot(has[kk]);\n"
       "      u32 waveBase = 0u;\n"
       "      if (lane == 0u && m) waveBase = __hip_atomic_fetch_add(&sEmit, (u32)__popcll(m), __ATOMIC_RELAXED, __HIP_MEMORY_SCOPE_WORKGROUP);\n"
       "      waveBase = (u32)__builtin_amdgcn_readfirstlane((int)waveBase);\n"
       "      at[kk] = sBase + waveBase + __builtin_amdgcn_mbcnt_hi((u32)(m >> 32), __builtin_amdgcn_mbcnt_lo((u32)m, 0u));\n"
       "      if (!has[kk]) continue;\n"
       "      const u32 row = sRows[s];\n"
    << (vectorVW ? "" : "      if (row >= a.prevSize) { eval_row(a, row - a.prevSize, dv[kk], nv[kk]); continue; }\n");
  if (SL.all4) {
    o << "#pragma unroll\n"
         "      for (int d = 0; d < ND; d++) {\n"
         "        dv[kk][d] = *reinterpret_cast<const u32 *>(a.prevDims + (u64)(4 * d) * a.prevCapacity + 4ull * row);\n"
         "        nv[kk][d] = nullsIn[(u64)d * a.prevCapacity + row];\n"
         "      }\n";
  } else {
    for (int d = 0; d < nd; d++)
      o << "      dv[kk][" << d << "] = " << slot_load(SL, d, "a.prevDims", "a.prevCapacity", "row") << "; nv[kk][" << d << "] = nullsIn[(u64)" << d
        << " * a.prevCapacity + row];\n";
  }
  o << "    }\n"
       "#pragma unroll\n"
       "    for (int kk = 0; kk < 4; kk++) {\n"
       "      if (!has[kk]) continue;\n"
       "      const u32 s = tid + (u32)(half * 4 + kk) * 1024u;\n";
  if (SL.all4) {
    o << "#pragma unroll\n"
         "      for (int d = 0; d < ND; d++) {\n"
         "        *reinterpret_cast<u32 *>(a.dimOut + (u64)(4 * d) * a.outCapacity + 4ull * at[kk]) = dv[kk][d];\n"
         "        nullsOut[(u64)d * a.outCapacity + at[kk]] = (u8)nv[kk][d];\n"
         "      }\n";
  } else {
    for (int d = 0; d < nd; d++)
      o << "      " << slot_store(SL, d, "a.dimOut", "a.outCapacity", "at[kk]", "dv[kk][" + std::to_string(d) + "]") << " nullsOut[(u64)" << d
        << " * a.outCapacity + at[kk]] = (u8)nv[kk][" << d << "];\n";
  }
  o << (wide ? "      reinterpret_cast<u64 *>(a.outValues)[at[kk]] = sVals[s];\n"
             : "      reinterpret_cast<u32 *>(a.outValues)[at[kk]] = (u32)sVals[s];\n")
    << (image == 1 ? "      sRows[s] = at[kk];\n      sKeys[s] &= ~NEWG;\n" : "")
    << "    }\n"
       "  }\n";
  if (image == 1)
    o << "  __syncthreads();\n"
         "  {\n"
         "    uint4 *img = a.imgOut + (u64)p * SLOTS;\n"
      << kStoreKeysPos << kStoreVals
      << "    if (tid == 0u) a.imgOutCount[p] = total;\n"
         "  }\n";
  o <<
       "  STAMP(5)\n"
       "  FINISH()\n"
       "}\n";
  return o.str();
}

enum ExprRole { FILTER, DIMENSION, MEASURE };
RtcExpr spec_expr(const FusedExpr &e, ExprRole role) {
  RtcExpr x{};
  x.col = e.col; x.akind = e.f.akind; x.arity = e.f.arity; x.I = e.f.I;
  if (role != FILTER) x.rk = e.f.rk;
  if (role == DIMENSION) x.outKind = e.outKind;
  if (e.f.arity != 2) return x;
  x.functor = e.f.functor; x.bok = e.f.bok != 0;
  if (role == FILTER) return x;
  x.bkind = e.f.bkind; x.divLike = e.f.divLike != 0;
  if (x.divLike) x.bbits = e.f.bbits;
  return x;
}
RtcSpec spec_of(RtcKind kind, int nd, int partBits, bool stamps = true) {
  RtcSpec s{};
  s.kind = kind; s.nd = nd; s.partBits = partBits;
  s.phases = stamps && phases_enabled();
  return s;
}
void spec_column(RtcSpec &s, const FusedPlanD &plan, int c) {
  s.step[c] = fused_col_step(plan, c);
  if (plan.cols[c].nulls) s.nullMask |= 1u << c;
}
void spec_dims(RtcSpec &s, const FusedPlanD &plan) {
  for (int d = 0; d < s.nd && d < kFusedDims; d++) {
    s.dimWidth[d] = fused_dim_width(plan, d);
    s.dims[d] = spec_expr(plan.dims[d], DIMENSION);
  }
}
void spec_agg(RtcSpec &s, const AggSpec &a, const hr::Widen &w) {
  s.aggVtype = a.vtype; s.aggIdentity = a.identity;
  if (a.vtype == V_U32 || a.vtype == V_I32) s.aggOp = a.op;
  s.widenMode = w.mode;
  if (w.mode) { s.widenRk = w.rk; s.widenDtype = w.dtype; }
}
RtcSpec spec_plan_scan(RtcKind kind, const FusedPlanD &plan, int nd, int partBits) {
  RtcSpec s = spec_of(kind, nd, partBits, kind != RTC_SCAN_TABLE);
  s.numCols = plan.numCols; s.numFilters = plan.numFilters;
  for (int c = 0; c < plan.numCols && c < kFusedCols; c++) spec_column(s, plan, c);
  for (int k = 0; k < plan.numFilters && k < kFusedFilters; k++) s.filters[k] = spec_expr(plan.filters[k], FILTER);
  spec_dims(s, plan);
  s.measureAvg = plan.measureAvg != 0;
  s.constMeasure = plan.measure.col < 0;
  if (!s.constMeasure) {
    s.measure = spec_expr(plan.measure, MEASURE);
    s.measureWidth = plan.measureWidth; s.identity = plan.identity;
    if (s.measureAvg || plan.measureWidth != 8) s.measureDtype = plan.measureDtype;
  }
  return s;
}
RtcSpec spec_vector(RtcKind kind, int nd, const int *widths, int vw, int partBits) {
  RtcSpec s = spec_of(kind, nd, partBits);
  for (int d = 0; d < nd && d < kFusedDims; d++) s.dimWidth[d] = widths ? widths[d] : 4;
  s.vectorVW = vw;
  return s;
}

}

const char *rtc_entry_name(int32_t kind) {
  switch (kind) {
    case RTC_SCAN_SORT64: case RTC_SORT_VECTOR_SCAN: return "sr_scan_rtc";
    case RTC_HLL_SCAN: return "hll_scan_rtc";
    case RTC_MERGE: case RTC_VECTOR_MERGE: return "hr_merge_rtc";
    default: return "hr_scan_rtc";
  }
}

RtcSpec rtc_spec_scan(const FusedPlanD &plan, int nd, int partBits, bool compact) {
  return spec_plan_scan(compact ? RTC_SCAN_COMPACT : RTC_SCAN_LINES16, plan, nd, partBits);
}
RtcSpec rtc_spec_sort_scan(const FusedPlanD &plan, int nd, int partBits) { return spec_plan_scan(RTC_SCAN_SORT64, plan, nd, partBits); }
RtcSpec rtc_spec_table_scan(const FusedPlanD &plan, int nd, int partBits, const AggSpec &a, const hr::Widen &w) {
  RtcSpec s = spec_plan_scan(RTC_SCAN_TABLE, plan, nd, partBits);
  spec_agg(s, a, w);
  return s;
}
RtcSpec rtc_spec_vector_scan(int nd, int vw, int partBits) { return spec_vector(RTC_VECTOR_SCAN, nd, nullptr, vw, partBits); }
RtcSpec rtc_spec_sort_vector_scan(int nd, const int *widths, int partBits) { return spec_vector(RTC_SORT_VECTOR_SCAN, nd, widths, 4, partBits); }
RtcSpec rtc_spec_hll_scan(int nd, const int *widths, int partBits) { return spec_vector(RTC_HLL_SCAN, nd, widths, 4, partBits); }
RtcSpec rtc_spec_merge(const FusedPlanD &plan, int nd, int partBits, const AggSpec &a, const hr::Widen &w, bool compact, bool regionA,
                       int image) {
  RtcSpec s = spec_of(RTC_MERGE, nd, partBits);
  spec_dims(s, plan);
  for (int d = 0; d < nd && d < kFusedDims; d++)
    if (plan.dims[d].col >= 0 && plan.dims[d].col < kFusedCols) spec_column(s, plan, plan.dims[d].col);
  spec_agg(s, a, w);
  s.aggWidth = a.width;
  s.compact = compact; s.regionA = regionA; s.image = image;
  return s;
}
RtcSpec rtc_spec_vector_merge(int nd, int vw, int partBits, const AggSpec &a) {
  RtcSpec s = spec_vector(RTC_VECTOR_MERGE, nd, nullptr, vw, partBits);
  spec_agg(s, a, hr::Widen{0, 0, 0});
  s.aggWidth = a.width;
  return s;
}

std::string rtc_source(const RtcSpec &s) {
  switch (s.kind) {
    case RTC_SCAN_LINES16: case RTC_SCAN_COMPACT: case RTC_SCAN_TABLE: case RTC_SCAN_SORT64: return generate(s);
    case RTC_VECTOR_SCAN: case RTC_SORT_VECTOR_SCAN: case RTC_HLL_SCAN: return generate_vector(s);
    case RTC_MERGE: case RTC_VECTOR_MERGE: return generate_merge(s);
    default: return "";
  }
}

}
```

### aresdb_amd/csrc/algo/hr_rtc_gen.hpp

```cpp
#pragma once

#include <cstdint>
#include <cstring>
#include <string>
#include <type_traits>

#include "aggregate.hpp"
#include "hash_reduce_lds.hpp"

namespace ares {
namespace hr { struct Widen; }

constexpr int kNumConsts = kFusedFilters + kFusedDims + 1;
constexpr int const_slot_filter(int f) { return f; }
constexpr int const_slot_dim(int d) { return kFusedFilters + d; }
constexpr int const_slot_measure() { return kFusedFilters + kFusedDims; }

enum RtcKind : int32_t {
  RTC_SCAN_LINES16 = 1, RTC_SCAN_COMPACT, RTC_SCAN_TABLE, RTC_SCAN_SORT64, RTC_VECTOR_SCAN, RTC_SORT_VECTOR_SCAN, RTC_HLL_SCAN,
  RTC_MERGE, RTC_VECTOR_MERGE
};
const char *rtc_entry_name(int32_t kind);

struct RtcExpr {
  int32_t col, outKind, akind, arity, functor, I, rk, bkind;
  uint32_t bbits, bok;
  int32_t divLike;
};

struct RtcSpec {
  uint64_t identity;
  uint64_t aggIdentity;
  int32_t kind, nd, partBits, numCols, numFilters;
  uint32_t nullMask;
  int32_t step[kFusedCols];
  int32_t dimWidth[kFusedDims];
  RtcExpr filters[kFusedFilters], dims[kFusedDims], measure;
  int32_t measureDtype, measureWidth, measureAvg;
  int32_t aggVtype, aggOp, aggWidth;
  int32_t widenMode, widenRk, widenDtype;
  int32_t compact, regionA, image;
  int32_t vectorVW;
  int32_t phases;
  int32_t constMeasure;
};
static_assert(std::has_unique_object_representations<RtcSpec>::value, "compared and hashed as bytes: no padding");
inline bool operator==(const RtcSpec &a, const RtcSpec &b) { return memcmp(&a, &b, sizeof(a)) == 0; }
inline bool operator!=(const RtcSpec &a, const RtcSpec &b) { return !(a == b); }
bool phases_enabled();

RtcSpec rtc_spec_scan(const FusedPlanD &plan, int nd, int partBits, bool compact);
RtcSpec rtc_spec_sort_scan(const FusedPlanD &plan, int nd, int partBits);
RtcSpec rtc_spec_table_scan(const FusedPlanD &plan, int nd, int partBits, const AggSpec &a, const hr::Widen &w);
RtcSpec rtc_spec_vector_scan(int nd, int vw, int partBits);
RtcSpec rtc_spec_sort_vector_scan(int nd, const int *widths, int partBits);
RtcSpec rtc_spec_hll_scan(int nd, const int *widths, int partBits);
RtcSpec rtc_spec_merge(const FusedPlanD &plan, int nd, int partBits, const AggSpec &a, const hr::Widen &w, bool compact = false,
                       bool regionA = false, int image = 0);
RtcSpec rtc_spec_vector_merge(int nd, int vw, int partBits, const AggSpec &a);

std::string rtc_source(const RtcSpec &s);

}
```

Measured before the change: 91.78 billion rows/s.

## Add block-record scan mode that locates new groups' rows by re-evaluating 512-row blocks

Adds a new 'block' record format for steady-state batches (image mode 2, few new groups). Each record stores a 512-row block index instead of the exact row id, so the scan can pack more per line. The merge finds a new group's source row by re-running filter and hash over that block with a wave ballot. It falls back to the compact path if a partition has too many new groups or the search fails, which can cost a rescan, and it adds a new RTC kernel pair to compile.

```diff
diff --git a/aresdb_amd/csrc/algo/hash_reduce_lds.hip b/aresdb_amd/csrc/algo/hash_reduce_lds.hip
--- a/aresdb_amd/csrc/algo/hash_reduce_lds.hip
+++ b/aresdb_amd/csrc/algo/hash_reduce_lds.hip
@@ -103,6 +103,7 @@
   std::shared_ptr<uint8_t> image;
   uint64_t lineage = 0;
   uint64_t gen = 0, parentGen = 0;
+  int appended = 0;
   bool lazyValues = false;
 };
 std::mutex g_groupedMutex;
@@ -289,6 +290,13 @@
   return on.get();
 }
 
+constexpr int kBlockMaxNewPerPartition = 64;
+constexpr int kBlockLineRecords = 16;
+bool block_records_enabled() {
+  static EnvSwitch<bool> on("ARES_HR_BLOCK_RECORDS", [](const char *e) { return !(e && e[0] == '0'); });
+  return on.get();
+}
+
 void make_regions(Regions &r, int partBits, int64_t rowsA, int64_t rowsB, int streams, int rwB, hipStream_t stream,
                   int lineRecords = 0) {
   const int numParts = 1 << partBits;
@@ -302,8 +310,8 @@
   size_t bBytes = 0;
   if (streams > 0) {
     const uint64_t mean = (static_cast<uint64_t>(rowsB) / (static_cast<uint64_t>(numParts) * streams)) << record_stream_slack();
-    if (lineRecords == static_cast<int>(kCompactLineRecords)) {
-      ws.capB = static_cast<uint32_t>(((2 * mean + 64) / kCompactLineRecords + 2) | 1ull);
+    if (lineRecords == static_cast<int>(kCompactLineRecords) || lineRecords == kBlockLineRecords) {
+      ws.capB = static_cast<uint32_t>(((2 * mean + 64) / static_cast<uint64_t>(lineRecords) + 2) | 1ull);
       bBytes = 128ull * ws.capB * numParts * streams;
     } else if (lineRecords) {
       ws.capB = static_cast<uint32_t>(((2 * mean + 64 + 7) / 8 * 8) | 8ull);
@@ -615,6 +623,13 @@
     if (imageMode) imageMerge = rtc_lookup(device, rtc_spec_merge(plan, nd, partBits, a, widen, compact, false, imageMode));
     if (!imageMerge) imageMode = 0;
   }
+  RtcKernel blockScan, blockMerge;
+  bool block = false, blockFellBack = false;
+  if (imageMode == 2 && compact && block_records_enabled() && prev.appended <= (kBlockMaxNewPerPartition << partBits)) {
+    blockScan = rtc_lookup(device, rtc_spec_scan(plan, nd, partBits, 2));
+    blockMerge = rtc_lookup(device, rtc_spec_merge(plan, nd, partBits, a, widen, 2, false, 2));
+    block = blockScan && blockMerge;
+  }
   if (imageMode == 2) {
     const bool mine = outFound && outOld.lineage == prev.lineage && outOld.image && outOld.image != prev.image &&
                       outOld.partBits == partBits && outOld.size <= prevSize && prev.parentGen != 0 && outOld.gen == prev.parentGen;
@@ -628,6 +643,7 @@
   if (imageMode && !imageOut) {
     imageMode = 0;
     knownOut = 0;
+    block = false;
     if (prevSize > 0) grouped_materialize_for_read(device, prevValues, static_cast<size_t>(mw) * prevSize);
   }
   {
@@ -638,6 +654,12 @@
               found && prev.image ? 1 : 0, found && prev.lazyValues ? 1 : 0, grouped ? 1 : 0, lean ? 1 : 0, table ? 1 : 0, compact ? 1 : 0,
               narrow ? 1 : 0, imageMode, knownOut);
   }
+  auto trace_format = [&] {
+    if (hr_trace_enabled() && lean)
+      fprintf(stderr, "fused_hash_reduce_run: records %s%s (batch %d prev %d appended before %d -> groups %u)\n",
+              block ? "block" : compact ? "compact" : "lines16", blockFellBack ? " after block fallback" : "", batchRows, prevSize,
+              found ? prev.appended : -1, res.groups);
+  };
   if (narrow && !imageMode) {
     narrowMerge = rtc_lookup(device, rtc_spec_merge(plan, nd, partBits, a, widen, wantLean && compact,
                                                     wantTable || (prevSize > 0 && !grouped)));
@@ -659,7 +681,7 @@
       SlowScope slow("make_regions");
       const int64_t rowsA = !lean ? length : (prevSize > 0 && !grouped && imageMode != 2) ? prevSize : 0;
       make_regions(r, partBits, rowsA, batchRows, streams, lean ? 4 : 3, stream,
-                   !lean ? 0 : compact ? static_cast<int>(kCompactLineRecords) : 8);
+                   !lean ? 0 : block ? kBlockLineRecords : compact ? static_cast<int>(kCompactLineRecords) : 8);
     }
     Workspace &ws = r.ws;
     ws.widen = widen;
@@ -669,7 +691,8 @@
     ws.outRanges = outRanges;
     Workspace wsPrev = ws;
     wsPrev.streams = 0;
-    RtcKernel leanMerge = imageMode ? imageMerge
+    const RtcKernel &scanKernel = block ? blockScan : lean;
+    RtcKernel leanMerge = imageMode ? (block ? blockMerge : imageMerge)
                           : narrow  ? (lean ? narrowMerge : nullptr)
                           : (lean && (prevSize == 0 || grouped)) ? rtc_lookup(device, rtc_spec_merge(plan, nd, partBits, a, widen, compact)) : nullptr;
     RtcImageArgs imageArgs{nullptr, nullptr, nullptr, nullptr, 0u};
@@ -699,7 +722,7 @@
                     prevKeys.DimValues, prevCapacity, prevValues, 0u, a, prevSize, wsPrev, 0);                         \
     }                                                                                                                  \
     if (batchRows > 0 && lean)                                                                                         \
-      rtc_scan_launch(lean, leanKind, plan, static_cast<uint32_t>(prevSize), batchRows, ws, stream);                   \
+      rtc_scan_launch(scanKernel, leanKind, plan, static_cast<uint32_t>(prevSize), batchRows, ws, stream);             \
     else if (batchRows > 0 && table)                                                                                   \
       rtc_scan_launch(table, RTC_SCAN_TABLE, plan, static_cast<uint32_t>(prevSize), batchRows, ws, stream);            \
     else if (batchRows > 0)                                                                                            \
@@ -708,7 +731,7 @@
     if (leanMerge || tableMerge)                                                                                       \
       rtc_merge_launch(leanMerge ? leanMerge : tableMerge, plan, prevKeys.DimValues, prevCapacity, prevValues,         \
                        static_cast<uint32_t>(prevSize), outKeys.DimValues, outCapacity, outValues, ws, stream, imagePtr, \
-                       result_slot());                                                                                 \
+                       result_slot(), static_cast<uint32_t>(batchRows));                                               \
     else if (lean)                                                                                                     \
       ARES_LAUNCH("hr_fused_merge_kernel", (hr_fused_merge_kernel<ND, 4>), numParts, kThreads, stream, plan,            \
                   prevKeys.DimValues, prevCapacity, prevValues, static_cast<uint32_t>(prevSize), outKeys.DimValues,    \
@@ -721,10 +744,10 @@
     switch (nd) {
       ARES_FUSED_CASE(1) ARES_FUSED_CASE(2) ARES_FUSED_CASE(3) ARES_FUSED_CASE(4)
       default:
-        if (batchRows > 0 && lean) rtc_scan_launch(lean, leanKind, plan, static_cast<uint32_t>(prevSize), batchRows, ws, stream);
+        if (batchRows > 0 && lean) rtc_scan_launch(scanKernel, leanKind, plan, static_cast<uint32_t>(prevSize), batchRows, ws, stream);
         else if (batchRows > 0 && table) rtc_scan_launch(table, RTC_SCAN_TABLE, plan, static_cast<uint32_t>(prevSize), batchRows, ws, stream);
         rtc_merge_launch(leanMerge ? leanMerge : tableMerge, plan, prevKeys.DimValues, prevCapacity, prevValues, static_cast<uint32_t>(prevSize),
-                         outKeys.DimValues, outCapacity, outValues, ws, stream, imagePtr, result_slot());
+                         outKeys.DimValues, outCapacity, outValues, ws, stream, imagePtr, result_slot(), static_cast<uint32_t>(batchRows));
         break;
     }
     {
@@ -738,8 +761,16 @@
       mem_note_dim_rows(device, outKeys, 0, res.groups);
       mem_note_write(device, outValues, static_cast<size_t>(mw) * res.groups);
     }
+    if (block && res.needGeneric == 2u) {
+      r.buf->mark_idle();
+      hip_check(hipMemsetAsync(image_counts(imageOut.get()), 0xFF, sizeof(uint32_t) * kMaxPartitions, stream), "hipMemsetAsync");
+      block = false;
+      blockFellBack = true;
+      continue;
+    }
     if ((narrow || imageMode == 2) && res.needGeneric) {
       r.buf->mark_idle();
+      trace_format();
       return -1;
     }
     if (imageMode == 1 && res.needGeneric) imageMode = 0;
@@ -766,11 +797,13 @@
       grouped_note_write(device, prevKeys.DimValues, slots.row_bytes() * prevCapacity);
       grouped = false;
       imageMode = 0;
+      block = false;
       continue;
     }
     if (res.overflow && lean && grow_record_stream_slack()) continue;
     break;
   }
+  trace_format();
   if (res.overflow) {
     return -1;
   }
@@ -791,11 +824,13 @@
       s.lineage = prev.lineage;
       s.gen = ++g_generation;
       s.parentGen = prev.gen;
+      s.appended = static_cast<int>(res.groups) - prevSize;
       s.lazyValues = true;
     } else if (imageMode == 1) {
       s.image = imageOut;
       s.lineage = ++g_lineage;
       s.gen = ++g_generation;
+      s.appended = static_cast<int>(res.groups) - prevSize;
     }
     if (res.groups > 0) grouped_register(s);
   }
diff --git a/aresdb_amd/csrc/algo/hr_rtc.hip b/aresdb_amd/csrc/algo/hr_rtc.hip
--- a/aresdb_amd/csrc/algo/hr_rtc.hip
+++ b/aresdb_amd/csrc/algo/hr_rtc.hip
@@ -101,7 +101,7 @@
   uint32_t capB, streams, prevSize, chunkRows;
   uint64_t *phases;
   uint32_t k[kNumConsts];
-  uint32_t pad;
+  uint32_t batchRows;
   const uint4 *recA;
   const uint32_t *cursorsA;
   uint64_t capA;
@@ -487,6 +487,8 @@
     args.bitOff[c] = plan.cols[c].bitOff;
   }
   for (int d = 0; d < kFusedDims; d++) args.k[const_slot_dim(d)] = plan.dims[d].f.bbits;
+  for (int k = 0; k < plan.numFilters && k < kFusedFilters; k++)
+    args.k[const_slot_filter(k)] = host_cvt32(plan.filters[k].f.bbits, plan.filters[k].f.bkind, plan.filters[k].f.I);
 }
 
 struct PhaseReport {
@@ -514,8 +516,6 @@
                  uint32_t chunkTiles, uint32_t pad, hipStream_t stream, const char *name) {
   RtcArgs args;
   fill_columns(args, plan);
-  for (int k = 0; k < plan.numFilters && k < kFusedFilters; k++)
-    args.k[const_slot_filter(k)] = host_cvt32(plan.filters[k].f.bbits, plan.filters[k].f.bkind, plan.filters[k].f.I);
   args.k[const_slot_measure()] = plan.measure.f.bbits;
   args.recB = ws.recB;
   args.countsB = ws.countsB;
@@ -599,7 +599,7 @@
 
 void rtc_merge_launch(const RtcKernel &kernel, const FusedPlanD &plan, const uint8_t *prevDims, size_t prevCapacity, const uint8_t *prevValues,
                       uint32_t prevSize, uint8_t *dimOut, size_t outCapacity, uint8_t *outValues, const hr::Workspace &ws,
-                      hipStream_t stream, const RtcImageArgs *image, uint32_t *hostOut) {
+                      hipStream_t stream, const RtcImageArgs *image, uint32_t *hostOut, uint32_t batchRows) {
   RtcMergeArgs args;
   fill_columns(args, plan);
   args.recB = ws.recB;
@@ -620,6 +620,7 @@
   args.streams = static_cast<uint32_t>(ws.streams);
   args.prevSize = prevSize;
   args.chunkRows = ws.chunkRows;
+  args.batchRows = batchRows;
   if (image) {
     args.imgIn = reinterpret_cast<const uint4 *>(image->in);
     args.imgOut = reinterpret_cast<uint4 *>(image->out);
diff --git a/aresdb_amd/csrc/algo/hr_rtc.hpp b/aresdb_amd/csrc/algo/hr_rtc.hpp
--- a/aresdb_amd/csrc/algo/hr_rtc.hpp
+++ b/aresdb_amd/csrc/algo/hr_rtc.hpp
@@ -32,6 +32,7 @@
 };
 void rtc_merge_launch(const RtcKernel &kernel, const FusedPlanD &plan, const uint8_t *prevDims, size_t prevCapacity,
                       const uint8_t *prevValues, uint32_t prevSize, uint8_t *dimOut, size_t outCapacity, uint8_t *outValues,
-                      const hr::Workspace &ws, hipStream_t stream, const RtcImageArgs *image = nullptr, uint32_t *hostOut = nullptr);
+                      const hr::Workspace &ws, hipStream_t stream, const RtcImageArgs *image = nullptr, uint32_t *hostOut = nullptr,
+                      uint32_t batchRows = 0);
 
 }
diff --git a/aresdb_amd/csrc/algo/hr_rtc_gen.hip b/aresdb_amd/csrc/algo/hr_rtc_gen.hip
--- a/aresdb_amd/csrc/algo/hr_rtc_gen.hip
+++ b/aresdb_amd/csrc/algo/hr_rtc_gen.hip
@@ -419,6 +419,136 @@
        "    const u64 mine = has ? (u64)sLo[T + p * LEFT + kk] << sh : 0ull;\n"
        "    const u64 hdr = ((u64)or8((u32)(mine >> 32)) << 32) | or8((u32)mine);\n"
        "    if (left && fits) STORE_LINE(&myB[((u64)p * a.capB + cur) * 16u + q], r8 ? rec : hdr);\n"
+       "    if (left && !fits) *a.overflow = 1u;\n"
+       "    if (q == 0u) a.countsB[(u64)blockIdx.x * NP + p] = cur * LR + ((left && fits) ? left : 0u);\n"
+       "  }\n"
+       "  PH(6)\n"
+       "  PH_OUT\n"
+       "}\n";
+}
+
+static void kernel_body_block(std::ostringstream &o, const RtcSpec &s) {
+  phase_macros(o, s);
+  o << "#define T 4096u\n#define LR 16u\n#define LEFT 15u\n#define LPL 5u\n"
+       "__device__ __forceinline__ u32 wave_incl_scan(u32 v) {\n"
+       "  v += (u32)__builtin_amdgcn_update_dpp(0, (int)v, 0x111, 0xF, 0xF, false);\n"
+       "  v += (u32)__builtin_amdgcn_update_dpp(0, (int)v, 0x112, 0xF, 0xF, false);\n"
+       "  v += (u32)__builtin_amdgcn_update_dpp(0, (int)v, 0x114, 0xF, 0xF, false);\n"
+       "  v += (u32)__builtin_amdgcn_update_dpp(0, (int)v, 0x118, 0xF, 0xF, false);\n"
+       "  v += (u32)__builtin_amdgcn_update_dpp(0, (int)v, 0x142, 0xA, 0xF, false);\n"
+       "  v += (u32)__builtin_amdgcn_update_dpp(0, (int)v, 0x143, 0xC, 0xF, false);\n"
+       "  return v;\n"
+       "}\n"
+       "extern \"C\" __global__ void __launch_bounds__(1024) hr_scan_rtc(Args a) {\n"
+       "  __shared__ u64 sRec[T + NP * LEFT];\n"
+       "  __shared__ u32 sCount[2][NP];\n"
+       "  __shared__ u32 sStart[NP];\n"
+       "  __shared__ uint2 sLines[(T + NP * LEFT) / LR + 2u];\n"
+       "  __shared__ u32 sWave[16];\n"
+       "  __shared__ u32 sTotalLines;\n"
+       "  const u32 tid = threadIdx.x, lane = tid & 63u, wave = tid >> 6;\n"
+       "  for (u32 p = tid; p < NP; p += 1024u) { sCount[0][p] = 0u; sCount[1][p] = 0u; }\n"
+       "  u32 myLeftN = 0u, myCursor = 0u;\n"
+       "  __syncthreads();\n"
+       "  u64 *myB = reinterpret_cast<u64 *>(a.recB) + (u64)blockIdx.x * NP * a.capB * 16u;\n"
+       "  const u32 numTiles = ((u32)a.length + T - 1u) / T;\n"
+       "  const u32 firstTile = blockIdx.x * a.chunkTiles;\n"
+       "  const u32 endTile = firstTile + a.chunkTiles < numTiles ? firstTile + a.chunkTiles : numTiles;\n"
+       "  u32 tile = firstTile, par = 0u;\n"
+       "  Raw R;\n"
+       "  PH_DECL\n"
+       "  load_tile(R, a, tile * T + tid * 4u);\n"
+       "  const u32 q = tid & 15u;\n"
+       "  while (tile < endTile) {\n"
+       "    u32 i0 = tile * T + tid * 4u;\n"
+       "    u32 hh[4], cv[4], cw[4], alive[4], rank[4];\n"
+       "    const u32 next = tile + 1u;\n"
+       "    eval4p(R, a, i0, hh, cv, cw, alive, next * T + tid * 4u);\n"
+       "    const u32 rc0 = i0 - firstTile * T;\n"
+       "    u32 *cnt = sCount[par];\n"
+       "#pragma unroll\n"
+       "    for (int j = 0; j < 4; j++) {\n"
+       "      rank[j] = 0u;\n"
+       "      if (alive[j]) rank[j] = __hip_atomic_fetch_add(&cnt[hh[j] >> (32 - PB)], 1u, __ATOMIC_RELAXED, __HIP_MEMORY_SCOPE_WORKGROUP);\n"
+       "    }\n"
+       "    __syncthreads();\n"
+       "    PH(0)\n"
+       "    u32 myCount = 0u, myLeft = 0u;\n"
+       "    if (tid < NP) { myCount = cnt[tid]; myLeft = myLeftN; }\n"
+       "    const u32 myHave = myCount + myLeft, myLines = myHave / LR;\n"
+       "    const u32 packed = (myCount << 16) | myLines;\n"
+       "    const u32 incl = wave_incl_scan(packed);\n"
+       "    if (lane == 63u) sWave[wave] = incl;\n"
+       "    __syncthreads();\n"
+       "    u32 before = 0u;\n"
+       "#pragma unroll\n"
+       "    for (u32 w = 0u; w < (NP + 63u) / 64u; w++) { const u32 t = sWave[w]; before += w < wave ? t : 0u; }\n"
+       "    const u32 excl = before + incl - packed;\n"
+       "    const u32 myStart = excl >> 16, myLineStart = excl & 0xFFFFu;\n"
+       "    if (tid < NP) {\n"
+       "      sStart[tid] = myLines ? myStart : T + tid * LEFT + myLeft;\n"
+       "      for (u32 c = 0u; c < myLines; c++) sLines[myLineStart + c] = make_uint2(tid | (c << 9) | (myLeft << 18), myStart | (myCursor << 13));\n"
+       "      if (tid == NP - 1u) sTotalLines = myLineStart + myLines;\n"
+       "    }\n"
+       "    __syncthreads();\n"
+       "    PH(1)\n"
+       "#pragma unroll\n"
+       "    for (int j = 0; j < 4; j++)\n"
+       "      if (alive[j]) sRec[sStart[hh[j] >> (32 - PB)] + rank[j]] = ((u64)((hh[j] << PB) | ((rc0 + (u32)j) >> 9)) << 32) | cv[j];\n"
+       "    __syncthreads();\n"
+       "    PH(2)\n"
+       "    const u32 totalLines = sTotalLines;\n"
+       "    for (u32 L0 = tid >> 4; L0 < totalLines; L0 += 64u * LPL) {\n"
+       "      u32 e[LPL], lf[LPL], st[LPL], cu[LPL];\n"
+       "      u64 rec[LPL];\n"
+       "#pragma unroll\n"
+       "      for (u32 j = 0u; j < LPL; j++) {\n"
+       "        const u32 L = L0 + j * 64u;\n"
+       "        const uint2 w = L < totalLines ? sLines[L] : make_uint2(0u, 0u);\n"
+       "        e[j] = w.x & 0x3FFFFu; lf[j] = w.x >> 18; st[j] = w.y & 0x1FFFu; cu[j] = w.y >> 13;\n"
+       "      }\n"
+       "#pragma unroll\n"
+       "      for (u32 j = 0u; j < LPL; j++) {\n"
+       "        const u32 p = e[j] & 511u, idx = (e[j] >> 9) * LR + q;\n"
+       "        rec[j] = sRec[idx < lf[j] ? T + p * LEFT + idx : st[j] + idx - lf[j]];\n"
+       "      }\n"
+       "#pragma unroll\n"
+       "      for (u32 j = 0u; j < LPL; j++) {\n"
+       "        const u32 p = e[j] & 511u, line = cu[j] + (e[j] >> 9);\n"
+       "        if (L0 + j * 64u < totalLines && line < a.capB) myB[((u64)p * a.capB + line) * 16u + q] = rec[j];\n"
+       "      }\n"
+       "    }\n"
+       "    __syncthreads();\n"
+       "    PH(3)\n"
+       "    if (tid < NP) {\n"
+       "      const u32 rem = myHave - myLines * LR;\n"
+       "      if (myLines) {\n"
+       "        const u32 from = myStart + myLines * LR - myLeft, to = T + tid * LEFT;\n"
+       "        u64 t[LEFT];\n"
+       "#pragma unroll\n"
+       "        for (u32 k = 0u; k < LEFT; k++) t[k] = sRec[from + k];\n"
+       "#pragma unroll\n"
+       "        for (u32 k = 0u; k < LEFT; k++) sRec[to + k] = t[k];\n"
+       "      }\n"
+       "      myLeftN = rem;\n"
+       "      u32 cur = myCursor + myLines;\n"
+       "      if (cur > a.capB) { *a.overflow = 1u; cur = a.capB; }\n"
+       "      myCursor = cur;\n"
+       "      cnt[tid] = 0u;\n"
+       "    }\n"
+       "    par ^= 1u;\n"
+       "    tile = next;\n"
+       "    PH(4)\n"
+       "  }\n"
+       "  __syncthreads();\n"
+       "  if (tid < NP) sLines[tid] = make_uint2(myLeftN, myCursor);\n"
+       "  __syncthreads();\n"
+       "  PH(5)\n"
+       "  for (u32 p = tid >> 4; p < NP; p += 64u) {\n"
+       "    const uint2 m = sLines[p];\n"
+       "    const u32 left = m.x, cur = m.y;\n"
+       "    const bool fits = cur < a.capB;\n"
+       "    if (left && fits) myB[((u64)p * a.capB + cur) * 16u + q] = q < left ? sRec[T + p * LEFT + q] : 0ull;\n"
        "    if (left && !fits) *a.overflow = 1u;\n"
        "    if (q == 0u) a.countsB[(u64)blockIdx.x * NP + p] = cur * LR + ((left && fits) ? left : 0u);\n"
        "  }\n"
@@ -804,7 +934,8 @@
     if (!gen_widen(o, s) || !gen_agg(o, s)) return "";
     kernel_body_table(o);
   } else if (kind == RTC_SCAN_COMPACT) {
-    kernel_body_compact(o, s);
+    if (s.compact == 2) kernel_body_block(o, s);
+    else kernel_body_compact(o, s);
   } else {
     Lines16 rec{sort64 ? "cw[j]" : "0u"};
     if (avg) rec.row = "(a.rowBase + i0 + j) | (alive[j] & 0x80000000u)";
@@ -950,9 +1081,10 @@
 
 std::string generate_merge(const RtcSpec &s) {
   const int nd = s.nd, partBits = s.partBits, image = s.image, vectorVW = s.kind == RTC_VECTOR_MERGE ? s.vectorVW : 0;
-  const bool compact = s.compact != 0, regionA = s.regionA != 0;
+  const bool block = s.compact == 2, compact = s.compact == 1, regionA = s.regionA != 0;
   if (nd < 1 || nd > kFusedDims) return "";
   if (image && vectorVW) return "";
+  if (block && (image != 2 || vectorVW || regionA || partBits < 3 || s.numFilters < 0 || s.numFilters > kFusedFilters)) return "";
   if (compact && (vectorVW || partBits < 3)) return "";
   if (partBits < 2) return "";
   const SlotLayout SL = slot_layout(s.dimWidth, nd, 4);
@@ -961,7 +1093,7 @@
   o << kPrelude
     << "struct MArgs { const u32 *vals[" << kFusedCols << "]; const u8 *nulls[" << kFusedCols << "]; const u32 *recB; const u32 *countsB;\n"
        "  const u32 *prevRanges; const u8 *prevDims; const u8 *prevValues; u8 *dimOut; u8 *outValues; u32 *outCount; u32 *outRanges;\n"
-       "  u64 prevCapacity, outCapacity; u32 bitOff[" << kFusedCols << "]; u32 capB, streams, prevSize, chunkRows; u64 *phases; u32 k[" << kNumConsts << "]; u32 pad;\n"
+       "  u64 prevCapacity, outCapacity; u32 bitOff[" << kFusedCols << "]; u32 capB, streams, prevSize, chunkRows; u64 *phases; u32 k[" << kNumConsts << "]; u32 batchRows;\n"
        "  const uint4 *recA; const u32 *cursorsA; u64 capA;\n"
        "  const uint4 *imgIn; uint4 *imgOut; const u32 *imgInCount; u32 *imgOutCount; u32 *hostOut; u32 knownOut, pad2; };\n"
        "#define FINISH() { __syncthreads(); if (threadIdx.x == 0u && a.hostOut) { __threadfence(); \\\n"
@@ -1072,6 +1204,18 @@
          "    }\n"
          "  }\n"
          "}\n";
+  else if (block)
+    o << "__device__ __forceinline__ void consume(const Stage &s, u32 lane, u32 p, u32 *sKeys, u32 *sRows, u64 *sVals, u32 *sClaimed, u32 *sOverflow, u32 *queue, u32 &qn) {\n"
+         "#pragma unroll\n"
+         "  for (int k = 0; k < 4; k++) {\n"
+         "#pragma unroll\n"
+         "    for (u32 j = 0u; j < 2u; j++) {\n"
+         "      const bool valid = 2u * lane + j < s.rem[k];\n"
+         "      const u32 z = j ? s.r[k].z : s.r[k].x, hw = j ? s.r[k].w : s.r[k].y;\n"
+         "      consume_one(valid, s.rb[k] + (hw & ((1u << PB) - 1u)), hw >> PB, z, 0u, lane, sKeys, sRows, sVals, sClaimed, sOverflow, queue, qn);\n"
+         "    }\n"
+         "  }\n"
+         "}\n";
   else
     o << "__device__ __forceinline__ void consume(const Stage &s, u32 lane, u32 p, u32 *sKeys, u32 *sRows, u64 *sVals, u32 *sClaimed, u32 *sOverflow, u32 *queue, u32 &qn) {\n"
          "#pragma unroll\n"
@@ -1093,6 +1237,34 @@
     o << "    bits[" << d << "] = x; ok[" << d << "] = okb;\n  }\n";
   }
   if (!vectorVW) o << "}\n";
+  if (block) {
+    o << "__device__ __forceinline__ bool block_row(const MArgs &a, u32 row, u32 &hash) {\n  u32 keep = 1u;\n";
+    auto column = [&](const RtcExpr &e) {
+      const int c = e.col;
+      o << "    const u32 v = " << column_elem(s.step[c], e.akind == K_I32, "a.vals[" + std::to_string(c) + "]", "row") << ";\n";
+      if (s.nullMask & (1u << c)) o << "    const u32 bit = row + a.bitOff[" << c << "]; const u32 okb = (a.nulls[" << c << "][bit >> 3] >> (bit & 7u)) & 1u;\n";
+      else o << "    const u32 okb = 1u;\n";
+    };
+    for (int k = 0; k < s.numFilters; k++) {
+      const RtcExpr &e = s.filters[k];
+      if (e.col < 0 || e.col >= kFusedCols) return "";
+      o << "  {\n";
+      column(e);
+      if (!gen_compare(e, o, "v", "okb", "keep", const_name(const_slot_filter(k)))) return "";
+      o << "  }\n";
+    }
+    for (int d = 0; d < nd; d++) o << "  u32 xv" << d << ", xo" << d << ";\n";
+    for (int d = 0; d < nd; d++) {
+      const RtcExpr &e = s.dims[d];
+      o << "  {\n";
+      column(e);
+      o << "    u32 x;\n";
+      if (!gen_value(e, o, "v", "okb", "x", const_name(const_slot_dim(d)))) return "";
+      o << "    xv" << d << " = x" << width_mask(SL.width[d]) << "; xo" << d << " = okb;\n  }\n";
+    }
+    gen_row_hash(o, SL, [](int d) { return "xv" + std::to_string(d); }, [](int d) { return "xo" + std::to_string(d); }, "hash", "  ");
+    o << "  return keep != 0u;\n}\n";
+  }
   const bool wide = s.aggWidth == 8;
   o << "extern \"C\" __global__ void __launch_bounds__(1024) hr_merge_rtc(MArgs a) {\n"
        "  __shared__ __attribute__((aligned(16))) u32 sKeys[SLOTS];\n"
@@ -1101,6 +1273,8 @@
        "  __shared__ u32 sRunCount[256];\n"
        "  __shared__ u32 sQueue[16u * QCAP * QW];\n"
        "  __shared__ u32 sClaimed, sOverflow, sCount, sBase, sEmit;\n"
+    << (block ? "  __shared__ u32 sSearch;\n" : "")
+    <<
        "  const u32 tid = threadIdx.x, lane = tid & 63u, wave = tid >> 6, p = blockIdx.x;\n"
        "  STAMP(0)\n";
   if (image == 2)
@@ -1111,7 +1285,7 @@
          "      reinterpret_cast<uint4 *>(sRows)[i] = img[SLOTS / 4u + i];\n"
          "    }\n"
          "    for (u32 i = tid; i < SLOTS / 2u; i += 1024u) reinterpret_cast<uint4 *>(sVals)[i] = img[SLOTS / 2u + i];\n"
-         "    if (tid == 0u) { sClaimed = a.imgInCount[p]; sOverflow = 0u; sCount = 0u; sEmit = 0u; }\n"
+         "    if (tid == 0u) { sClaimed = a.imgInCount[p]; sOverflow = 0u; sCount = 0u; sEmit = 0u; " << (block ? "sSearch = 0u; " : "") << "}\n"
          "  }\n";
   else
     o << "  for (u32 s = tid; s < SLOTS; s += 1024u) { sKeys[s] = 0u; sRows[s] = 0xFFFFFFFFu; sVals[s] = IDENT; }\n"
@@ -1121,7 +1295,8 @@
        "  const u32 *ranges = a.prevRanges ? a.prevRanges + (u64)p * RANGEWORDS : nullptr;\n"
        "  u32 nRanges = ranges ? ranges[0] : 0u;\n"
        "  if (nRanges > MAXRANGES) { if (tid == 0u) a.outCount[2] = 1u; nRanges = 0u; }\n"
-       "  __syncthreads();\n"
+    << (block ? "  nRanges = 0u;\n" : "")
+    << "  __syncthreads();\n"
        "  STAMP(1)\n"
        "  {\n"
        "    const u8 *nullsIn = a.prevDims + (u64)VB * a.prevCapacity;\n"
@@ -1186,8 +1361,8 @@
        "  for (u32 g = lane; g < G; g += 64u) { const u32 c = sRunCount[g]; maxRun = c > maxRun ? c : maxRun; }\n"
        "#pragma unroll\n"
        "  for (int off = 32; off > 0; off >>= 1) { const u32 t = (u32)__shfl_xor((int)maxRun, off); maxRun = t > maxRun ? t : maxRun; }\n"
-       "  const u32 LPR = (maxRun + " << (compact ? "13u) / 14u" : "7u) / 8u") << ";\n"
-       "  if (G > 0u && LPR <= 4u && LPR <= a.capB" << (compact ? "" : " / 8u") << ") {\n"
+       "  const u32 LPR = (maxRun + " << (block ? "15u) / 16u" : compact ? "13u) / 14u" : "7u) / 8u") << ";\n"
+       "  if (G > 0u && LPR <= 4u && LPR <= a.capB" << (compact || block ? "" : " / 8u") << ") {\n"
        "    u32 qn = 0u;\n"
        "    u32 *queue = sQueue + wave * (QCAP * QW);\n"
        "    const u32 units = G * 8u * LPR;\n"
@@ -1198,7 +1373,10 @@
        "        const u32 u = base + (u32)k * 1024u + tid;\n"
        "        const bool in = u < units;\n"
        "        const u32 ul = in ? u >> 3 : 0u, g = ul / LPR, l = ul - g * LPR, cnt = in ? sRunCount[g] : 0u;\n"
-    << (compact ? "        const u32 here = cnt > l * 14u ? cnt - l * 14u : 0u;\n"
+    << (block   ? "        const u32 here = cnt > l * 16u ? cnt - l * 16u : 0u;\n"
+                  "        s.r[k] = reinterpret_cast<const uint4 *>(a.recB)[(((u64)g * NP + p) * a.capB + l) * 8u + (u & 7u)];\n"
+                  "        s.n[k] = here ? 64u : 0u; s.rem[k] = (lane >> 3) * 16u + here; s.rb[k] = g * (a.chunkRows >> 9);\n"
+        : compact ? "        const u32 here = cnt > l * 14u ? cnt - l * 14u : 0u;\n"
                   "        s.r[k] = reinterpret_cast<const uint4 *>(a.recB)[(((u64)g * NP + p) * a.capB + l) * 8u + (u & 7u)];\n"
                   "        s.n[k] = here ? 64u : 0u; s.rem[k] = (lane >> 3) * 14u + here; s.rb[k] = a.prevSize + g * a.chunkRows;\n"
                 : "        const u32 here = cnt > l * 8u ? cnt - l * 8u : 0u;\n"
@@ -1215,7 +1393,25 @@
        "    u32 *queue = sQueue + wave * (QCAP * QW);\n"
        "    const u32 myRuns = (G + 15u - wave) / 16u;\n"
        "    const u32 myCnt = lane < myRuns ? sRunCount[wave + 16u * lane] : 0u;\n";
-  if (compact)
+  if (block)
+    o << "    auto next = [&]() -> Seg {\n"
+         "      Seg c{dummy, 0u, 0u, 0u};\n"
+         "      while (j < myRuns) {\n"
+         "        const u32 cnt = (u32)__builtin_amdgcn_readlane((int)myCnt, (int)j);\n"
+         "        const u32 units = (cnt + 1u) >> 1;\n"
+         "        if (off < units) {\n"
+         "          c.ptr = reinterpret_cast<const uint4 *>(a.recB) + ((u64)(wave + 16u * j) * NP + p) * a.capB * 8u + off;\n"
+         "          c.n = units - off < 64u ? units - off : 64u;\n"
+         "          c.rem = cnt - 2u * off;\n"
+         "          c.rb = (wave + 16u * j) * (a.chunkRows >> 9);\n"
+         "          off += 64u;\n"
+         "          break;\n"
+         "        }\n"
+         "        j++; off = 0u;\n"
+         "      }\n"
+         "      return c;\n"
+         "    };\n";
+  else if (compact)
     o << "    auto next = [&]() -> Seg {\n"
          "      Seg c{dummy, 0u, 0u, 0u};\n"
          "      while (j < myRuns) {\n"
@@ -1259,22 +1455,24 @@
        "    Stage s0, s1, s2;\n"
        "    load(s0);\n"
        "    load(s1);\n"
+       "#define LIVE(s) (s." << (block ? "rem" : "n") << "[0] != 0u)\n"
        "    for (;;) {\n"
        "      load(s2);\n"
-       "      if (!s0.n[0]) break;\n"
+       "      if (!LIVE(s0)) break;\n"
        "      consume(s0, lane, p, sKeys, sRows, sVals, &sClaimed, &sOverflow, queue, qn);\n"
        "      load(s0);\n"
-       "      if (!s1.n[0]) break;\n"
+       "      if (!LIVE(s1)) break;\n"
        "      consume(s1, lane, p, sKeys, sRows, sVals, &sClaimed, &sOverflow, queue, qn);\n"
        "      load(s1);\n"
-       "      if (!s2.n[0]) break;\n"
+       "      if (!LIVE(s2)) break;\n"
        "      consume(s2, lane, p, sKeys, sRows, sVals, &sClaimed, &sOverflow, queue, qn);\n"
        "    }\n"
        "    while (qn) { const u32 take = qn < 64u ? qn : 64u; qn -= take; drain(queue, qn, take, lane, sKeys, sRows, sVals, &sClaimed, &sOverflow); }\n"
        "  }\n"
        "  __syncthreads();\n"
        "  STAMP(3)\n"
-       "  if (sOverflow) { if (tid == 0u) a.outCount[3] = 1u; FINISH() return; }\n";
+    << (block ? "  if (sOverflow) { if (tid == 0u) atomicOr(a.outCount + 3, 1u); FINISH() return; }\n"
+              : "  if (sOverflow) { if (tid == 0u) a.outCount[3] = 1u; FINISH() return; }\n");
   const char *kStoreKeysPos =
       "    for (u32 i = tid; i < SLOTS / 4u; i += 1024u) {\n"
       "      img[i] = reinterpret_cast<const uint4 *>(sKeys)[i];\n"
@@ -1287,12 +1485,43 @@
          "  for (int k = 0; k < SLOTS / 1024; k++) mineNew += (sKeys[tid + (u32)k * 1024u] & NEWG) != 0u;\n"
          "  if (mineNew) __hip_atomic_fetch_add(&sCount, mineNew, __ATOMIC_RELAXED, __HIP_MEMORY_SCOPE_WORKGROUP);\n"
          "  __syncthreads();\n"
-         "  const u32 totalNew = sCount;\n"
-         "  if (tid == 0u) sBase = a.prevSize + (totalNew ? atomicAdd(a.outCount, totalNew) : 0u);\n"
+         "  const u32 totalNew = sCount;\n";
+    if (block)
+      o << "  if (totalNew > " << kBlockSearchCap << "u) { if (tid == 0u) atomicOr(a.outCount + 3, 2u); FINISH() return; }\n";
+    o << "  if (tid == 0u) sBase = a.prevSize + (totalNew ? atomicAdd(a.outCount, totalNew) : 0u);\n"
          "  __syncthreads();\n"
          "  STAMP(4)\n"
-         "  u8 *nullsOut = a.dimOut + (u64)VB * a.outCapacity;\n"
-         "  if (totalNew) {\n"
+         "  u8 *nullsOut = a.dimOut + (u64)VB * a.outCapacity;\n";
+    if (block)
+      o << "  if (totalNew) {\n"
+           "#pragma unroll 1\n"
+           "    for (u32 k = 0u; k < SLOTS / 1024u; k++) {\n"
+           "      const u32 s = tid + k * 1024u;\n"
+           "      if (sKeys[s] & NEWG) sQueue[__hip_atomic_fetch_add(&sSearch, 1u, __ATOMIC_RELAXED, __HIP_MEMORY_SCOPE_WORKGROUP)] = s;\n"
+           "    }\n"
+           "    __syncthreads();\n"
+           "#pragma unroll 1\n"
+           "    for (u32 i = (u32)__builtin_amdgcn_readfirstlane((int)wave), nNew = (u32)__builtin_amdgcn_readfirstlane((int)totalNew); i < nNew; i += 16u) {\n"
+           "      const u32 s = sQueue[i];\n"
+           "      const u32 gh = (p << (32 - PB)) | (sKeys[s] & HMASK), gb = sRows[s];\n"
+           "      u32 found = 0xFFFFFFFFu;\n"
+           "      if (gb <= (a.batchRows >> 9)) {\n"
+           "#pragma unroll 1\n"
+           "        for (u32 j = 0u; j < 8u; j++) {\n"
+           "          const u32 row = gb * 512u + j * 64u + lane;\n"
+           "          u32 h = 0u;\n"
+           "          const bool in = row < a.batchRows;\n"
+           "          const bool keep = block_row(a, in ? row : 0u, h);\n"
+           "          const u64 mm = __ballot(in && keep && h == gh);\n"
+           "          if (mm) { found = gb * 512u + j * 64u + (u32)(__ffsll((long long)mm) - 1); break; }\n"
+           "        }\n"
+           "      }\n"
+           "      if (found == 0xFFFFFFFFu) { found = 0u; if (lane == 0u) atomicOr(a.outCount + 3, 2u); }\n"
+           "      if (lane == 0u) sRows[s] = a.prevSize + found;\n"
+           "    }\n"
+           "    __syncthreads();\n"
+           "  }\n";
+    o << "  if (totalNew) {\n"
          "#pragma unroll\n"
          "    for (int half = 0; half < 2; half++) {\n"
          "      u32 dv[4][ND], nv[4][ND], at[4]; bool has[4];\n"
@@ -1492,8 +1721,10 @@
   }
 }
 
-RtcSpec rtc_spec_scan(const FusedPlanD &plan, int nd, int partBits, bool compact) {
-  return spec_plan_scan(compact ? RTC_SCAN_COMPACT : RTC_SCAN_LINES16, plan, nd, partBits);
+RtcSpec rtc_spec_scan(const FusedPlanD &plan, int nd, int partBits, int compact) {
+  RtcSpec s = spec_plan_scan(compact ? RTC_SCAN_COMPACT : RTC_SCAN_LINES16, plan, nd, partBits);
+  if (compact == 2) s.compact = 2;
+  return s;
 }
 RtcSpec rtc_spec_sort_scan(const FusedPlanD &plan, int nd, int partBits) { return spec_plan_scan(RTC_SCAN_SORT64, plan, nd, partBits); }
 RtcSpec rtc_spec_table_scan(const FusedPlanD &plan, int nd, int partBits, const AggSpec &a, const hr::Widen &w) {
@@ -1504,7 +1735,7 @@
 RtcSpec rtc_spec_vector_scan(int nd, int vw, int partBits) { return spec_vector(RTC_VECTOR_SCAN, nd, nullptr, vw, partBits); }
 RtcSpec rtc_spec_sort_vector_scan(int nd, const int *widths, int partBits) { return spec_vector(RTC_SORT_VECTOR_SCAN, nd, widths, 4, partBits); }
 RtcSpec rtc_spec_hll_scan(int nd, const int *widths, int partBits) { return spec_vector(RTC_HLL_SCAN, nd, widths, 4, partBits); }
-RtcSpec rtc_spec_merge(const FusedPlanD &plan, int nd, int partBits, const AggSpec &a, const hr::Widen &w, bool compact, bool regionA,
+RtcSpec rtc_spec_merge(const FusedPlanD &plan, int nd, int partBits, const AggSpec &a, const hr::Widen &w, int compact, bool regionA,
                        int image) {
   RtcSpec s = spec_of(RTC_MERGE, nd, partBits);
   spec_dims(s, plan);
@@ -1513,6 +1744,13 @@
   spec_agg(s, a, w);
   s.aggWidth = a.width;
   s.compact = compact; s.regionA = regionA; s.image = image;
+  if (compact == 2) {
+    s.numFilters = plan.numFilters;
+    for (int k = 0; k < plan.numFilters && k < kFusedFilters; k++) {
+      s.filters[k] = spec_expr(plan.filters[k], FILTER);
+      if (plan.filters[k].col >= 0 && plan.filters[k].col < kFusedCols) spec_column(s, plan, plan.filters[k].col);
+    }
+  }
   return s;
 }
 RtcSpec rtc_spec_vector_merge(int nd, int vw, int partBits, const AggSpec &a) {
diff --git a/aresdb_amd/csrc/algo/hr_rtc_gen.hpp b/aresdb_amd/csrc/algo/hr_rtc_gen.hpp
--- a/aresdb_amd/csrc/algo/hr_rtc_gen.hpp
+++ b/aresdb_amd/csrc/algo/hr_rtc_gen.hpp
@@ -49,13 +49,14 @@
 inline bool operator!=(const RtcSpec &a, const RtcSpec &b) { return !(a == b); }
 bool phases_enabled();
 
-RtcSpec rtc_spec_scan(const FusedPlanD &plan, int nd, int partBits, bool compact);
+RtcSpec rtc_spec_scan(const FusedPlanD &plan, int nd, int partBits, int compact);
 RtcSpec rtc_spec_sort_scan(const FusedPlanD &plan, int nd, int partBits);
 RtcSpec rtc_spec_table_scan(const FusedPlanD &plan, int nd, int partBits, const AggSpec &a, const hr::Widen &w);
 RtcSpec rtc_spec_vector_scan(int nd, int vw, int partBits);
 RtcSpec rtc_spec_sort_vector_scan(int nd, const int *widths, int partBits);
 RtcSpec rtc_spec_hll_scan(int nd, const int *widths, int partBits);
-RtcSpec rtc_spec_merge(const FusedPlanD &plan, int nd, int partBits, const AggSpec &a, const hr::Widen &w, bool compact = false,
+constexpr int kBlockSearchCap = 256;
+RtcSpec rtc_spec_merge(const FusedPlanD &plan, int nd, int partBits, const AggSpec &a, const hr::Widen &w, int compact = 0,
                        bool regionA = false, int image = 0);
 RtcSpec rtc_spec_vector_merge(int nd, int vw, int partBits, const AggSpec &a);
 
```

Result: faster. 94.73 billion rows/s, median of 3 (+3.2%).
